# nreHieW/Eagle

Hardware: AMD Instinct MI355X
Metric: frames/sec end-to-end (detect+keypoint+homography) @1280x720 (higher is better)
Workload: dtype f32 (split: hi/lo binary16 pairs, 3 x fp16 MFMA per product, fp32 accumulate); detector (1.4 % of the FLOP): f32, exact v_mfma_f32_16x16x4_f32 chains

## Files before the change

### eagle_amd/csrc/common.h

```cpp
#pragma once
#include <hip/hip_runtime.h>
#include <hip/hip_fp16.h>
#include <cstdint>
#include <cstdio>
#include <string>
#include <vector>

#include "../../include/eagle.h"

namespace eagle {

enum Act : int { ACT_NONE = 0, ACT_RELU = 1, ACT_SILU = 2 };

struct Err {
    int code;
    std::string msg;
};
[[noreturn]] void fail(int code, const char* fmt, ...);

#define HIP_CHECK(expr)                                                                                \
    do {                                                                                               \
        hipError_t _e = (expr);                                                                        \
        if (_e != hipSuccess) ::eagle::fail(EAGLE_E_HIP, "%s failed: %s (%s:%d)", #expr, hipGetErrorString(_e), \
                                            __FILE__, __LINE__);                                       \
    } while (0)

void ensure_max_dynamic_lds(const void* fn, int bytes);

struct TView {
    void* p = nullptr;
    int n = 0, h = 0, w = 0;
    int c = 0;
    int cs = 0;
    int off = 0;
    int f32 = 0;
    size_t esize() const { return f32 ? 4 : 2; }
    TView slice(int o, int cc) const { TView v = *this; v.off = off + o; v.c = cc; return v; }
};

struct ConvConfig {
    int ks = 3, stride = 1;
    int kc = 0;
    int nt = 0;
    int wx = 2;
    int cin = 0, cout_pad = 0;
    int variant = 0;
};
struct ArgmaxPart { float score; int idx; };
struct ConvLaunch {
    ConvConfig cfg;
    TView x, y, r1, r2;
    const void* w = nullptr;
    const float* bias = nullptr;
    int pre_act = 0, post_act = 0;
    int out_f32 = 0;
    double flop = 0;
    float descale = 1.0f;
    ArgmaxPart* const* am_slot = nullptr;
    unsigned* const* sat_slot = nullptr;
};
int conv_tiles_per_frame(int precision, const ConvConfig& cfg, int ho, int wo);
void conv_tile_shape(int precision, const ConvConfig& cfg, int* th, int* tw);
bool conv_supported(int precision, const ConvConfig& cfg);
void conv_launch(int precision, const ConvLaunch& L, hipStream_t s);
size_t conv_weight_elems(int precision, const ConvConfig& cfg);
size_t conv_lds_bytes(int precision, const ConvConfig& cfg);
void conv_tile_weights(int precision, const ConvConfig& cfg, const float* w_hwio, int cin_real, int cout_real, void* dst, float* descale = nullptr);
inline int prec_tensor_fmt(int precision) { return precision == EAGLE_PREC_F32 ? 1 : precision == EAGLE_PREC_F32S ? 2 : 0; }
inline bool prec_is_f16_kernels(int precision) { return precision == EAGLE_PREC_F16 || precision == EAGLE_PREC_F32S; }
ConvConfig conv_choose(int precision, int ks, int stride, int cin_pad, int cout_pad, int wo, bool plain_epilogue = false, bool second_residual = false);

struct BneckLaunch {
    TView x, res, y;
    const void *w1 = nullptr, *w2 = nullptr, *w3 = nullptr;
    const float *b1 = nullptr, *b2 = nullptr, *b3 = nullptr;
    float ds1 = 1.f, ds2 = 1.f, ds3 = 1.f;
    unsigned* const* sat_slot = nullptr;
    unsigned long long* dbg = nullptr;
    bool ds_fused = false;
};
bool bneck_supported(const TView& x, int cmid, int cout);
void bneck_tile_weights(const float* w, int taps, int cin, int cout, std::vector<_Float16>& out, float* descale);
void bneck_scale_bias(std::vector<float>& b, float descale);
void bneck_launch(const BneckLaunch& L, hipStream_t s);

struct StemLaunch {
    const uint8_t* bgr = nullptr;
    int n = 0, sh = 0, sw = 0;
    int dh = 540, dw = 960;
    const void* w = nullptr;
    const float* bias = nullptr;
    float descale = 1.f;
    TView y;
    unsigned* const* sat_slot = nullptr;
};
bool stem_supported(int precision, int ks, int stride, int cin, int cout);
void stem_tile_weights(const float* w , std::vector<_Float16>& out, float* descale);
void stem_launch(const StemLaunch& L, hipStream_t s);

struct LetterBox { int new_h, new_w, top, left, out_h, out_w; };
LetterBox letterbox_geometry(int h, int w, int imgsz, int square = 0);
int detector_anchor_count(int h, int w, int imgsz, int square);
void preprocess_launch(int precision, const uint8_t* d_bgr, int n, int h, int w, const TView& kp, const TView& det,
                       const LetterBox& lb, hipStream_t s, int which = 3, int det_precision = -1);
struct FuseUp { TView z; };
void fuse_sum_launch(const TView& base, const FuseUp* ups, int n_up, int relu, const TView& y, hipStream_t s, unsigned* sat = nullptr);
void maxpool5_launch(const TView& x, const TView& y, hipStream_t s);
void upsample2_launch(const TView& x, const TView& y, hipStream_t s);
void split_to_f32_launch(const TView& x, const TView& y, hipStream_t s);

void heat_argmax_launch(const TView& logits, ArgmaxPart* parts, int chunks, hipStream_t s);

struct DetLevel { TView box, cls; int gh, gw; float stride; int a0; };
struct DetScratch {
    int A = 0;
    float* boxes = nullptr;
    float* conf = nullptr;
    int* cls = nullptr;
    unsigned long long* keys = nullptr;
    int* count = nullptr;
};
void yolo_decode_launch(const DetLevel* lv, int n_lv, int n, int nc, float conf_floor, const DetScratch& sc, hipStream_t s);

struct PostParams {
    int frame_h, frame_w, in_h, in_w;
    int hm_h, hm_w, hm_chunks;
    double keypoint_conf, detector_conf, ransac_thresh;
    float nms_iou;
    int ransac_max_iters, lm_iters;
};
void nms_launch(const DetScratch& sc, int n, const PostParams& pp, EagleFrameResult* d_out, hipStream_t s);
int nms_anchor_limit();
void check_anchor_limit(const EagleConfig& cfg);
void post_launch(const ArgmaxPart* parts, int n, const PostParams& pp, EagleFrameResult* d_out, hipStream_t s);
void reproject_launch(EagleFrameResult* d_recs, const double* d_Hs, const unsigned char* d_flags, int n, int frame_h, int frame_w, hipStream_t s);
void homography_only_launch(const float* d_img, const float* d_world, int npts, double thresh, int max_iters, int lm_iters,
                            double* d_H, uint8_t* d_mask, int* d_ok, hipStream_t s);


struct ClipView {
    const uint8_t* bgr = nullptr;
    const uint8_t* g[3] = {nullptr, nullptr, nullptr};
    int lh[3] = {0, 0, 0}, lw[3] = {0, 0, 0};
    int levels = 0;
    int n = 0, h = 0, w = 0;
};
struct MemList { int n; EagleFlowKp kp[EAGLE_N_LANDMARKS]; };
struct ChainState {
    int n_prev; EagleFlowKp prev[EAGLE_N_LANDMARKS];
    int has_H, compute_h; double H[9];
    int stalled;
    int error;
    int lk_valid, lk_n;
    float lk_prev[2 * EAGLE_N_LANDMARKS], lk_next[2 * EAGLE_N_LANDMARKS];
    unsigned char lk_status[EAGLE_N_LANDMARKS];
    int flow_n; EagleFlowKp flow[EAGLE_N_LANDMARKS];
};
void clip_view_levels(ClipView& cv);
void gray_pyramid_launch(const uint8_t* d_bgr, int n, int h, int w, uint8_t* g0, uint8_t* g1, uint8_t* g2, hipStream_t s);
void lk_launch(const ClipView& cv, int src_frame, int dst_frame, ChainState* st, const MemList* mem, int kint, hipStream_t s);
struct EccResult { int ok, iters; double rho; float M[6]; };
void ecc_small_launch(const uint8_t* gray, uint8_t* small, int n, int h, int w, int dh, int dw, double inv_scale , hipStream_t s);
void ecc_launch(const uint8_t* small, const uint8_t* carry, const int2* pairs, int n_pairs, EccResult* out, int h, int w, int max_iter, double eps, hipStream_t s);
struct YuvArgs {
    const uint8_t* src;
    uint8_t* dst;
    int h, w;
    int64_t frame_stride, y_pitch, c_offset, c_pitch, v_offset;
    int c_step;
    int vec;
};
void yuv_to_bgr_launch(const YuvArgs& a, int n, hipStream_t s);
struct AnnotArgs {
    const uint8_t* src;
    uint8_t* dst;
    const EaglePrim* prims;
    const int32_t* offs;
    int h, w, fmt;
    int64_t frame_stride, y_pitch, c_offset, c_pitch, v_offset;
    int c_step;
    int vec;
};
void annotate_launch(const AnnotArgs& a, int n, hipStream_t s);
int overlay_from_record(const EagleFrameResult& rec, const int32_t* team_ids, const int32_t* team_vals, int n_team, EaglePrim* out);
void check_prims(const EaglePrim* prims, const int32_t* offs, int n);
void team_colors_launch(const uint8_t* d_bgr, int n_frames, int fh, int fw, const EagleCrop* d_crops, int n_crops, int* d_counts, hipStream_t s);

void reid_crop_launch(const uint8_t* d_bgr, int n_frames, int fh, int fw, const EagleCrop* d_crops, int n, const TView& out, hipStream_t s);
void reid_conv7_launch(const TView& x, const float* w, const float* b, const TView& y, int n, hipStream_t s);
void reid_maxpool3s2_launch(const TView& x, const TView& y, int n, hipStream_t s);
void reid_avgpool2_launch(const TView& x, const TView& y, int n, hipStream_t s);
void reid_dw3_launch(const TView& x, const float* w, const float* b, const TView& y, int n, hipStream_t s);
void reid_gate_launch(const TView* streams, const float* w1, const float* b1, const float* w2, const float* b2, int c_real, int r, float* g, const TView& y, int n, hipStream_t s);
void reid_head_launch(const TView& x, const float* w, const float* b, float* feats, int dim, int n, hipStream_t s);

struct Tracker;
Tracker* tracker_create(const EagleTrackParams* p);
void tracker_destroy(Tracker* t);
bool tracker_apply(Tracker* t, EagleFrameResult* rec, int frame_h, int frame_w, double detector_conf, const double* warp = nullptr,
                   const float* feats = nullptr, const int* feat_det = nullptr, int n_feat = 0);
void similarity_ransac(const double* p0, const double* p1, int n, double* W6);
int lk_debug(const char* key, long long value, void* out, long long out_bytes);
void decode_mem_launch(const ArgmaxPart* parts, int n, const PostParams& pp, MemList* mem, int first, int stride, hipStream_t s);
void chain_launch(const ClipView& cv, ChainState* st, const MemList* mem, EagleFrameResult* recs, const PostParams& pp, int frame,
                  int kint, int hint, int calib, hipStream_t s);
void flow_filter_launch(const ClipView& cv, ChainState* st, int hue_frame, hipStream_t s);

}
```

### eagle_amd/csrc/conv.hip

```cpp
#include <algorithm>
#include <cmath>
#include <cstdlib>
#include <mutex>

#include "common.h"
#include "dmath.h"
#include "conv_internal.h"

namespace eagle {

static int f16_ps(int kc) { const int g = kc / 8; return kc * 2 + ((g % 2 == 0) ? 16 : 0); }
static int f16_ni(int ks, int kc) { return (ks * ks * (kc / 8) + 3) / 4; }

enum FormKind { GENERIC, WSTAT, ADIRECT };
enum StrideForm { S1, S2D, S2T, S1L };
enum WeightImage { W_F32, W_F16, W_F16_S2D, W_SPLIT, W_SPLIT_AD, W_SPLIT_S2D, W_SPLIT_M32 };
struct Form {
    int prec, variant, kind;
    int pw;
    int sform, rows, cols;
    int kc, nt, halo_bufs;
    int wimage;
    int grid_cap;
    ConvKernelGetter get;
};
static constexpr Form gen(int prec, int variant, int pw, int wimage, int kind = GENERIC) { return {prec, variant, kind, pw, S1, 0, 0, 0, 0, 0, wimage, 0, nullptr}; }
static constexpr Form ad(int prec, int variant, int sform, int rows, int cols, int nt, int halo_bufs, int wimage, ConvKernelGetter get, int grid_cap = 0)
{
    return {prec, variant, ADIRECT, 0, sform, rows, cols, prec == EAGLE_PREC_F16 ? 32 : 16, nt, halo_bufs, wimage, grid_cap, get};
}
static constexpr int F16 = EAGLE_PREC_F16, F32 = EAGLE_PREC_F32, F32S = EAGLE_PREC_F32S;
static constexpr Form g_forms[] = {
    gen(F32, 0, 4, W_F32), gen(F32, 3, 2, W_F32), gen(F32, 4, 1, W_F32),
    gen(F16, 0, 4, W_F16), gen(F16, 2, 4, W_F16), gen(F16, 3, 2, W_F16), gen(F16, 4, 1, W_F16), gen(F16, 6, 4, W_F16, WSTAT), gen(F16, 7, 2, W_F16, WSTAT),
    ad(F16, 8, S1, 4, 32, 12, 2, W_F16, conv_ad_kernel_s1_bn192), ad(F16, 9, S1, 8, 32, 6, 2, W_F16, conv_ad_kernel_s1_bn96),
    ad(F16, 10, S2D, 4, 32, 12, 2, W_F16_S2D, conv_ad_kernel_s2_bn192), ad(F16, 11, S2D, 8, 32, 6, 2, W_F16_S2D, conv_ad_kernel_s2_bn96),
    gen(F32S, 0, 4, W_SPLIT), gen(F32S, 3, 2, W_SPLIT), gen(F32S, 18, 6, W_SPLIT),
    ad(F32S, 8, S1, 4, 32, 12, 2, W_SPLIT_AD, conv_ad_split_kernel_bn192), ad(F32S, 9, S1, 8, 32, 6, 2, W_SPLIT_AD, conv_ad_split_kernel_bn96),
    ad(F32S, 10, S2D, 4, 32, 12, 2, W_SPLIT_S2D, conv_ad_split_kernel_s2_bn192), ad(F32S, 11, S2D, 8, 32, 6, 2, W_SPLIT_S2D, conv_ad_split_kernel_s2_bn96),
    ad(F32S, 12, S1, 8, 32, 3, 2, W_SPLIT_AD, conv_ad_split_kernel48), ad(F32S, 13, S1, 16, 32, 3, 1, W_SPLIT_AD, conv_ad_split_kernel48sb),
    ad(F32S, 19, S1, 16, 32, 3, 2, W_SPLIT_AD, conv_ad_split_kernel48ring, 256),
    ad(F32S, 14, S2T, 4, 32, 12, 1, W_SPLIT_AD, conv_ad_split_kernel_s2t_bn192), ad(F32S, 15, S2T, 4, 32, 6, 1, W_SPLIT_AD, conv_ad_split_kernel_s2t_bn96),
    ad(F32S, 21, S1, 4, 32, 12, 2, W_SPLIT_M32, conv_ad_split32_kernel_bn192), ad(F32S, 22, S1, 8, 32, 6, 2, W_SPLIT_M32, conv_ad_split32_kernel_bn96),
    ad(F32S, 23, S1, 2, 64, 12, 2, W_SPLIT_M32, conv_ad_split32_kernel_w64_bn192), ad(F32S, 24, S1, 4, 64, 6, 2, W_SPLIT_M32, conv_ad_split32_kernel_w64_bn96),
    ad(F32S, 27, S1L, 6, 30, 12, 2, W_SPLIT_M32, conv_ad_split32_kernel_lin30)};
static constexpr int LIN_PIXELS = 128;

static const Form* find_form(int precision, int variant)
{
    for (const Form& f : g_forms)
        if (f.prec == precision && f.variant == variant) return &f;
    return nullptr;
}
static const Form& form_of(int precision, const ConvConfig& c)
{
    const Form* f = find_form(precision, c.variant);
    if (!f) fail(EAGLE_E_NOKERNEL, "no conv kernel form: prec=%d variant=%d", precision, c.variant);
    return *f;
}
static int kind_of(int precision, const ConvConfig& c) { const Form* f = find_form(precision, c.variant); return f ? f->kind : -1; }

static size_t lds_bytes(int precision, const ConvConfig& c)
{
    const Form& f = form_of(precision, c);
    if (f.kind == ADIRECT) {
        int hpix, rec, strips;
        if (precision == EAGLE_PREC_F16) { hpix = f.sform == S2D ? (f.rows + 1) * 33 : (f.rows + 2) * 34; rec = 96; strips = 4 * 32 * 112; }
        else if (f.wimage == W_SPLIT_M32) { hpix = (f.rows + 2) * (f.cols + 2); rec = 80; strips = 4 * 32 * 128; }
        else { hpix = f.sform == S2T ? (2 * f.rows + 1) * 66 : (f.rows + 2) * 34; rec = 96; strips = 4 * 16 * 208; }
        const int slabs = ((hpix * rec + 1023) / 1024 + 3) / 4 * 4;
        return (size_t)f.halo_bufs * slabs * 1024 + strips;
    }
    const int th = 4 * f.pw / c.wx, tw = 16 * c.wx;
    const int hw = (tw - 1) * c.stride + c.ks, hh = (th - 1) * c.stride + c.ks;
    const int bn = c.nt * 16;
    if (precision == EAGLE_PREC_F16) {
        const size_t operands = (size_t)f16_ni(c.ks, c.kc) * 4 * bn * 16 + (size_t)hh * hw * f16_ps(c.kc);
        const size_t strips = (size_t)4 * f.pw * 16 * (bn * 2 + 16);
        return f.kind == WSTAT ? operands + strips + 16 : std::max(operands + 16, strips);
    }
    if (precision == EAGLE_PREC_F32S) {
        const size_t operands = (size_t)f16_ni(c.ks, c.kc) * 2 * 4 * bn * 16 + (size_t)hh * hw * f16_ps(2 * c.kc);
        const size_t strips = (size_t)4 * f.pw * 16 * (bn * 4 + 16);
        return std::max(operands + 16, strips);
    }
    return (size_t)c.ks * c.ks * (c.kc / 4) * 4 * bn * 4 + (size_t)hh * hw * (c.kc + 1) * 4;
}

size_t conv_lds_bytes(int precision, const ConvConfig& c) { return lds_bytes(precision, c); }
void conv_tile_shape(int precision, const ConvConfig& c, int* th, int* tw)
{
    const Form& f = form_of(precision, c);
    *th = f.kind == ADIRECT ? f.rows : 4 * f.pw / c.wx; *tw = f.kind == ADIRECT ? f.cols : 16 * c.wx;
}

int conv_tiles_per_frame(int precision, const ConvConfig& c, int ho, int wo)
{
    int th, tw;
    conv_tile_shape(precision, c, &th, &tw);
    if (form_of(precision, c).sform == S1L) return (ho * wo + LIN_PIXELS - 1) / LIN_PIXELS;
    return ((wo + tw - 1) / tw) * ((ho + th - 1) / th);
}

static const Inst* generic_inst(int precision, const ConvConfig& c)
{
    for (auto part : {conv_inst_part0, conv_inst_part1, conv_inst_part2, conv_inst_part3, conv_inst_split0, conv_inst_split1, conv_inst_split2}) {
        int n = 0;
        const Inst* t = part(&n);
        for (int k = 0; k < n; ++k)
            if (t[k].prec == precision && t[k].ks == c.ks && t[k].s == c.stride && t[k].kc == c.kc && t[k].nt == c.nt && t[k].variant == c.variant) return &t[k];
    }
    return nullptr;
}
bool conv_supported(int precision, const ConvConfig& c)
{
    const Form* f = find_form(precision, c.variant);
    if (f && f->kind == ADIRECT) return c.ks == 3 && c.stride == (f->sform == S1 || f->sform == S1L ? 1 : 2) && c.kc == f->kc && c.nt == f->nt;
    return f && generic_inst(precision, c);
}

struct Tuned { int ks, s, cin, cout, wo, kc, nt, wx, variant; };
static const Tuned g_tuned[] = {
#include "conv_tuned.inc"
    {0, 0, 0, 0, 0, 0, 0, 0, 0}};
static const Tuned g_tuned_f32[] = {
#include "conv_tuned_f32.inc"
    {0, 0, 0, 0, 0, 0, 0, 0, 0}};
static const Tuned g_tuned_split[] = {
#include "conv_tuned_split.inc"
    {0, 0, 0, 0, 0, 0, 0, 0, 0}};
static bool tuned_match(const Tuned& t, const ConvConfig& c, int wo, ConvConfig* q)
{
    if (t.ks != c.ks || t.s != c.stride || t.cin != c.cin || t.cout != c.cout_pad || t.wo != wo) return false;
    *q = c; q->kc = t.kc; q->nt = t.nt; q->wx = t.wx; q->variant = t.variant;
    return true;
}

static bool env_force(const char* name, int* a, int* b, int* c) { const char* f = getenv(name); return f && sscanf(f, "%d,%d,%d", a, b, c) == 3; }
static bool env_off(const char* name) { const char* e = getenv(name); return e && atoi(e) == 0; }

static const int g_nts[] = {6, 4, 3, 2, 1};
static ConvConfig with_ad(ConvConfig c, int kc, int v192, int v96)
{
    c.kc = kc;
    if (c.cout_pad % 192 == 0) { c.nt = 12; c.variant = v192; } else { c.nt = 6; c.variant = v96; }
    return c;
}

static ConvConfig choose_f32(ConvConfig c, int wo)
{
    ConvConfig q = c; q.kc = (c.cin < 16) ? 4 : 16;
    if (env_force("EAGLE_F32_FORCE", &q.nt, &q.wx, &q.variant) && (q.wx == 1 || q.wx == 2) && q.nt >= 1 && c.cout_pad % (16 * q.nt) == 0 &&
        conv_supported(EAGLE_PREC_F32, q) && lds_bytes(EAGLE_PREC_F32, q) <= 160 * 1024)
        return q;
    for (const Tuned& t : g_tuned_f32)
        if (tuned_match(t, c, wo, &q) && conv_supported(EAGLE_PREC_F32, q)) return q;
    c.nt = 1;
    for (int nt : g_nts)
        if (c.cout_pad % (16 * nt) == 0) { c.nt = nt; break; }
    c.kc = (c.cin < 16) ? 4 : 16;
    if (c.stride == 2 && c.ks == 3) {
        q = c; q.variant = 3;
        if (conv_supported(EAGLE_PREC_F32, q)) return q;
    }
    return c;
}

static ConvConfig choose_split(ConvConfig c, int wo, bool plain_epilogue)
{
    const int prec = EAGLE_PREC_F32S, cin = c.cin, cout = c.cout_pad;
    ConvConfig q = c;
    if (env_force("EAGLE_CONV_FORCE", &q.kc, &q.nt, &q.variant) && cin % q.kc == 0 && cout % (16 * q.nt) == 0 && conv_supported(prec, q) &&
        (form_of(prec, q).sform != S1L || (plain_epilogue && wo == form_of(prec, q).cols))) {
        if (form_of(prec, q).pw == 6) q.wx = 3;
        if (lds_bytes(prec, q) <= 160 * 1024) return q;
    }
    if (plain_epilogue && c.ks == 3 && c.stride == 2 && cin % 48 == 0 && cout % 96 == 0) return with_ad(c, 16, 14, 15);
    if (!env_off("EAGLE_CONV_M32") && plain_epilogue && c.ks == 3 && c.stride == 1 && cin % 16 == 0 && cout % 96 == 0) {
        q = with_ad(c, 16, 21, wo > 32 ? 24 : 22);
        if (q.variant == 21 && wo == 30) q.variant = 27;
        return q;
    }
    for (const Tuned& t : g_tuned_split)
        if (tuned_match(t, c, wo, &q)) {
            const Form* f = find_form(prec, q.variant);
            if (kind_of(prec, q) == ADIRECT && !(plain_epilogue && cin % (f->sform == S2D ? 16 : 48) == 0)) continue;
            if (conv_supported(prec, q) && lds_bytes(prec, q) <= 160 * 1024) return q;
        }
    if (plain_epilogue && c.ks == 3 && c.stride == 1 && cin % 48 == 0 && cout % 96 == 0) return with_ad(c, 16, 8, 9);
    static const int skcs[] = {32, 16, 8};
    long best = -1;
    c.nt = 1; c.kc = 8; c.variant = 0;
    for (int variant : {0, 3})
        for (int nt : g_nts) {
            if (cout % (16 * nt)) continue;
            for (int kc : skcs) {
                if (cin % kc) continue;
                ConvConfig t = c; t.nt = nt; t.kc = kc; t.variant = variant;
                if (!conv_supported(prec, t)) continue;
                if (lds_bytes(prec, t) > 80 * 1024) continue;
                const int pw = form_of(prec, t).pw;
                if (nt * pw > 12) continue;
                const long score = (long)nt * pw * 1000 + kc * 10 + (variant == 0 ? 1 : 0);
                if (score > best) { best = score; c.nt = nt; c.kc = kc; c.variant = variant; }
            }
        }
    return c;
}

static ConvConfig choose_f16(ConvConfig c, int wo, bool plain_epilogue, bool plain_one)
{
    const int prec = EAGLE_PREC_F16, cin = c.cin, cout = c.cout_pad;
    ConvConfig q = c;
    if (env_force("EAGLE_CONV_FORCE", &q.kc, &q.nt, &q.variant) && cin % q.kc == 0 && cout % (16 * q.nt) == 0 && conv_supported(prec, q) &&
        lds_bytes(prec, q) <= 160 * 1024 && (kind_of(prec, q) == WSTAT ? plain_one : kind_of(prec, q) == ADIRECT ? plain_epilogue : true))
        return q;
    if (plain_epilogue && c.ks == 3 && c.stride == 1 && cin % 32 == 0 && cout % 96 == 0) return with_ad(c, 32, 8, 9);
    if (plain_epilogue && c.ks == 3 && c.stride == 2 && cin % 8 == 0 && cin >= 32 && cout % 96 == 0) return with_ad(c, 32, 10, 11);
    for (const Tuned& t : g_tuned)
        if (tuned_match(t, c, wo, &q)) {
            if (kind_of(prec, q) == WSTAT && !plain_one) continue;
            if (conv_supported(prec, q) && lds_bytes(prec, q) <= 160 * 1024) return q;
        }
    static const int kcs[] = {64, 48, 32, 16, 8};
    long best = -1;
    c.nt = 1; c.kc = 8;
    for (int nt : g_nts) {
        if (cout % (16 * nt)) continue;
        for (int kc : kcs) {
            if (cin % kc) continue;
            ConvConfig t = c; t.nt = nt; t.kc = kc;
            if (!conv_supported(prec, t)) continue;
            if (lds_bytes(prec, t) > 80 * 1024) continue;
            const long score = (long)kc * nt * 1000 + kc;
            if (score > best) { best = score; c.nt = nt; c.kc = kc; }
        }
    }
    return c;
}

ConvConfig conv_choose(int precision, int ks, int stride, int cin_pad, int cout_pad, int wo, bool plain_epilogue, bool second_residual)
{
    ConvConfig c;
    c.ks = ks; c.stride = stride; c.cin = cin_pad; c.cout_pad = cout_pad;
    c.wx = (wo > 16) ? 2 : 1;
    if (precision == EAGLE_PREC_F32) return choose_f32(c, wo);
    if (precision == EAGLE_PREC_F32S) return choose_split(c, wo, plain_epilogue);
    return choose_f16(c, wo, plain_epilogue, plain_epilogue && !second_residual);
}

size_t conv_weight_elems(int precision, const ConvConfig& c)
{
    const int bn = c.nt * 16, nblk = c.cout_pad / bn, nch = c.cin / c.kc;
    switch (form_of(precision, c).wimage) {
    case W_F16_S2D: return (size_t)nblk * (4 * c.cin / 32) * 16 * bn * 8;
    case W_F16: return (size_t)nblk * nch * f16_ni(c.ks, c.kc) * 4 * bn * 8;
    case W_SPLIT_S2D: return (size_t)nblk * (4 * c.cin / 16) * 6 * 4 * bn * 8;
    case W_SPLIT_M32: return (size_t)nblk * (c.cin / 16) * 18 * (bn / 32) * 512;
    case W_SPLIT_AD: return (size_t)nblk * (c.cin / 16) * 14 * 4 * bn * 8;
    case W_SPLIT: return (size_t)nblk * nch * f16_ni(c.ks, c.kc) * 2 * 4 * bn * 8;
    default: return (size_t)nblk * nch * c.ks * c.ks * (c.kc / 4) * 4 * bn;
    }
}

void conv_tile_weights(int precision, const ConvConfig& c, const float* w, int cin_real, int cout_real, void* dst, float* descale)
{
    const int bn = c.nt * 16, nblk = c.cout_pad / bn, nch = c.cin / c.kc, taps = c.ks * c.ks, wimage = form_of(precision, c).wimage;
    auto W = [&](int tap, int ci, int co) -> float {
        return (ci < cin_real && co < cout_real) ? w[((size_t)tap * cin_real + ci) * cout_real + co] : 0.0f;
    };
    if (descale) *descale = 1.0f;
    if (precision == EAGLE_PREC_F32S) {
        float amax = 0.f;
        for (size_t k = 0; k < (size_t)taps * cin_real * cout_real; ++k) amax = std::max(amax, std::fabs(w[k]));
        int e = 0;
        if (amax > 0.f) (void)std::frexp(amax, &e);
        const int sw = 15 - e;
        const float scale = std::ldexp(1.0f, sw);
        if (descale) *descale = std::ldexp(1.0f, -(sw + 4));
        _Float16* d = (_Float16*)dst;
        if (wimage == W_SPLIT_S2D) {
            const int per_phase = c.cin / 16;
            for (int b = 0; b < nblk; ++b)
                for (int ch = 0; ch < 4 * per_phase; ++ch)
                    for (int k = 0; k < 6; ++k)
                        for (int qq = 0; qq < 4; ++qq)
                            for (int nn = 0; nn < bn; ++nn)
                                for (int j = 0; j < 8; ++j) {
                                    const int ph = ch / per_phase, c0 = (ch - ph * per_phase) * 16, ry = ph >> 1, rx = ph & 1;
                                    const int tp = k < 4 ? k : 2 * (k - 4) + (qq >> 1), tyy = tp >> 1, txx = tp & 1;
                                    const int ky = tyy == 0 ? (ry == 1 ? 0 : -1) : (ry == 0 ? 1 : 2), kx = txx == 0 ? (rx == 1 ? 0 : -1) : (rx == 0 ? 1 : 2);
                                    float v = 0.f;
                                    if (ky >= 0 && kx >= 0) v = W(ky * 3 + kx, c0 + (qq & 1) * 8 + j, b * bn + nn) * scale;
                                    const _Float16 hi = (_Float16)v;
                                    *d++ = k < 4 ? hi : (_Float16)(v - (float)hi);
                                }
            return;
        }
        if (wimage == W_SPLIT_M32) {
            for (int b = 0; b < nblk; ++b)
                for (int ch = 0; ch < c.cin / 16; ++ch)
                    for (int tap = 0; tap < 9; ++tap)
                        for (int part = 0; part < 2; ++part)
                            for (int mb = 0; mb < bn / 32; ++mb)
                                for (int l = 0; l < 64; ++l)
                                    for (int j = 0; j < 8; ++j) {
                                        const float v = W(tap, ch * 16 + (l >> 5) * 8 + j, b * bn + mb * 32 + (l & 31)) * scale;
                                        const _Float16 hi = (_Float16)v;
                                        *d++ = part == 0 ? hi : (_Float16)(v - (float)hi);
                                    }
            return;
        }
        if (wimage == W_SPLIT_AD) {
            for (int b = 0; b < nblk; ++b)
                for (int ch = 0; ch < c.cin / 16; ++ch)
                    for (int k = 0; k < 14; ++k)
                        for (int qq = 0; qq < 4; ++qq)
                            for (int nn = 0; nn < bn; ++nn)
                                for (int j = 0; j < 8; ++j) {
                                    const int tap = k < 9 ? k : 2 * (k - 9) + (qq >> 1);
                                    float v = 0.f;
                                    if (tap < 9) v = W(tap, ch * 16 + (qq & 1) * 8 + j, b * bn + nn) * scale;
                                    const _Float16 hi = (_Float16)v;
                                    *d++ = k < 9 ? hi : (_Float16)(v - (float)hi);
                                }
            return;
        }
        const int G = c.kc / 8, NGR = taps * G, NI = f16_ni(c.ks, c.kc);
        for (int b = 0; b < nblk; ++b)
            for (int ch = 0; ch < nch; ++ch)
                for (int i = 0; i < NI; ++i)
                    for (int part = 0; part < 2; ++part)
                        for (int qq = 0; qq < 4; ++qq)
                            for (int nn = 0; nn < bn; ++nn)
                                for (int j = 0; j < 8; ++j) {
                                    const int g = 4 * i + qq;
                                    float v = 0.f;
                                    if (g < NGR) { const int tap = g / G, cg = g % G; v = W(tap, ch * c.kc + cg * 8 + j, b * bn + nn) * scale; }
                                    const _Float16 hi = (_Float16)v;
                                    *d++ = part == 0 ? hi : (_Float16)(v - (float)hi);
                                }
        return;
    }
    if (wimage == W_F16_S2D) {
        _Float16* d = (_Float16*)dst;
        const int nch2 = 4 * c.cin / 32;
        for (int b = 0; b < nblk; ++b)
            for (int ch = 0; ch < nch2; ++ch)
                for (int g = 0; g < 16; ++g)
                    for (int nn = 0; nn < bn; ++nn)
                        for (int j = 0; j < 8; ++j) {
                            const int tp = g / 4, cg = g % 4, tyy = tp >> 1, txx = tp & 1;
                            const int sc = ch * 32 + cg * 8 + j, ph = sc / c.cin, ci = sc - ph * c.cin, ry = ph >> 1, rx = ph & 1;
                            const int ky = tyy == 0 ? (ry == 1 ? 0 : -1) : (ry == 0 ? 1 : 2), kx = txx == 0 ? (rx == 1 ? 0 : -1) : (rx == 0 ? 1 : 2);
                            *d++ = (_Float16)((ky < 0 || kx < 0) ? 0.f : W(ky * 3 + kx, ci, b * bn + nn));
                        }
        return;
    }
    if (precision == EAGLE_PREC_F16) {
        const int G = c.kc / 8, NGR = taps * G, NI = f16_ni(c.ks, c.kc);
        _Float16* d = (_Float16*)dst;
        for (int b = 0; b < nblk; ++b)
            for (int ch = 0; ch < nch; ++ch)
                for (int g = 0; g < NI * 4; ++g)
                    for (int nn = 0; nn < bn; ++nn)
                        for (int j = 0; j < 8; ++j) {
                            float v = 0.f;
                            if (g < NGR) {
                                const int tap = g / G, cg = g % G;
                                v = W(tap, ch * c.kc + cg * 8 + j, b * bn + nn);
                            }
                            *d++ = (_Float16)v;
                        }
    } else {
        const int CSTEPS = c.kc / 4;
        float* d = (float*)dst;
        for (int b = 0; b < nblk; ++b)
            for (int ch = 0; ch < nch; ++ch)
                for (int tap = 0; tap < taps; ++tap)
                    for (int cs = 0; cs < CSTEPS; ++cs)
                        for (int qq = 0; qq < 4; ++qq)
                            for (int nn = 0; nn < bn; ++nn) *d++ = W(tap, ch * c.kc + cs * 4 + qq, b * bn + nn);
    }
}

static std::mutex g_page_mutex;
static const void* conv_zero_page()
{
    static void* z[64] = {};
    int dev = 0;
    HIP_CHECK(hipGetDevice(&dev));
    std::lock_guard<std::mutex> g(g_page_mutex);
    if (!z[dev]) { HIP_CHECK(hipMalloc(&z[dev], 256)); HIP_CHECK(hipMemset(z[dev], 0, 256)); }
    return z[dev];
}
static void* conv_trash_page()
{
    static void* z[64] = {};
    int dev = 0;
    HIP_CHECK(hipGetDevice(&dev));
    std::lock_guard<std::mutex> g(g_page_mutex);
    if (!z[dev]) HIP_CHECK(hipMalloc(&z[dev], 8192));
    return z[dev];
}

void conv_launch(int precision, const ConvLaunch& L, hipStream_t s)
{
    const ConvConfig& c = L.cfg;
    if (!conv_supported(precision, c)) fail(EAGLE_E_NOKERNEL, "no conv kernel instance: prec=%d ks=%d s=%d kc=%d nt=%d", precision, c.ks, c.stride, c.kc, c.nt);
    const Form& f = form_of(precision, c);
    ConvArgs a;
    a.x = L.x.p; a.xcs = L.x.cs; a.xoff = L.x.off; a.N = L.x.n; a.H = L.x.h; a.W = L.x.w;
    a.w = L.w; a.bias = L.bias;
    a.y = L.y.p; a.ycs = L.y.cs; a.yoff = L.y.off; a.Ho = L.y.h; a.Wo = L.y.w;
    a.r1 = L.r1.p; a.r1cs = L.r1.cs; a.r1off = L.r1.off;
    a.r2 = L.r2.p; a.r2cs = L.r2.cs; a.r2off = L.r2.off;
    a.descale = L.descale;
    if (precision == EAGLE_PREC_F32S) {
        if (L.x.f32 != 2 || (L.r1.p && L.r1.f32 != 2) || (L.r2.p && L.r2.f32 != 2) || L.y.f32 != (L.out_f32 ? 1 : 2))
            fail(EAGLE_E_INVALID, "split conv: operand tensor formats do not match the family");
        a.xcs *= 2; a.xoff *= 2; a.r1cs *= 2; a.r1off *= 2; a.r2cs *= 2; a.r2off *= 2;
        if (!L.out_f32) { a.ycs *= 2; a.yoff *= 2; }
    }
    if (!a.r1 && a.r2) { a.r1 = a.r2; a.r1cs = a.r2cs; a.r1off = a.r2off; a.r2 = nullptr; }
    a.pre_act = L.pre_act; a.post_act = L.post_act; a.out_f32 = L.out_f32 || precision == EAGLE_PREC_F32;
    a.wx = c.wx;
    a.nchunks = c.cin / c.kc;
    a.zeros = conv_zero_page(); a.trash = conv_trash_page(); a.xcd = 0; a.gy = 1; a.stack = 0;
    a.am = L.am_slot ? *L.am_slot : nullptr; a.am_cs = c.cout_pad;
    a.sat = (L.sat_slot && precision == EAGLE_PREC_F32S) ? *L.sat_slot : nullptr;
    if (f.kind == ADIRECT) {
        if (a.out_f32 || a.pre_act != 0 || a.post_act > 1 || L.am_slot || (precision == EAGLE_PREC_F32S && c.cin % (f.wimage == W_SPLIT_AD ? 48 : 16)))
            fail(EAGLE_E_NOKERNEL, "A-direct conv needs 2-byte / split output, pre_act none, post_act in {none, ReLU} and, in the split family, Cin = 16 k (48 k for variants 8, 9 and 12 - 15)");
        if (f.sform == S2D) a.nchunks = 4 * c.cin / c.kc;
        a.tiles_x = (a.Wo + f.cols - 1) / f.cols; a.tiles_y = (a.Ho + f.rows - 1) / f.rows;
        if (f.sform == S1L) {
            if (a.Wo != f.cols || a.W != a.Wo || a.H != a.Ho) fail(EAGLE_E_NOKERNEL, "linear A-direct conv (variant %d) needs a map %d columns wide, got %d x %d", c.variant, f.cols, a.Ho, a.Wo);
            a.tiles_x = (a.Ho * a.Wo + LIN_PIXELS - 1) / LIN_PIXELS; a.tiles_y = 1;
        }
        a.gy = c.cout_pad / (c.nt * 16);
        const size_t lim = (size_t)1 << 31;
        if ((size_t)a.N * a.H * a.W * a.xcs * 2 >= lim || (size_t)a.N * a.Ho * a.Wo * std::max(std::max(a.ycs, a.r1 ? a.r1cs : 0), a.r2 ? a.r2cs : 0) * 2 >= lim)
            fail(EAGLE_E_INVALID, "fp16 conv: a tensor of %d frames reaches 2 GiB; use a smaller device batch", a.N);
        const int nres = (a.r1 ? 1 : 0) + (a.r2 ? 1 : 0);
        const int items = a.tiles_x * a.tiles_y * a.N * a.gy;
        const bool deep = items <= 256;
        for (bool d : {false, true}) ensure_max_dynamic_lds((const void*)f.get(nres, d), 160 * 1024);
        hipLaunchKernelGGL(f.get(nres, deep), dim3(f.grid_cap ? std::min(items, f.grid_cap) : items), dim3(256), lds_bytes(precision, c), s, a);
        HIP_CHECK(hipGetLastError());
        return;
    }
    const int th = 4 * f.pw / c.wx, tw = 16 * c.wx;
    a.tiles_x = (a.Wo + tw - 1) / tw; a.tiles_y = (a.Ho + th - 1) / th;
    if (precision == EAGLE_PREC_F32) {
        if (!env_off("EAGLE_F32_STACK") && c.stride == 1 && a.N > 1 && a.Ho == a.H) { a.stack = 1; a.tiles_y = (a.N * (a.Ho + 1) + th - 1) / th; }
        if ((size_t)a.N * a.H * a.W * a.xcs * 4 >= ((size_t)1 << 31)) fail(EAGLE_E_INVALID, "fp32 conv: the input tensor of %d frames reaches 2 GiB; use a smaller device batch", a.N);
    }
    const bool ws = f.kind == WSTAT;
    if (a.am && (!prec_is_f16_kernels(precision) || ws))
        fail(EAGLE_E_NOKERNEL, "fused heat-map maxima need the generic fp16 kernel");
    if (prec_is_f16_kernels(precision)) {
        const size_t lim = (size_t)1 << 31;
        const size_t cs_out = std::max(std::max(a.out_f32 ? 2 * a.ycs : a.ycs, a.r1 ? a.r1cs : 0), a.r2 ? a.r2cs : 0);
        if ((size_t)a.N * a.H * a.W * a.xcs * 2 >= lim || (size_t)a.N * a.Ho * a.Wo * cs_out * 2 >= lim)
            fail(EAGLE_E_INVALID, "fp16 conv: a tensor of %d frames reaches 2 GiB; use a smaller device batch", a.N);
    }
    const ConvKernel fn = generic_inst(precision, c)->fn;
    const size_t lds = lds_bytes(precision, c);
    ensure_max_dynamic_lds((const void*)fn, 160 * 1024);
    const int gy = c.cout_pad / (c.nt * 16);
    int gx = a.stack ? a.tiles_x * a.tiles_y : a.tiles_x * a.tiles_y * a.N;
    if (ws) {
        if (c.kc != c.cin || a.out_f32 || a.r2 || a.pre_act != 0 || a.post_act > 1 || (size_t)a.N * a.H * a.W * a.xcs * 2 >= (1ull << 31) || (size_t)a.N * a.Ho * a.Wo * std::max(a.ycs, a.r1 ? a.r1cs : 0) * 2 >= (1ull << 31))
            fail(EAGLE_E_NOKERNEL, "weight-stationary conv needs kc == cin, fp16 output, at most one residual, pre_act none, post_act in {none, ReLU} and tensors below 2 GiB (kc=%d cin=%d)", c.kc, c.cin);
        const int per_cu = (int)std::max<size_t>(1, std::min<size_t>(2, (160 * 1024) / lds));
        const int unit = 8 * gy;
        gx = std::max(unit, std::min((gx * gy + unit - 1) / unit * unit, 256 * per_cu / unit * unit));
    }
    a.gy = gy;
    a.xcd = (prec_is_f16_kernels(precision) && !ws && (c.ks == 3 || (c.ks == 1 && gy > 1))) ? 1 : 0;
    dim3 grid(gx, gy);
    if (a.xcd) grid = dim3(gx * gy, 1);
    if (ws) grid = dim3(gx, 1);
    hipLaunchKernelGGL(fn, grid, dim3(256), lds, s, a);
    HIP_CHECK(hipGetLastError());
}

}
```

### eagle_amd/csrc/conv_ad_split.inc

```
#ifndef EAGLE_CONV_AD_SPLIT_INC
#define EAGLE_CONV_AD_SPLIT_INC
#ifndef EAGLE_ABL_AD
#define EAGLE_ABL_AD 0
#endif
#if EAGLE_ABL_AD == 1 || EAGLE_ABL_AD == 6
__device__ __forceinline__ f32x4 abl_ad_xor(const half8& a_, const half8& b_, f32x4 c_)
{
    const u32x4 ua = __builtin_bit_cast(u32x4, a_), ub = __builtin_bit_cast(u32x4, b_);
    u32x4 uc = __builtin_bit_cast(u32x4, c_);
    uc[0] = uc[0] ^ ua[0] ^ ub[3];
    return __builtin_bit_cast(f32x4, uc);
}
#define EAGLE_MFMA_AD(A_, B_, C_) abl_ad_xor(A_, B_, C_)
#else
#define EAGLE_MFMA_AD(A_, B_, C_) __builtin_amdgcn_mfma_f32_16x16x32_f16(A_, B_, C_, 0, 0, 0)
#endif
template <int CQ, int PG, int RES, int KQ = 1, bool SB = false, bool S2 = false, bool S2T = false>
__global__ __launch_bounds__(256, 2) void conv_split_ad_kernel(ConvArgs a)
{
    static_assert(!S2 || (KQ == 1 && !SB), "stride-2 form: plain ring");
    static_assert(!S2T || (SB && !S2 && PG == 1), "true stride-2 form: one pixel group, single halo buffer");
    static_assert(CQ * PG * KQ == 4, "four waves per workgroup");
    static_assert(!SB || KQ == 1 || S2T, "single-buffer form: no K split (except the true stride-2 form)");
    static_assert(KQ == 1 || (KQ == 2 && (CQ == 1 || S2T)), "K split: one Cout group (two in the true stride-2 form)");
// ... 51 lines not shown
#pragma unroll
        for (int s = 0; s < KPW; ++s) {
            int o[2];
#pragma unroll
            for (int hq = 0; hq < 2; ++hq) {
                const int kg = hq * KPW + s;
                if (kg < 9) {
                    o[hq] = bbase + tapoff(kg) * PS;
                } else {
                    const int t0 = 2 * (kg - 9), t1 = t0 + 1 < 9 ? t0 + 1 : t0;
                    o[hq] = bpair + bsel * ((tapoff(t1) - tapoff(t0)) * PS) + tapoff(t0) * PS;
                }
            }
            bk[s] = kq == 0 ? o[0] : o[1];
        }
    }

    auto decode = [&](int item, int& n, int& ty, int& tx, int& nb) {
        int t = item / gy; nb = item - t * gy;
        tx = t % a.tiles_x; t /= a.tiles_x;
        ty = t % a.tiles_y; n = t / a.tiles_y;
    };
    int h_g = 0, h_ch = 0, h_item = item0;
    int h_iy0, h_ix0, h_gb;
    auto halo_origin = [&](int item) {
        int n, ty, tx, nb; decode(item, n, ty, tx, nb);
        h_iy0 = S2T ? 2 * ty * TH - 1 : ty * TH - 1; h_ix0 = S2T ? 64 * tx - 1 : tx * 32 - 1;
        h_gb = S2 ? n * a.H : (((n * a.H + h_iy0) * a.W + h_ix0) * a.xcs + a.xoff) * 2;
    };
    const int cin_s2 = nch * 4;
    halo_origin(h_item);
    auto issue_h = [&]() {
        char* dst = Hb + (SB ? 0 : (h_g & 1)) * HB;
        const unsigned so = S2 ? 0u : (unsigned)(h_ch * 32) * 2u;
        const int s2_ph = S2 ? (h_ch * 16) / cin_s2 : 0, s2_c0 = S2 ? h_ch * 16 - s2_ph * cin_s2 : 0;
#pragma unroll
        for (int k = 0; k < HK; ++k) {
            int hy, hx, unit; bool live;
            if constexpr (RECOMP) {
                int e = e0 + NW * 64 * k;
                asm volatile("" : "+v"(e));
                const int pix = (int)(((unsigned)e * 43691u) >> 18), slot = e - pix * 6;
                hy = S2T ? (int)(((unsigned)pix * 993u) >> 16) : S2 ? (int)(((unsigned)pix * 1986u) >> 16) : (int)(((unsigned)pix * 1928u) >> 16); hx = pix - hy * HW_;
                unit = (slot & 1) * 2 + (slot >> 1);
                live = pix < HPIX && slot < 4;
                if constexpr (S2T) { const int pl = hx >= 33 ? 1 : 0; hx = 2 * (hx - 33 * pl) + pl; live = live && hx <= 64; }
            } else {
                hy = hpk[k] & 0xFF; hx = (hpk[k] >> 8) & 0xFF; unit = (hpk[k] >> 16) & 7; live = hpk[k] >= 0;
            }
            const int iy = S2 ? 2 * (h_iy0 + hy) + (s2_ph >> 1) : h_iy0 + hy, ix = S2 ? 2 * (h_ix0 + hx) + (s2_ph & 1) : h_ix0 + hx;
            const unsigned off = !(live && (unsigned)iy < (unsigned)a.H && (unsigned)ix < (unsigned)a.W) ? OOB
                                 : S2 ? (unsigned)((((h_gb + iy) * a.W + ix) * a.xcs + a.xoff + 2 * s2_c0 + unit * 8) * 2)
                                      : (unsigned)(h_gb + ((hy * a.W + hx) * a.xcs + unit * 8) * 2);
            __builtin_amdgcn_raw_ptr_buffer_load_lds(xrs, (__attribute__((address_space(3))) void*)(dst + (wave + NW * k) * 1024), 16,
                                                     ((EAGLE_ABL_AD == 3 || EAGLE_ABL_AD >= 6) && h_g > 0) ? OOB : off, so, 0, 0);
        }
        if (h_g + 1 >= GC) return;
        ++h_g;
        if (++h_ch == nch) { h_ch = 0; ++h_item; halo_origin(h_item); }
    };
    if constexpr (!SB) issue_h();
    int gc = 0;
    for (int item = item0; item < item_end; ++item) {
        int n, ty, tx, nb; decode(item, n, ty, tx, nb);
        const int oy0 = ty * TH, ox0 = tx * 32;
        f32x4 acc[NT][PW];
#pragma unroll
        for (int i = 0; i < NT; ++i)
#pragma unroll
            for (int p = 0; p < PW; ++p) acc[i][p] = f32x4{0.f, 0.f, 0.f, 0.f};
        u32x4 A[RING][NT];
        unsigned wsrc = (unsigned)(nb * nch * KPC * 4) * (unsigned)(BN * 16) + (unsigned)(kq * KPW) * KSTEP;
        const unsigned wend = wsrc - (unsigned)(kq * KPW) * KSTEP + (unsigned)(nch * KPC) * KSTEP;
        int a_s = 0;
        bool abl_a_done = false;
        auto load_a = [&](int slot) {
            const unsigned so = wsrc < wend ? wsrc : wend - KSTEP;
#pragma unroll
            for (int tt = 0; tt < NT; ++tt)
                if (!((EAGLE_ABL_AD == 2 || EAGLE_ABL_AD >= 6) && abl_a_done)) A[slot][tt] = __builtin_amdgcn_raw_buffer_load_b128(wrs, wlane + tt * 256, so, 0);
            wsrc += KSTEP;
            if constexpr (KQ > 1) { if (++a_s == KPW) { a_s = 0; wsrc += (unsigned)(KPC - KPW) * KSTEP; } }
        };
        load_a(0); load_a(1);
        abl_a_done = true;
        auto chunk = [&](auto ph_, auto k0_) {
            constexpr int PH = decltype(ph_)::value, K0 = decltype(k0_)::value;
            if constexpr (SB) {
                __builtin_amdgcn_s_barrier();
                issue_h();
                asm volatile("s_waitcnt vmcnt(0)" ::: "memory");
                __builtin_amdgcn_s_barrier();
            } else {
                asm volatile("s_waitcnt vmcnt(6)" ::: "memory");
                __builtin_amdgcn_s_barrier();
                issue_h();
            }
            const char* hb = Hb + (SB ? 0 : (gc & 1)) * HB;
            half8 B[2][PW];
            auto read_b = [&](int slot, int kk) {
                if constexpr (KQ == 2) {
#pragma unroll
                    for (int p = 0; p < PW; ++p)
                        B[slot][p] = *(const half8*)(hb + bk[kk] + ((p >> 1) * ROWREC + (p & 1) * 16) * PS);
                } else if constexpr (S2) {
                    const int tp = kk < 4 ? kk : 2 * (kk - 4), ky = tp >> 1, kx = tp & 1;
                    const char* hp = kk < 4 ? hb + bbase : hb + bpair + bsel * PS;
#pragma unroll
                    for (int p = 0; p < PW; ++p)
                        B[slot][p] = *(const half8*)(hp + (((p >> 1) + ky) * HW_ + (p & 1) * 16 + kx) * PS);
                } else if (kk < 9) {
#pragma unroll
                    for (int p = 0; p < PW; ++p)
                        B[slot][p] = *(const half8*)(hb + bbase + ((p >> 1) * ROWREC + (p & 1) * 16 + tapoff(kk)) * PS);
                } else {
                    const int t0 = 2 * (kk - 9), t1 = t0 + 1 < 9 ? t0 + 1 : t0;
                    const int d = (tapoff(t1) - tapoff(t0)) * PS;
                    const char* hp = hb + bpair + bsel * d;
#pragma unroll
                    for (int p = 0; p < PW; ++p)
                        B[slot][p] = *(const half8*)(hp + ((p >> 1) * ROWREC + (p & 1) * 16 + tapoff(t0)) * PS);
                }
            };
            read_b(0, K0);
#pragma unroll
            for (int kk = 0; kk < KPW; ++kk) {
                load_a((PH + kk + 2) % RING);
                if (kk + 1 < KPW && !(EAGLE_ABL_AD == 4 || EAGLE_ABL_AD == 6)) read_b((kk + 1) & 1, K0 + kk + 1);
#pragma unroll
                for (int tt = 0; tt < NT; ++tt)
#pragma unroll
                    for (int p = 0; p < PW; ++p)
                        acc[tt][p] = EAGLE_MFMA_AD((half8)A[(PH + kk) % RING][tt], B[(EAGLE_ABL_AD == 4 || EAGLE_ABL_AD == 6) ? 0 : (kk & 1)][p], acc[tt][p]);
                __builtin_amdgcn_sched_barrier(0);
            }
        };
        using I0 = std::integral_constant<int, 0>;
        constexpr int P1 = KPW % RING, P2 = (2 * KPW) % RING;
        if constexpr (S2) {
            for (int ch = 0; ch < nch; ++ch) { chunk(I0{}, I0{}); ++gc; }
        } else
        for (int ch = 0; ch < nch; ch += 3) {
            if constexpr (KQ == 1) {
                chunk(I0{}, I0{}); ++gc;
                chunk(std::integral_constant<int, P1>{}, I0{}); ++gc;
                chunk(std::integral_constant<int, P2>{}, I0{}); ++gc;
            } else {
                chunk(I0{}, I0{}); ++gc;
                chunk(std::integral_constant<int, P1>{}, I0{}); ++gc;
                chunk(std::integral_constant<int, P2>{}, I0{}); ++gc;
            }
        }
        const int co0 = nb * BN + cq * 48;
        __builtin_amdgcn_sched_barrier(0);
        constexpr int NHR = 8 / KQ;
        const int row0 = (KQ == 2 && kq == 1) ? 2 : 0;
        if constexpr (KQ == 2) {
            if (kq == 1) {
#pragma unroll
                for (int tt = 0; tt < NT; ++tt)
#pragma unroll
                    for (int p = 0; p < 4; ++p) { const f32x4 t = acc[tt][p]; acc[tt][p] = acc[tt][p + 4]; acc[tt][p + 4] = t; }
            }
            char* const X = SB ? Hb : Hb + ((gc - 1) & 1) * HB;
            const int mine = wave * 6144, theirs = (wave ^ (CQ * PG)) * 6144;
#pragma unroll
            for (int rnd = 0; rnd < 2; ++rnd) {
                __builtin_amdgcn_s_barrier();
#pragma unroll
                for (int pp = 0; pp < 2; ++pp)
#pragma unroll
                    for (int tt = 0; tt < NT; ++tt) *(f32x4*)(X + mine + ((pp * NT + tt) * 64 + lane) * 16) = acc[tt][4 + rnd * 2 + pp];
                __builtin_amdgcn_fence(__ATOMIC_RELEASE, "workgroup", "local");
                __builtin_amdgcn_s_barrier();
                __builtin_amdgcn_fence(__ATOMIC_ACQUIRE, "workgroup", "local");
#pragma unroll
                for (int pp = 0; pp < 2; ++pp)
#pragma unroll
                    for (int tt = 0; tt < NT; ++tt) {
                        const f32x4 o = *(const f32x4*)(X + theirs + ((pp * NT + tt) * 64 + lane) * 16);
#pragma unroll
                        for (int r = 0; r < 4; ++r) acc[tt][rnd * 2 + pp][r] = kq == 0 ? acc[tt][rnd * 2 + pp][r] + o[r] : o[r] + acc[tt][rnd * 2 + pp][r];
                    }
            }
        }
        float4 bias[NT];
#pragma unroll
        for (int tt = 0; tt < NT; ++tt) bias[tt] = *(const float4*)(a.bias + co0 + tt * 16 + q * 4);
        const float ds = a.descale;
        int pstrip[3], ppx[3];
#pragma unroll
        for (int i = 0; i < 3; ++i) {
            const int e = i * 64 + lane, px = e / 12, gq = e - px * 12;
            pstrip[i] = px * RS + gq * 16;
            ppx[i] = px | (gq << 8);
        }
        auto piece_off = [&](int hr, int i, int cs, int off) -> unsigned {
            const int oy = oy0 + pg * 4 + row0 + (hr >> 1), ox2 = ox0 + (hr & 1) * 16 + (ppx[i] & 0xFF), gq = ppx[i] >> 8;
            return (oy < a.Ho && ox2 < a.Wo) ? (unsigned)((((n * a.Ho + oy) * a.Wo + ox2) * cs + off + co0 * 2 + gq * 8) * 2) : OOB;
        };
        float vmax = 0.0f;
        constexpr int HRB = (RES == 2 || KQ == 2) ? 4 : 8;
        u32x4 rres[RES >= 1 ? HRB : 1][3], rres2[RES >= 2 ? HRB : 1][3];
#pragma unroll
        for (int hb0 = 0; hb0 < NHR; hb0 += HRB) {
            if (RES >= 1) {
#pragma unroll
                for (int h2 = 0; h2 < HRB; ++h2)
#pragma unroll
                    for (int i = 0; i < 3; ++i) rres[h2][i] = __builtin_amdgcn_raw_buffer_load_b128(rrs, piece_off(hb0 + h2, i, a.r1cs, a.r1off), 0, EAGLE_RES_NT * 2);
            }
            if (RES >= 2) {
#pragma unroll
                for (int h2 = 0; h2 < HRB; ++h2)
#pragma unroll
                    for (int i = 0; i < 3; ++i) rres2[h2][i] = __builtin_amdgcn_raw_buffer_load_b128(rrs2, piece_off(hb0 + h2, i, a.r2cs, a.r2off), 0, EAGLE_RES_NT * 2);
            }
#pragma unroll
            for (int h2 = 0; h2 < HRB; ++h2) {
                const int p = hb0 + h2;
                if (RES >= 1) {
#pragma unroll
                    for (int i = 0; i < 3; ++i) *(u32x4*)(strip + pstrip[i]) = rres[h2][i];
                }
                float v[NT][4];
#pragma unroll
                for (int tt = 0; tt < NT; ++tt) {
                    const char* sp = strip + lx * RS + split_elem(tt * 16 + q * 4) * 2;
                    v[tt][0] = acc[tt][p][0] * ds + bias[tt].x; v[tt][1] = acc[tt][p][1] * ds + bias[tt].y;
                    v[tt][2] = acc[tt][p][2] * ds + bias[tt].z; v[tt][3] = acc[tt][p][3] * ds + bias[tt].w;
                    if (RES >= 1) {
                        const half4 rh = *(const half4*)sp, rl = *(const half4*)(sp + 16);
#pragma unroll
                        for (int r = 0; r < 4; ++r) v[tt][r] = ((float)rh[r] + (float)rl[r]) * SPLIT_RX + v[tt][r];
                    }
                }
                if (RES >= 2) {
#pragma unroll
                    for (int i = 0; i < 3; ++i) *(u32x4*)(strip + pstrip[i]) = rres2[h2][i];
#pragma unroll
                    for (int tt = 0; tt < NT; ++tt) {
                        const char* sp = strip + lx * RS + split_elem(tt * 16 + q * 4) * 2;
                        const half4 rh = *(const half4*)sp, rl = *(const half4*)(sp + 16);
#pragma unroll
                        for (int r = 0; r < 4; ++r) v[tt][r] = v[tt][r] + ((float)rh[r] + (float)rl[r]) * SPLIT_RX;
                    }
                }
#pragma unroll
                for (int tt = 0; tt < NT; ++tt) {
                    if (a.post_act == 1) {
#pragma unroll
                        for (int r = 0; r < 4; ++r) v[tt][r] = v[tt][r] > 0.f ? v[tt][r] : 0.f;
                    }
                    split_store4(strip + lx * RS + split_elem(tt * 16 + q * 4) * 2, v[tt][0], v[tt][1], v[tt][2], v[tt][3]);
                    vmax = split_absmax4(vmax, v[tt][0], v[tt][1], v[tt][2], v[tt][3]);
                }
#pragma unroll
                for (int i = 0; i < 3; ++i)
                    __builtin_amdgcn_raw_buffer_store_b128(*(const u32x4*)(strip + pstrip[i]), yrs, (EAGLE_ABL_AD >= 5) ? OOB : piece_off(p, i, a.ycs, a.yoff), 0, EAGLE_STORE_NT * 2);
            }
        }
        split_report(a.sat, n, vmax);
    }
}

#endif
```

### eagle_amd/csrc/conv_internal.h

```cpp
#pragma once
#include "common.h"

namespace eagle {

using half8 = __attribute__((ext_vector_type(8))) _Float16;
using half4 = __attribute__((ext_vector_type(4))) _Float16;
using f32x4 = __attribute__((ext_vector_type(4))) float;
using u32x4 = __attribute__((ext_vector_type(4))) unsigned int;
using u32x2 = __attribute__((ext_vector_type(2))) unsigned int;

struct ConvArgs {
    const void* x; int xcs, xoff; int N, H, W;
    const void* w; const float* bias;
    void* y; int ycs, yoff; int Ho, Wo;
    const void* r1; int r1cs, r1off;
    const void* r2; int r2cs, r2off;
    int pre_act, post_act, out_f32;
    int wx, tiles_x, tiles_y, nchunks;
    int gy;
    int stack;
    int xcd;
    ArgmaxPart* am;
    int am_cs;
    float descale;
    const void* zeros;
    void* trash;
    unsigned* sat;
};

struct BneckArgs {
    const void* x; int xcs, xoff; int N, H, W, nch1;
    const void *w1, *w2, *w3; const float *b1, *b2, *b3; float ds1, ds2, ds3;
    const void* r; int rcs, roff;
    void* y; int ycs, yoff;
    int tiles_x, tiles_y;
    unsigned* sat;
    unsigned long long* dbg;
};

typedef void (*ConvKernel)(ConvArgs);
struct Inst { int prec, ks, s, kc, nt, variant; ConvKernel fn; };
const Inst* conv_inst_part0(int* n); const Inst* conv_inst_part1(int* n); const Inst* conv_inst_part2(int* n); const Inst* conv_inst_part3(int* n);
const Inst* conv_inst_split0(int* n); const Inst* conv_inst_split1(int* n); const Inst* conv_inst_split2(int* n);
inline int res_slot(int n_res) { return n_res < 0 ? 0 : n_res > 2 ? 2 : n_res; }
typedef ConvKernel (*ConvKernelGetter)(int n_res, bool deep);
ConvKernel conv_ad_kernel_s1_bn192(int n_res, bool deep);
ConvKernel conv_ad_kernel_s1_bn96(int n_res, bool deep);
ConvKernel conv_ad_kernel_s2_bn192(int n_res, bool deep);
ConvKernel conv_ad_kernel_s2_bn96(int n_res, bool deep);
ConvKernel conv_ad_split_kernel_bn192(int n_res, bool deep);
ConvKernel conv_ad_split_kernel_bn96(int n_res, bool deep);
ConvKernel conv_ad_split_kernel_s2_bn192(int n_res, bool deep);
ConvKernel conv_ad_split_kernel_s2_bn96(int n_res, bool deep);
ConvKernel conv_ad_split_kernel_s2t_bn192(int n_res, bool deep);
ConvKernel conv_ad_split_kernel_s2t_bn96(int n_res, bool deep);
ConvKernel conv_ad_split_kernel48(int n_res, bool deep);
ConvKernel conv_ad_split_kernel48sb(int n_res, bool deep);
ConvKernel conv_ad_split_kernel48ring(int n_res, bool deep);
ConvKernel conv_ad_split32_kernel_bn192(int n_res, bool deep);
ConvKernel conv_ad_split32_kernel_bn96(int n_res, bool deep);
ConvKernel conv_ad_split32_kernel_w64_bn192(int n_res, bool deep);
ConvKernel conv_ad_split32_kernel_w64_bn96(int n_res, bool deep);
ConvKernel conv_ad_split32_kernel_lin30(int n_res, bool deep);

}
```

### eagle_amd/csrc/nets.hip

```cpp
#include "runtime.h"

namespace eagle {

struct Builder {
    EagleHandle* H;
    Net* net;
    int prec;
    double bn_eps;
    int N;
    const char* label_suffix = "";
    int cur_stream = 0;
    void set_stream(int k) { cur_stream = k; net->pool = k; }
    void fork_join(Op::Kind kind, int nbranch) { Op op; op.kind = kind; op.nbranch = nbranch; op.tag = kind == Op::FORK ? "fork" : "join"; net->ops.push_back(op); }

    int gran() const { return prec == EAGLE_PREC_F32 ? 4 : 8; }

    TView act(int h, int w, int c, bool f32 = false)
    {
        TView v; v.n = N; v.h = h; v.w = w; v.c = c; v.cs = c; v.off = 0;
        v.f32 = (f32 || prec == EAGLE_PREC_F32) ? 1 : prec_tensor_fmt(prec);
        v.p = net->get((size_t)N * h * w * c * v.esize());
        return v;
    }
    void release(const TView& v) { net->put(v.p); }

    const HostTensor& W(const std::string& name)
    {
        auto it = H->weights.find(name);
        if (it == H->weights.end()) fail(EAGLE_E_MISSING, "weight tensor '%s' was not loaded", name.c_str());
        return it->second;
    }

    TView conv(const TView& x, const std::string& cname, const std::string& bn, int stride, int pre, const TView* r1,
               const TView* r2, int post, const TView* out = nullptr, bool out_f32 = false, ArgmaxPart* const* am_slot = nullptr)
    {
        std::vector<float> hwio, bias; int cin, cout, ks;
        fold(cname, bn, hwio, bias, cin, cout, ks);
        if (cin > x.c) fail(EAGLE_E_INVALID, "%s: input has %d channels, weight expects %d", cname.c_str(), x.c, cin);
        const int cout_pad = (cout + 15) / 16 * 16;
        bias.resize(cout_pad, 0.f);
        const int ho = (x.h + 2 * (ks / 2) - ks) / stride + 1, wo = (x.w + 2 * (ks / 2) - ks) / stride + 1;
        if (const char* dump = getenv("EAGLE_DUMP_LAYERS")) {
            if (FILE* f = fopen(dump, "a")) { fprintf(f, "%d,%d,%d,%d,%d,%d,%d\n", ks, stride, x.c, cout_pad, x.h, x.w, N); fclose(f); }
        }
        ConvLaunch L;
        L.cfg = conv_choose(prec, ks, stride, x.c, cout_pad, wo, pre == ACT_NONE && post <= ACT_RELU && !out_f32, r1 && r2);
        if (!conv_supported(prec, L.cfg))
            fail(EAGLE_E_NOKERNEL, "%s: no kernel instance (ks=%d s=%d kc=%d nt=%d)", cname.c_str(), ks, stride, L.cfg.kc, L.cfg.nt);
        const size_t ne = conv_weight_elems(prec, L.cfg);
        std::vector<char> tiled(ne * (prec == EAGLE_PREC_F32 ? 4 : 2));
        conv_tile_weights(prec, L.cfg, hwio.data(), cin, cout, tiled.data(), &L.descale);
        L.w = net->upload(tiled.data(), tiled.size());
        L.bias = (const float*)net->upload(bias.data(), bias.size() * 4);
        L.x = x;
        if (out) {
            L.y = *out;
            if (out->c != cout_pad || out->h != ho || out->w != wo) fail(EAGLE_E_INVALID, "%s: output slice mismatch", cname.c_str());
        } else {
            L.y = act(ho, wo, cout_pad, out_f32);
        }
        if (r1) L.r1 = *r1;
        if (r2) L.r2 = *r2;
        L.pre_act = pre; L.post_act = post; L.out_f32 = out_f32 ? 1 : 0;
        refuse_2gib(cname, "layer", {&L.x, &L.y, r1 ? &L.r1 : nullptr, r2 ? &L.r2 : nullptr});
        L.am_slot = am_slot;
        if (prec == EAGLE_PREC_F32S && !out_f32 && !am_slot) L.sat_slot = &H->cur_sat;
        if (am_slot) { H->hm_chunks = conv_tiles_per_frame(prec, L.cfg, ho, wo); H->fused_argmax = true; }
        L.flop = 2.0 * N * ho * wo * (double)cout * cin * ks * ks;
        const int pr = prec;
        char label[64];
        snprintf(label, sizeof(label), "conv %dx%d/%d %d->%d @%dx%d v%d%s", ks, ks, stride, cin, cout, ho, wo, L.cfg.variant, label_suffix);
        const double es = prec == EAGLE_PREC_F16 ? 2 : 4;
        emit_conv(label, L.flop, (double)N * x.h * x.w * cin * es + (double)N * ho * wo * cout * ((out_f32 || prec != EAGLE_PREC_F16) ? 4 : 2) * (am_slot ? 0 : 1) +
                                 (r1 ? (double)N * ho * wo * cout * es : 0) + (r2 ? (double)N * ho * wo * cout * es : 0) + (double)ks * ks * cin * cout * es,
                  [L, pr](hipStream_t s) { conv_launch(pr, L, s); });
        return L.y;
    }
    void fold(const std::string& cname, const std::string& bn, std::vector<float>& hwio, std::vector<float>& bias, int& cin, int& cout, int& ks)
    {
        const HostTensor& w = W(cname + ".weight");
        if (w.shape.size() != 4) fail(EAGLE_E_INVALID, "%s.weight: expected 4-d", cname.c_str());
        cout = (int)w.shape[0]; cin = (int)w.shape[1]; ks = (int)w.shape[2];
        hwio.assign((size_t)ks * ks * cin * cout, 0.f); bias.assign(cout, 0.f);
        std::vector<double> scale(cout, 1.0);
        if (!bn.empty()) {
            const HostTensor &g = W(bn + ".weight"), &b = W(bn + ".bias"), &m = W(bn + ".running_mean"), &v = W(bn + ".running_var");
            for (int o = 0; o < cout; ++o) {
                scale[o] = (double)g.data[o] / std::sqrt((double)v.data[o] + bn_eps);
                bias[o] = (float)((double)b.data[o] - (double)m.data[o] * scale[o]);
            }
        } else if (H->weights.count(cname + ".bias")) {
            const HostTensor& b = W(cname + ".bias");
            for (int o = 0; o < cout; ++o) bias[o] = b.data[o];
        }
        for (int o = 0; o < cout; ++o)
            for (int i = 0; i < cin; ++i)
                for (int t = 0; t < ks * ks; ++t) {
                    const float wv = w.data[((size_t)o * cin + i) * ks * ks + t];
                    hwio[((size_t)t * cin + i) * cout + o] = bn.empty() ? wv : (float)((double)wv * scale[o]);
                }
    }
    void refuse_2gib(const std::string& name, const char* what, std::initializer_list<const TView*> ts)
    {
        for (const TView* t : ts)
            if (t && (size_t)t->n * t->h * t->w * t->cs * t->esize() >= ((size_t)1 << 31))
                fail(EAGLE_E_INVALID, "%s: a %d x %d x %d x %d-channel tensor of this %s reaches 2 GiB at a device batch of %d frames (32-bit tensor offsets); use a smaller EagleConfig.batch",
                     name.c_str(), t->n, t->h, t->w, t->cs, what, N);
    }
    void emit_conv(const char* label, double flop, double bytes, std::function<void(hipStream_t)> run)
    {
        net->names.emplace_back(new std::string(label));
        Op op; op.kind = Op::CONV; op.flop = flop; op.bytes = bytes; op.tag = net->names.back()->c_str(); op.stream = cur_stream; op.run = std::move(run);
        net->ops.push_back(op);
    }
    TView bottleneck(const TView& x, const std::string& q, const TView& res, const std::string& ds_conv = "", const std::string& ds_bn = "")
    {
        BneckLaunch L;
        const bool dsf = !ds_conv.empty();
        std::vector<float> hw, bs; int ci, co, ks;
        std::vector<_Float16> img;
        double flop = 0;
        const char* cn[3] = {"conv1", "conv2", "conv3"}; const char* bnn[3] = {"bn1", "bn2", "bn3"};
        const int want_ks[3] = {1, 3, 1}, want_ci[3] = {x.c, 64, 64}, want_co[3] = {64, 64, 256};
        for (int k = 0; k < 3; ++k) {
            fold(q + cn[k], q + bnn[k], hw, bs, ci, co, ks);
            if (ks != want_ks[k] || ci != want_ci[k] || co != want_co[k]) fail(EAGLE_E_INVALID, "%s%s: not the Bottleneck shape of the fused kernel", q.c_str(), cn[k]);
            if (k == 2 && dsf) {
                std::vector<float> hwd, bd; int cid, cod, ksd;
                fold(ds_conv, ds_bn, hwd, bd, cid, cod, ksd);
                if (ksd != 1 || cid != 64 || cod != 256 || x.c != 64) fail(EAGLE_E_INVALID, "%s: not the 1x1 64->256 downsample of the fused kernel", ds_conv.c_str());
                hw.insert(hw.end(), hwd.begin(), hwd.end());
                for (int o = 0; o < 256; ++o) bs[o] = bs[o] + bd[o];
                ci = 128;
                flop += 2.0 * N * x.h * x.w * 256.0 * 64;
            }
            float ds = 1.f;
            bneck_tile_weights(hw.data(), ks * ks, ci, co, img, &ds);
            bneck_scale_bias(bs, ds);
            const void* dw = net->upload(img.data(), img.size() * 2);
            const float* db = (const float*)net->upload(bs.data(), bs.size() * 4);
            if (k == 0) { L.w1 = dw; L.b1 = db; L.ds1 = ds; } else if (k == 1) { L.w2 = dw; L.b2 = db; L.ds2 = ds; } else { L.w3 = dw; L.b3 = db; L.ds3 = ds; }
            flop += 2.0 * N * x.h * x.w * (double)co * (k == 2 ? 64 : ci) * ks * ks;
        }
        L.x = x; L.y = act(x.h, x.w, 256); L.res = dsf ? L.y : res; L.ds_fused = dsf;
        L.sat_slot = &H->cur_sat;
        refuse_2gib(q, "block", {&L.x, &L.y, &L.res});
        char label[64];
        snprintf(label, sizeof(label), "bneck %d->64->256%s @%dx%d%s", x.c, dsf ? "+ds" : "", x.h, x.w, label_suffix);
        emit_conv(label, flop, (double)N * x.h * x.w * 4.0 * (x.c + 256 + ((dsf || res.p == x.p) ? 0 : 256)) + 4.0 * (x.c * 64 + 9 * 64 * 64 + 64 * 256 + (dsf ? 64 * 256 : 0)),
                  [L](hipStream_t s) { bneck_launch(L, s); });
        return L.y;
    }
    TView stem(const TView& x_in, const std::string& cname, const std::string& bn)
    {
        std::vector<float> hwio, bias; int cin, cout, ks;
        fold(cname, bn, hwio, bias, cin, cout, ks);
        if (!stem_supported(prec, ks, 2, cin, cout)) fail(EAGLE_E_NOKERNEL, "%s: not the 3x3/2 3->64 convolution of the fused stem", cname.c_str());
        StemLaunch L;
        std::vector<_Float16> img;
        stem_tile_weights(hwio.data(), img, &L.descale);
        L.w = net->upload(img.data(), img.size() * 2);
        L.bias = (const float*)net->upload(bias.data(), bias.size() * 4);
        L.sh = H->cfg.frame_h; L.sw = H->cfg.frame_w; L.dh = x_in.h; L.dw = x_in.w;
        L.y = act((x_in.h - 1) / 2 + 1, (x_in.w - 1) / 2 + 1, 64);
        L.sat_slot = &H->cur_sat;
        refuse_2gib(cname, "layer", {&L.y});
        const double flop = 2.0 * N * L.y.h * L.y.w * 64.0 * 27;
        char label[64];
        snprintf(label, sizeof(label), "conv stem 3x3/2 3->64 @%dx%d%s", L.y.h, L.y.w, label_suffix);
        EagleHandle* const Hh = H;
        emit_conv(label, flop, (double)N * L.sh * L.sw * 3.0 + (double)N * L.y.h * L.y.w * 64 * 4.0 + 27.0 * 64 * 4,
                  [L, Hh](hipStream_t s) { StemLaunch l = L; l.bgr = Hh->cur_src; l.n = Hh->cur_n; stem_launch(l, s); });
        return L.y;
    }
    static double vbytes(const TView& v) { return (double)v.n * v.h * v.w * v.c * (v.f32 ? 4 : 2); }
    void other(std::function<void(hipStream_t)> fn, const char* tag, double bytes = 0)
    {
        Op op; op.kind = Op::OTHER; op.run = std::move(fn); op.tag = tag; op.stream = cur_stream; op.bytes = bytes;
        net->ops.push_back(op);
    }
};

static const char* HRP = "unnormalized_model.0.";

static std::vector<TView> hr_stage(Builder& B, std::vector<TView> xs, int stage_idx, int n_modules, int nb, bool last_single)
{
    const int R = ACT_RELU;
    for (int m = 0; m < n_modules; ++m) {
        const std::string q = std::string(HRP) + "stage" + std::to_string(stage_idx) + "." + std::to_string(m) + ".";
        B.fork_join(Op::FORK, nb - 1);
        const bool interleave = !(getenv("EAGLE_HR_INTERLEAVE") && atoi(getenv("EAGLE_HR_INTERLEAVE")) == 0);
        for (int step = 0; step < 4 * nb; ++step) {
            const int k = interleave ? step / nb : step % 4, b = interleave ? nb - 1 - step % nb : step / 4;
            B.set_stream(b);
            TView x = xs[b];
            const std::string r = q + "branches." + std::to_string(b) + "." + std::to_string(k) + ".";
            TView o = B.conv(x, r + "conv1", r + "bn1", 1, 0, nullptr, nullptr, R);
            TView y = B.conv(o, r + "conv2", r + "bn2", 1, 0, &x, nullptr, R);
            B.release(o);
            B.release(x);
            xs[b] = y;
        }
        B.set_stream(0);
        B.fork_join(Op::JOIN, nb - 1);
        const int n_out = (last_single && m == n_modules - 1) ? 1 : nb;
        std::vector<TView> out;
        if (n_out > 1) B.fork_join(Op::FORK, n_out - 1);
        for (int i = 0; i < n_out; ++i) {
            B.set_stream(n_out > 1 ? i : 0);
            TView y; bool have_y = false;
            for (int j = 0; j < i; ++j) {
                TView t = xs[j];
                for (int k = 0; k < i - j; ++k) {
                    const std::string r = q + "fuse_layers." + std::to_string(i) + "." + std::to_string(j) + "." + std::to_string(k) + ".";
                    const bool last = k == i - j - 1;
                    TView nt;
                    if (!last) {
                        nt = B.conv(t, r + "0", r + "1", 2, 0, nullptr, nullptr, R);
                    } else {
                        const TView* ident = (j == i - 1) ? &xs[i] : nullptr;
                        const bool relu_now = ident && i == nb - 1;
                        nt = B.conv(t, r + "0", r + "1", 2, 0, have_y ? &y : nullptr, ident, relu_now ? R : 0);
                    }
                    if (k > 0) B.release(t);
                    t = nt;
                }
                if (have_y) B.release(y);
                y = t; have_y = true;
            }
            if (i == 0) y = xs[0];
            FuseUp ups[3]; int nu = 0;
            for (int j = i + 1; j < nb; ++j) {
                const std::string r = q + "fuse_layers." + std::to_string(i) + "." + std::to_string(j) + ".";
                ups[nu++].z = B.conv(xs[j], r + "0", r + "1", 1, 0, nullptr, nullptr, 0);
            }
            if (nu) {
                TView o = B.act(y.h, y.w, y.c);
                const TView base = y; FuseUp u0 = ups[0], u1 = ups[1], u2 = ups[2]; const int n_up = nu;
                EagleHandle* const Hh = B.H;
                B.other([base, u0, u1, u2, n_up, o, Hh](hipStream_t s) { FuseUp u[3] = {u0, u1, u2}; fuse_sum_launch(base, u, n_up, 1, o, s, Hh->cur_sat); }, "fuse_sum",
                        Builder::vbytes(base) + Builder::vbytes(o) + (nu > 0 ? Builder::vbytes(ups[0].z) : 0) + (nu > 1 ? Builder::vbytes(ups[1].z) : 0) + (nu > 2 ? Builder::vbytes(ups[2].z) : 0));
                for (int k = 0; k < nu; ++k) B.release(ups[k].z);
                if (i != 0) B.release(y);
                y = o;
            }
            out.push_back(y);
        }
        B.set_stream(0);
        if (n_out > 1) B.fork_join(Op::JOIN, n_out - 1);
        for (int b = 0; b < nb; ++b) B.release(xs[b]);
        xs = out;
    }
    return xs;
}

static TView build_hrnet(Builder& B, const TView& x_in)
{
    const int R = ACT_RELU;
    const std::string P = HRP;
    TView x = B.H->stem_on ? B.stem(x_in, P + "conv1", P + "bn1") : B.conv(x_in, P + "conv1", P + "bn1", 2, 0, nullptr, nullptr, R);
    TView x2 = B.conv(x, P + "conv2", P + "bn2", 2, 0, nullptr, nullptr, R);
    B.release(x); x = x2;
    for (int b = 0; b < 4; ++b) {
        const std::string q = P + "layer1." + std::to_string(b) + ".";
        const char* fe = getenv("EAGLE_BNECK_FUSED");
        const char* de = getenv("EAGLE_BNECK_DS");
        const bool fused = B.prec == EAGLE_PREC_F32S && !(fe && atoi(fe) == 0) && bneck_supported(x, 64, 256);
        const bool dsf = fused && b == 0 && x.c == 64 && !(de && atoi(de) == 0);
        TView res = x;
        if (b == 0 && !dsf) res = B.conv(x, q + "downsample.0", q + "downsample.1", 1, 0, nullptr, nullptr, 0);
        if (fused) {
            TView y = dsf ? B.bottleneck(x, q, x, q + "downsample.0", q + "downsample.1") : B.bottleneck(x, q, res);
            if (b == 0 && !dsf) B.release(res);
            B.release(x);
            x = y;
            continue;
        }
        TView o1 = B.conv(x, q + "conv1", q + "bn1", 1, 0, nullptr, nullptr, R);
        TView o2 = B.conv(o1, q + "conv2", q + "bn2", 1, 0, nullptr, nullptr, R);
        TView y = B.conv(o2, q + "conv3", q + "bn3", 1, 0, &res, nullptr, R);
        B.release(o1); B.release(o2);
        if (b == 0) B.release(res);
        B.release(x);
        x = y;
    }
    std::vector<TView> ys(2);
    B.fork_join(Op::FORK, 1);
    B.set_stream(1);
    ys[1] = B.conv(x, P + "transition1.1.0.0", P + "transition1.1.0.1", 2, 0, nullptr, nullptr, R);
    B.set_stream(0);
    ys[0] = B.conv(x, P + "transition1.0.0", P + "transition1.0.1", 1, 0, nullptr, nullptr, R);
    B.fork_join(Op::JOIN, 1);
    B.release(x);
    ys = hr_stage(B, ys, 2, 1, 2, false);
    ys.push_back(B.conv(ys.back(), P + "transition2.2.0.0", P + "transition2.2.0.1", 2, 0, nullptr, nullptr, R));
    ys = hr_stage(B, ys, 3, 4, 3, false);
    ys.push_back(B.conv(ys.back(), P + "transition3.3.0.0", P + "transition3.3.0.1", 2, 0, nullptr, nullptr, R));
    ys = hr_stage(B, ys, 4, 3, 4, true);
    ArgmaxPart* const* am = (prec_is_f16_kernels(B.prec) && !getenv("EAGLE_NO_FUSED_ARGMAX")) ? &B.H->cur_parts : nullptr;
    TView logits = B.conv(ys[0], "unnormalized_model.1", "", 1, 0, nullptr, nullptr, 0, nullptr, true, am);
    B.release(ys[0]);
    return logits;
}

struct YoloDims { int c[5]; int n[4]; };
static YoloDims yolo_dims(int variant)
{
    static const double D[5] = {0.33, 0.33, 0.67, 1.0, 1.0}, Wd[5] = {0.25, 0.5, 0.75, 1.0, 1.25};
    static const int MC[5] = {1024, 1024, 768, 512, 512};
    YoloDims y;
    const int base[5] = {64, 128, 256, 512, 1024};
    for (int i = 0; i < 5; ++i) y.c[i] = (int)std::ceil(std::min(base[i], MC[variant]) * Wd[variant] / 8.0) * 8;
    const int rep[4] = {3, 6, 6, 3};
    for (int i = 0; i < 4; ++i) y.n[i] = std::max((int)std::nearbyint(rep[i] * D[variant]), 1);
    return y;
}

struct YoloBuilder {
    Builder& B;
    int S = ACT_SILU;
    TView cv(const TView& x, const std::string& name, int stride = 1, const TView* r1 = nullptr, const TView* out = nullptr)
    {
        return B.conv(x, name + ".conv", name + ".bn", stride, S, r1, nullptr, 0, out);
    }
    TView c2f(const TView& x, int idx, int cout, int n, bool shortcut, const TView* out = nullptr)
    {
        const std::string p = "model." + std::to_string(idx);
        const int c = cout / 2;
        TView cat = B.act(x.h, x.w, (2 + n) * c);
        TView first = cat.slice(0, 2 * c);
        cv(x, p + ".cv1", 1, nullptr, &first);
        for (int k = 0; k < n; ++k) {
            TView in = cat.slice((1 + k) * c, c);
            TView t = cv(in, p + ".m." + std::to_string(k) + ".cv1");
            TView o = cat.slice((2 + k) * c, c);
            cv(t, p + ".m." + std::to_string(k) + ".cv2", 1, shortcut ? &in : nullptr, &o);
            B.release(t);
        }
        TView y = cv(cat, p + ".cv2", 1, nullptr, out);
        B.release(cat);
        return y;
    }
};

static void build_yolo(Builder& B, const TView& x_in, int variant, DetLevel lv[3], int nc, bool mixed = false)
{
    YoloBuilder Y{B};
    const YoloDims d = yolo_dims(variant);
    const int c1 = d.c[0], c2 = d.c[1], c3 = d.c[2], c4 = d.c[3], c5 = d.c[4];
    TView x0 = Y.cv(x_in, "model.0", 2);
    TView x1 = Y.cv(x0, "model.1", 2); B.release(x0);
    TView x2 = Y.c2f(x1, 2, c2, d.n[0], true); B.release(x1);
    TView x3 = Y.cv(x2, "model.3", 2); B.release(x2);
    const int h3 = x3.h, w3 = x3.w;
    const int h4 = (h3 - 1) / 2 + 1, w4 = (w3 - 1) / 2 + 1, h5 = (h4 - 1) / 2 + 1, w5 = (w4 - 1) / 2 + 1;
    TView cat15 = B.act(h3, w3, c4 + c3);
    TView cat12 = B.act(h4, w4, c5 + c4);
    TView cat18 = B.act(h4, w4, c3 + c4);
    TView cat21 = B.act(h5, w5, c4 + c5);
    TView p3 = cat15.slice(c4, c3), p4 = cat12.slice(c5, c4), p5 = cat21.slice(c4, c5), h12 = cat18.slice(c3, c4);
    Y.c2f(x3, 4, c3, d.n[1], true, &p3); B.release(x3);
    TView x5 = Y.cv(p3, "model.5", 2);
    Y.c2f(x5, 6, c4, d.n[2], true, &p4); B.release(x5);
    TView x7 = Y.cv(p4, "model.7", 2);
    TView x8 = Y.c2f(x7, 8, c5, d.n[3], true); B.release(x7);
    {
        const int ch = c5 / 2;
        TView cat = B.act(h5, w5, 4 * ch);
        TView s0 = cat.slice(0, ch), s1 = cat.slice(ch, ch), s2 = cat.slice(2 * ch, ch), s3 = cat.slice(3 * ch, ch);
        Y.cv(x8, "model.9.cv1", 1, nullptr, &s0); B.release(x8);
        B.other([s0, s1](hipStream_t s) { maxpool5_launch(s0, s1, s); }, "maxpool5", 2 * Builder::vbytes(s0));
        B.other([s1, s2](hipStream_t s) { maxpool5_launch(s1, s2, s); }, "maxpool5", 2 * Builder::vbytes(s0));
        B.other([s2, s3](hipStream_t s) { maxpool5_launch(s2, s3, s); }, "maxpool5", 2 * Builder::vbytes(s0));
        Y.cv(cat, "model.9.cv2", 1, nullptr, &p5);
        B.release(cat);
    }
    {
        TView u = cat12.slice(0, c5);
        B.other([p5, u](hipStream_t s) { upsample2_launch(p5, u, s); }, "upsample2", Builder::vbytes(p5) + Builder::vbytes(u));
        Y.c2f(cat12, 12, c4, d.n[0], false, &h12);
    }
    TView h15, h18, h21;
    {
        TView u = cat15.slice(0, c4);
        B.other([h12, u](hipStream_t s) { upsample2_launch(h12, u, s); }, "upsample2", Builder::vbytes(h12) + Builder::vbytes(u));
    }
    if (!mixed) {
        h15 = Y.c2f(cat15, 15, c3, d.n[0], false);
        {
            TView o = cat18.slice(0, c3);
            Y.cv(h15, "model.16", 2, nullptr, &o);
        }
        h18 = Y.c2f(cat18, 18, c4, d.n[0], false);
        {
            TView o = cat21.slice(0, c4);
            Y.cv(h18, "model.19", 2, nullptr, &o);
        }
        h21 = Y.c2f(cat21, 21, c5, d.n[0], false);
    } else {
        B.prec = EAGLE_PREC_F32;
        auto to_f32 = [&B](const TView& x, const TView& y) {
            B.other([x, y](hipStream_t s) { split_to_f32_launch(x, y, s); }, "split_to_f32", Builder::vbytes(x) + Builder::vbytes(y));
// ... 225 lines not shown
```

### eagle_amd/csrc/ops_api.hip

```cpp
#include "runtime.h"

extern "C" {

static void to_dev(Net& net, int prec, const float* src, int n, int h, int w, int c, int cpad, TView& v)
{
    v.n = n; v.h = h; v.w = w; v.c = cpad; v.cs = cpad; v.off = 0; v.f32 = prec_tensor_fmt(prec);
    const size_t px = (size_t)n * h * w;
    if (v.f32 == 2) {
        std::vector<_Float16> t(px * cpad * 2, (_Float16)0.f);
        for (size_t p = 0; p < px; ++p)
            for (int k = 0; k < c; ++k) {
                const float sv = src[p * c + k] * 16.0f;
                const _Float16 hi = (_Float16)sv;
                t[p * cpad * 2 + (k / 8) * 16 + (k % 8)] = hi;
                t[p * cpad * 2 + (k / 8) * 16 + 8 + (k % 8)] = (_Float16)(sv - (float)hi);
            }
        v.p = net.upload(t.data(), t.size() * 2);
    } else if (v.f32) {
        std::vector<float> t(px * cpad, 0.f);
        for (size_t p = 0; p < px; ++p) for (int k = 0; k < c; ++k) t[p * cpad + k] = src[p * c + k];
        v.p = net.upload(t.data(), t.size() * 4);
    } else {
        std::vector<_Float16> t(px * cpad, (_Float16)0.f);
        for (size_t p = 0; p < px; ++p) for (int k = 0; k < c; ++k) t[p * cpad + k] = (_Float16)src[p * c + k];
        v.p = net.upload(t.data(), t.size() * 2);
    }
}
static void from_dev(const TView& v, int c, float* dst)
{
    const size_t px = (size_t)v.n * v.h * v.w;
    if (v.f32 == 2) {
        std::vector<_Float16> t(px * v.cs * 2);
        HIP_CHECK(hipMemcpy(t.data(), v.p, t.size() * 2, hipMemcpyDeviceToHost));
        for (size_t p = 0; p < px; ++p)
            for (int k = 0; k < c; ++k) {
                const size_t e = p * v.cs * 2 + (size_t)((v.off + k) / 8) * 16 + (v.off + k) % 8;
                dst[p * c + k] = ((float)t[e] + (float)t[e + 8]) * 0.0625f;
            }
    } else if (v.f32) {
        std::vector<float> t(px * v.cs);
        HIP_CHECK(hipMemcpy(t.data(), v.p, t.size() * 4, hipMemcpyDeviceToHost));
        for (size_t p = 0; p < px; ++p) for (int k = 0; k < c; ++k) dst[p * c + k] = t[p * v.cs + v.off + k];
    } else {
        std::vector<_Float16> t(px * v.cs);
        HIP_CHECK(hipMemcpy(t.data(), v.p, t.size() * 2, hipMemcpyDeviceToHost));
        for (size_t p = 0; p < px; ++p) for (int k = 0; k < c; ++k) dst[p * c + k] = (float)t[p * v.cs + v.off + k];
    }
}

int eagle_op_conv2d(int device, int precision, const float* x, int n, int h, int w, int cin, const float* w_hwio,
                    const float* bias, int cout, int ks, int stride, int pre_act, const float* r1, const float* r2,
                    int post_act, float* y)
{
    EagleHandle* hh = nullptr;
    API_BEGIN
    HIP_CHECK(hipSetDevice(device));
    Net net;
    const int g = precision == EAGLE_PREC_F32 ? 4 : 8;
    const int cin_pad = cin <= g ? g : (cin + 15) / 16 * 16, cout_pad = (cout + 15) / 16 * 16;
    const int ho = (h + 2 * (ks / 2) - ks) / stride + 1, wo = (w + 2 * (ks / 2) - ks) / stride + 1;
    ConvLaunch L;
    to_dev(net, precision, x, n, h, w, cin, cin_pad, L.x);
    L.cfg = conv_choose(precision, ks, stride, cin_pad, cout_pad, wo, pre_act == ACT_NONE && post_act <= ACT_RELU, r1 && r2);
    if (!conv_supported(precision, L.cfg)) fail(EAGLE_E_NOKERNEL, "no kernel instance ks=%d s=%d kc=%d nt=%d", ks, stride, L.cfg.kc, L.cfg.nt);
    std::vector<char> tiled(conv_weight_elems(precision, L.cfg) * (precision == EAGLE_PREC_F32 ? 4 : 2));
    conv_tile_weights(precision, L.cfg, w_hwio, cin, cout, tiled.data(), &L.descale);
    L.w = net.upload(tiled.data(), tiled.size());
    std::vector<float> b(cout_pad, 0.f);
    for (int i = 0; i < cout; ++i) b[i] = bias[i];
    L.bias = (const float*)net.upload(b.data(), b.size() * 4);
    L.y.n = n; L.y.h = ho; L.y.w = wo; L.y.c = cout_pad; L.y.cs = cout_pad; L.y.f32 = prec_tensor_fmt(precision);
    L.y.p = net.get((size_t)n * ho * wo * cout_pad * L.y.esize());
    if (r1) to_dev(net, precision, r1, n, ho, wo, cout, cout_pad, L.r1);
    if (r2) to_dev(net, precision, r2, n, ho, wo, cout, cout_pad, L.r2);
    L.pre_act = pre_act; L.post_act = post_act;
    conv_launch(precision, L, nullptr);
    HIP_CHECK(hipDeviceSynchronize());
    from_dev(L.y, cout, y);
    API_END(hh)
}

int eagle_op_bottleneck(int device, const float* x, int n, int h, int w, int cin, const float* w1, const float* b1, const float* w2, const float* b2,
                        const float* w3, const float* b3, const float* res, float* y, int reps, float* ms, const float* wd, const float* bd)
{
    EagleHandle* hh = nullptr;
    API_BEGIN
    HIP_CHECK(hipSetDevice(device));
    if (!x || !w1 || !b1 || !w2 || !b2 || !w3 || !b3 || !y || n < 1 || h < 1 || w < 1 || cin % 16 || cin < 16) fail(EAGLE_E_INVALID, "eagle_op_bottleneck: bad argument (Cin must be a multiple of 16)");
    if ((wd != nullptr) != (bd != nullptr) || (wd && (res || cin != 64))) fail(EAGLE_E_INVALID, "eagle_op_bottleneck: the in-kernel downsample branch takes (wd, bd) together, Cin = 64 and no residual tensor");
    if (!res && !wd && cin != 256) fail(EAGLE_E_INVALID, "eagle_op_bottleneck: an identity shortcut needs Cin = 256");
    Net net;
    BneckLaunch L;
    to_dev(net, EAGLE_PREC_F32S, x, n, h, w, cin, cin, L.x);
    if (res) to_dev(net, EAGLE_PREC_F32S, res, n, h, w, 256, 256, L.res); else L.res = L.x;
    L.y = L.x; L.y.c = L.y.cs = 256; L.y.off = 0; L.y.p = net.get((size_t)n * h * w * 256 * 4);
    if (wd) L.res = L.y;
    std::vector<_Float16> img;
    bneck_tile_weights(w1, 1, cin, 64, img, &L.ds1); L.w1 = net.upload(img.data(), img.size() * 2);
    bneck_tile_weights(w2, 9, 64, 64, img, &L.ds2); L.w2 = net.upload(img.data(), img.size() * 2);
    std::vector<float> w3x(w3, w3 + 64 * 256), sb3(b3, b3 + 256);
    if (wd) {
        w3x.insert(w3x.end(), wd, wd + 64 * 256);
        for (int o = 0; o < 256; ++o) sb3[o] = sb3[o] + bd[o];
        L.ds_fused = true;
    }
    bneck_tile_weights(w3x.data(), 1, wd ? 128 : 64, 256, img, &L.ds3); L.w3 = net.upload(img.data(), img.size() * 2);
    std::vector<float> sb1(b1, b1 + 64), sb2(b2, b2 + 64);
    bneck_scale_bias(sb1, L.ds1); bneck_scale_bias(sb2, L.ds2); bneck_scale_bias(sb3, L.ds3);
    L.b1 = (const float*)net.upload(sb1.data(), 64 * 4); L.b2 = (const float*)net.upload(sb2.data(), 64 * 4); L.b3 = (const float*)net.upload(sb3.data(), 256 * 4);
    if (getenv("EAGLE_BNECK_TIMING")) L.dbg = (unsigned long long*)net.get(8192 * 8 * 8);
    unsigned* op_sat = nullptr; unsigned* const* op_sat_slot = &op_sat;
    if (getenv("EAGLE_BNECK_OPSAT")) { op_sat = (unsigned*)net.get(sizeof(unsigned) * (size_t)n); L.sat_slot = op_sat_slot; }
    bneck_launch(L, nullptr);
    HIP_CHECK(hipDeviceSynchronize());
    if (L.dbg) {
        std::vector<unsigned long long> t(8192 * 8);
        HIP_CHECK(hipMemcpy(t.data(), L.dbg, t.size() * 8, hipMemcpyDeviceToHost));
        double sum[8] = {0}; int nw = 0;
        for (int b = 0; b < 8192; ++b) { bool any = false; for (int k = 0; k < 8; ++k) { sum[k] += (double)t[b * 8 + k]; any |= t[b * 8 + k] != 0; } nw += any; }
        if (nw) fprintf(stderr, "[bneck timing] %d workgroups, mean us per workgroup: phase1 %.1f  wait %.1f  epi1 %.1f  phase2 %.1f  epi2 %.1f  phase3 %.1f\n", nw,
                        sum[0] / nw / 100, sum[1] / nw / 100, sum[2] / nw / 100, sum[3] / nw / 100, sum[4] / nw / 100, sum[5] / nw / 100);
    }
    if (reps > 0 && ms) {
        hipEvent_t e0, e1;
        HIP_CHECK(hipEventCreate(&e0)); HIP_CHECK(hipEventCreate(&e1));
        HIP_CHECK(hipEventRecord(e0, nullptr));
        for (int i = 0; i < reps; ++i) bneck_launch(L, nullptr);
        HIP_CHECK(hipEventRecord(e1, nullptr));
        HIP_CHECK(hipEventSynchronize(e1));
        HIP_CHECK(hipEventElapsedTime(ms, e0, e1));
        *ms /= (float)reps;
        (void)hipEventDestroy(e0); (void)hipEventDestroy(e1);
    }
    from_dev(L.y, 256, y);
    API_END(hh)
}

int eagle_op_stem(int device, const uint8_t* bgr, int n, int h, int w, int dh, int dw, const float* w1, const float* b1, float* y, uint32_t* sat)
{
    EagleHandle* hh = nullptr;
    API_BEGIN
    HIP_CHECK(hipSetDevice(device));
    if (!bgr || !w1 || !b1 || !y || n < 1 || h < 1 || w < 1 || dh < 1 || dw < 1) fail(EAGLE_E_INVALID, "eagle_op_stem: bad argument");
    if (!stem_supported(EAGLE_PREC_F32S, 3, 2, 3, 64)) fail(EAGLE_E_NOKERNEL, "eagle_op_stem: no kernel");
    Net net;
    StemLaunch L;
    L.bgr = (const uint8_t*)net.upload(bgr, (size_t)n * h * w * 3);
    L.n = n; L.sh = h; L.sw = w; L.dh = dh; L.dw = dw;
    std::vector<_Float16> img;
    stem_tile_weights(w1, img, &L.descale);
    L.w = net.upload(img.data(), img.size() * 2);
    L.bias = (const float*)net.upload(b1, 64 * 4);
    L.y.n = n; L.y.h = (dh - 1) / 2 + 1; L.y.w = (dw - 1) / 2 + 1; L.y.c = L.y.cs = 64; L.y.f32 = 2;
    L.y.p = net.get((size_t)n * L.y.h * L.y.w * 64 * 4);
    unsigned* d_sat = (unsigned*)net.get(sizeof(unsigned) * (size_t)n);
    unsigned* const* slot = &d_sat;
    L.sat_slot = slot;
    stem_launch(L, nullptr);
    HIP_CHECK(hipDeviceSynchronize());
    from_dev(L.y, 64, y);
    if (sat) HIP_CHECK(hipMemcpy(sat, d_sat, sizeof(unsigned) * (size_t)n, hipMemcpyDeviceToHost));
    API_END(hh)
}

int eagle_op_fuse_sum(int device, int precision, const float* base, int n, int H, int W, int c, int n_up,
                      const float* const* ups, const int* up_h, const int* up_w, int relu, float* y)
{
    EagleHandle* hh = nullptr;
    API_BEGIN
    HIP_CHECK(hipSetDevice(device));
    if (n_up > 3 || c % 8) fail(EAGLE_E_INVALID, "fuse_sum: n_up <= 3 and c %% 8 == 0 required");
    Net net;
    TView b, o;
    to_dev(net, precision, base, n, H, W, c, c, b);
    FuseUp u[3];
    for (int i = 0; i < n_up; ++i) to_dev(net, precision, ups[i], n, up_h[i], up_w[i], c, c, u[i].z);
    o = b; o.p = net.get((size_t)n * H * W * c * b.esize());
    fuse_sum_launch(b, u, n_up, relu, o, nullptr);
    HIP_CHECK(hipDeviceSynchronize());
    from_dev(o, c, y);
    API_END(hh)
}

int eagle_op_preprocess(int device, int precision, const uint8_t* bgr, int n, int h, int w, int det_imgsz,
                        float* kp_out, float* det_out, int* det_hw)
{
    return eagle_op_preprocess_lb(device, precision, bgr, n, h, w, det_imgsz, EAGLE_LETTERBOX_RECT, kp_out, det_out, det_hw);
}

int eagle_op_preprocess_lb(int device, int precision, const uint8_t* bgr, int n, int h, int w, int det_imgsz, int letterbox,
                           float* kp_out, float* det_out, int* det_hw)
{
    EagleHandle* hh = nullptr;
    API_BEGIN
    HIP_CHECK(hipSetDevice(device));
    Net net;
    const int cp = precision == EAGLE_PREC_F32 ? 4 : 8;
    const LetterBox lb = letterbox_geometry(h, w, det_imgsz, letterbox);
    det_hw[0] = lb.out_h; det_hw[1] = lb.out_w;
    if (!kp_out || !det_out) return EAGLE_OK;
    uint8_t* d = (uint8_t*)net.upload(bgr, (size_t)n * h * w * 3);
    TView kp, det;
    kp.n = n; kp.h = 540; kp.w = 960; kp.c = kp.cs = cp; kp.f32 = prec_tensor_fmt(precision);
    det = kp; det.h = lb.out_h; det.w = lb.out_w;
    kp.p = net.get((size_t)n * 540 * 960 * cp * kp.esize());
    det.p = net.get((size_t)n * lb.out_h * lb.out_w * cp * det.esize());
    preprocess_launch(precision, d, n, h, w, kp, det, lb, nullptr);
    HIP_CHECK(hipDeviceSynchronize());
    from_dev(kp, 3, kp_out);
    from_dev(det, 3, det_out);
    API_END(hh)
}

int eagle_op_find_homography(int device, const float* img_pts, const float* world_pts, int n, double thresh,
                             int max_iters, int lm_iters, double* H9, uint8_t* mask, int* ok)
{
    EagleHandle* hh = nullptr;
    API_BEGIN
    HIP_CHECK(hipSetDevice(device));
    if (n < 0 || n > EAGLE_MAX_KP) fail(EAGLE_E_INVALID, "0 <= n <= %d required", EAGLE_MAX_KP);
    Net net;
    float* di = (float*)net.upload(img_pts, sizeof(float) * 2 * std::max(n, 1));
    float* dw = (float*)net.upload(world_pts, sizeof(float) * 2 * std::max(n, 1));
    double* dH = (double*)net.get(72);
    uint8_t* dm = (uint8_t*)net.get(256);
    int* dok = (int*)net.get(16);
    homography_only_launch(di, dw, n, thresh, max_iters, lm_iters, dH, dm, dok, nullptr);
    HIP_CHECK(hipDeviceSynchronize());
    HIP_CHECK(hipMemcpy(H9, dH, 72, hipMemcpyDeviceToHost));
    if (n > 0) HIP_CHECK(hipMemcpy(mask, dm, n, hipMemcpyDeviceToHost));
    HIP_CHECK(hipMemcpy(ok, dok, sizeof(int), hipMemcpyDeviceToHost));
// ... 463 lines not shown
```

### eagle_amd/csrc/runtime.h

```cpp
#pragma once
#include <algorithm>
#include <atomic>
#include <chrono>
#include <cmath>
#include <condition_variable>
#include <mutex>
#include <shared_mutex>
#include <thread>
#include <cstdarg>
#include <cstring>
#include <functional>
#include <map>
#include <memory>
#include <string>
#include <vector>
#include <cstddef>
#include "common.h"

namespace eagle {

extern thread_local std::string g_create_error;
extern std::shared_timed_mutex g_capture_mutex;
extern std::mutex g_gate_m;
extern std::condition_variable g_gate_cv;
// ... 106 lines not shown
    }
    void put(void* p) { if (p) free_list[pool].insert({sizes.at(p), p}); }
    void* upload(const void* src, size_t b)
    {
        void* p = nullptr;
        HIP_CHECK(hipMalloc(&p, std::max<size_t>(b, 16)));
        HIP_CHECK(hipMemcpy(p, src, b, hipMemcpyHostToDevice));
        owned.push_back(p); bytes += b;
        return p;
    }
};

}

using namespace eagle;

struct EagleHandle {
    EagleConfig cfg;
    std::string err;
    std::map<std::string, HostTensor> weights;
    bool finalized = false;
    int prec = 0, det_prec = 0;
    hipStream_t s_main = nullptr, s_det = nullptr, s_post = nullptr, s_copy = nullptr;
    hipStream_t s_br[3] = {nullptr, nullptr, nullptr};
    hipEvent_t ev_fork = nullptr, ev_join[3] = {nullptr, nullptr, nullptr};
    bool multi_stream = true;
    hipEvent_t ev_pre = nullptr, ev_det = nullptr, ev_t0 = nullptr, ev_t1 = nullptr;
    struct StepBuf {
        ArgmaxPart* parts = nullptr;
        EagleFrameResult* d_out = nullptr;
        EagleFrameResult* h_out = nullptr;
        unsigned* d_sat = nullptr;
        unsigned* h_sat = nullptr;
        uint8_t* d_frames = nullptr;
        uint8_t* h_frames = nullptr;
        uint8_t* d_yuv = nullptr;
        uint8_t* h_yuv = nullptr;
        bool copy_pending = false;
        hipEvent_t ev_compute = nullptr, ev_done = nullptr, ev_copy = nullptr;
        std::map<int, hipGraphExec_t> graphs;
        int capture_backoff = 0, capture_skip = 0;
    } sb[2];
    bool graph_broken = false;
    int graph_captures = 0, graph_skipped = 0;
    std::unique_ptr<Net> hr, yo, misc, reid;
    TView reid_in; float* reid_feats = nullptr; EagleCrop* reid_crops = nullptr; EagleCrop* reid_crops_h = nullptr; float* reid_feats_h = nullptr;
    eagle::Tracker* tracker = nullptr;
    std::unique_ptr<CopyPool> pool;
    TView kp_in, det_in, logits;
    bool stem_on = false;
    const uint8_t* cur_src = nullptr;
    int cur_n = 0;
    LetterBox lb;
    int hm_chunks = 64;
    ArgmaxPart* cur_parts = nullptr;
    unsigned* cur_sat = nullptr;
    unsigned* clip_sat = nullptr;
    unsigned* clip_sat_h = nullptr;
    long long sat_events = 0; int sat_frames = 0;
    bool fused_argmax = false;
    DetScratch ds;
    DetLevel levels[3];
    PostParams pp;
    bool warmed = false;
    int call_steps = 0;
    bool prof = false;
    std::vector<hipEvent_t> conv_ev;
    struct Span { int k; double bytes; hipEvent_t a, b; };
    std::vector<hipEvent_t> span_pool; size_t span_used = 0;
    std::vector<Span> spans;
    std::vector<EagleKernelTime> ktab;
    std::vector<const Op*> conv_ops;
    EagleTimings timings{};
    double conv_flop_step = 0; int n_conv = 0, n_launch = 0;
    struct Clip {
        bool open = false;
        ClipView cv;
        uint8_t* g[3] = {nullptr, nullptr, nullptr};
        EagleFrameResult* recs = nullptr;
        MemList* mem = nullptr;
        ChainState* st = nullptr;
        ChainState* st_op = nullptr;
        ChainState* h_st = nullptr;
        ChainState* h_zero = nullptr;
        int* h_tail = nullptr;
        MemList* h_mem = nullptr;
        hipEvent_t ev_gray = nullptr, ev_det = nullptr, ev_kp = nullptr, ev_loop = nullptr;
        uint8_t* ecc_small = nullptr;
        int ecc_h = 0, ecc_w = 0;
        int2* ecc_pairs = nullptr; eagle::EccResult* ecc_out = nullptr;
        int ecc_next = -1, ecc_tmpl = -2;
    } clip;
    uint8_t* ecc_prev = nullptr; int ecc_prev_h = 0, ecc_prev_w = 0; bool ecc_has_prev = false;
    void* rccl = nullptr; void* comm = nullptr; int rank = 0, world = 1;
    void* gather_buf = nullptr; size_t gather_cap = 0;
    void* annot_prims = nullptr; size_t annot_prims_cap = 0;
    uint8_t* annot_out = nullptr; size_t annot_out_cap = 0;
    uint8_t* annot_ring = nullptr; size_t annot_ring_cap = 0;
    void* mm_list = nullptr; size_t mm_list_cap = 0;
    void* mm_cols = nullptr; size_t mm_cols_cap = 0;
    void* mm_tr[9] = {}; size_t mm_tr_cap[9] = {};
    uint8_t* mm_mask = nullptr; size_t mm_mask_cap = 0; int mm_mask_scale = 0, mm_mask_margin = -1;
    void* ct_list = nullptr; size_t ct_list_cap = 0;
    void* ct_cols = nullptr; size_t ct_cols_cap = 0;
    void* ct_grid = nullptr; size_t ct_grid_cap = 0;
};

struct EaglePostTable {
    EagleHandle* h = nullptr;
    int rows = 0, cols = 0, flags = 0;
    std::vector<int32_t> frames;
    std::vector<EaglePostColumn> columns;
    std::vector<int32_t> team_ids, team_vals;
    bool has_team = false;
    std::vector<EaglePostMerge> merges;
    double* d_values = nullptr;
    std::vector<double> host;
    bool host_ok = false;
    double* d_vel = nullptr;
    EagleKinematicsParams kin{};
    std::vector<double> host_vel;
    bool host_vel_ok = false;
    bool has_control = false;
    EagleControlParams control{};
    void* d_poss = nullptr;
    bool has_poss = false;
    std::vector<EaglePossessionEvent> events;
    int64_t max_bytes = 0;
    void* d_occ = nullptr;
    int occ_nsel = 0, occ_R = 0;
    bool has_occ = false;
    bool has_trails = false;
    EagleTrailParams trails{};
    std::vector<int32_t> trail_cols;
    void* d_shape = nullptr;
    bool has_shape = false;
    bool has_hulls = false;
    EagleHullParams hulls{};
    void* d_phys = nullptr;
    int phys_persons = 0;
    bool has_phys = false;
    std::vector<EagleLoadTotals> phys_totals;
    std::vector<EagleLoadEffort> phys_efforts;
    void* d_roles = nullptr;
    int roles_members = 0;
    bool has_roles = false;
    void* d_space = nullptr;
    int space_members = 0;
};

namespace eagle {
constexpr int REID_NB = 64;
void finalize(EagleHandle* h);
size_t sat_pad_bytes(int B);
void run_net(EagleHandle* h, Net* net, hipStream_t s, size_t& ev_i);
void check_saturation(EagleHandle* h, const char* what);
void timed_launch(EagleHandle* h, const char* name, double bytes, hipStream_t st, const std::function<void()>& fn);
void collect_spans(EagleHandle* h);
struct HostPlane { int64_t off, pitch, rows, row_bytes, dense_off; };
struct YuvGeom {
    int fmt, h, w, nplanes;
    int64_t frame_stride, y_pitch, c_offset, c_pitch, v_offset;
    int64_t extent;
    int64_t dense_bytes;
    bool dense;
    HostPlane pl[3];
};
YuvGeom yuv_geometry(int fmt, int h, int w, const EagleYuvLayout* L, bool output = false);
bool host_pinned(EagleHandle* h, const void* p);
AnnotArgs annot_args(const YuvGeom& g, const uint8_t* src, uint8_t* dst, const EaglePrim* prims, const int32_t* offs);
void frames_to_host(EagleHandle* h, int n, int fh, int fw, int batch, int out_format, const EagleYuvLayout* out_layout, uint8_t* out,
                    const std::function<void(int, int, const YuvGeom&, uint8_t*)>& draw);
void clip_close(EagleHandle* h);
struct CtCol { int32_t col; int32_t team0; };
struct ControlArgs {
    const double2* values;
    const double2* vel;
    const CtCol* cols;
    float4* lists;
    uint8_t* out;
    unsigned long long* share;
    int rows, row0, n, ncols, stride, R, gw, gh;
    float t_react, v_max, beta;
};
static constexpr int CT_PASS = 65535;
void control_check(const EagleControlParams* p);
void control_columns(const EaglePostColumn* columns, int ncols, const int32_t* team_ids, const int32_t* team_vals, size_t n_team, std::vector<CtCol>& out);
void control_launch(const ControlArgs& a, hipStream_t s);
ControlArgs control_prepare(EagleHandle* h, EaglePostTable* t, const EagleControlParams* p, int max_pass);
void control_rows(EagleHandle* h, const ControlArgs& prepared, int row0, int n, uint8_t* d_out, int64_t* d_share);
struct MmPlan { int S, M, w, h, r, rb, t; };
MmPlan minimap_plan(const EagleMinimapParams* p);
std::vector<uint8_t> markings_mask(const MmPlan& pl, int* pitch);
const uint8_t* minimap_mask(EagleHandle* h, const MmPlan& pl);
struct ShapeCols { std::vector<int32_t> gcols; int n0 = 0, n1 = 0; };
ShapeCols shape_columns(const char* who, const EaglePostColumn* columns, int ncols, const int32_t* team_ids, const int32_t* team_vals, size_t n_team);
void hull_check(const char* who, const EagleHullParams* p);
void shape_run(EagleHandle* h, const ShapeCols& sc, const double2* d_values, int rows, EagleTeamShape* d_shapes, int32_t* d_hull, hipStream_t s);
void shape_edges_launch(const double2* values, int rows, const EagleTeamShape* shapes, const int32_t* hull, int row0, int n, int scale, int margin, int4* edges, hipStream_t s);
}

#define API_BEGIN try { eagle::ApiGuard api_guard_;
#define API_BEGIN_H(h) if (!(h)) return EAGLE_E_INVALID; API_BEGIN
#define API_END(h)                                                       \
    }                                                                    \
    catch (const eagle::Err& e) { if (h) (h)->err = e.msg; else eagle::g_create_error = e.msg; return e.code; } \
    catch (const std::exception& e) { if (h) (h)->err = e.what(); else eagle::g_create_error = e.what(); return EAGLE_E_INVALID; } \
    return EAGLE_OK;
```

### eagle_amd/lib.py

```python
import ctypes as C
import os

import numpy as np

_HERE = os.path.dirname(os.path.abspath(__file__))
LIB_PATH = os.environ.get("EAGLE_HIP_LIB") or os.path.join(_HERE, "libeagle_hip.so")

MAX_DET, N_LANDMARKS, MAX_KP = 300, 57, 87
PREC_F16, PREC_F32, PREC_F32S = 0, 1, 2
PRECISIONS = {"f16": PREC_F16, "f32": PREC_F32, "f32s": PREC_F32S}
DET_VARIANTS = {"n": 0, "s": 1, "m": 2, "l": 3, "x": 4}
AUTO, SMALL_BATCH = -1, 32
LETTERBOX = {"rect": 0, "square": 1}
DET_PREC_AUTO = -1
DET_PREC_MIXED = 4


class EagleError(RuntimeError):
    pass


class EagleRangeError(EagleError):
    records = None

# ... 85 lines not shown
                               ("opp_rows", "<i4"), ("within_rows", "<i4"), ("reserved", "<i4")])
assert C.sizeof(EagleSpaceParams) == 32 and (SPACE_ROW_DTYPE.itemsize, SPACE_SITE_DTYPE.itemsize, SPACE_TOTALS_DTYPE.itemsize) == (64, 48, 64)


class EagleShotParams(C.Structure):
    _fields_ = [("cut", C.c_int32), ("low", C.c_int32), ("grass_thr", C.c_int32), ("window", C.c_int32), ("min_len", C.c_int32), ("reserved", C.c_int32 * 3)]


SHOT_SIGNATURE = 1537
SHOT_START, SHOT_AFTER_CUT, SHOT_AFTER_TRANSITION, SHOT_TRANSITION = 0, 1, 2, 3
SHOT_KIND_NAMES = ("start", "after_cut", "after_transition", "transition")
SHOT_FRAME_FLASH, SHOT_FRAME_HARD, SHOT_FRAME_GRADUAL_END, SHOT_FRAME_IN_TRANSITION = 1, 2, 4, 8
SHOT_PITCH, SHOT_SHORT, SHOT_USABLE = 1, 2, 4
SHOT_FRAME_DTYPE = np.dtype([("d1", "<i4"), ("d2", "<i4"), ("dW", "<i4"), ("sg", "<i4"), ("st", "<i4"), ("grass", "<u4"), ("flags", "<i4"), ("reserved", "<i4")])
SHOT_DTYPE = np.dtype([("first", "<i4"), ("count", "<i4"), ("kind", "<i4"), ("flags", "<i4"), ("grass_sum", "<i8"), ("reserved", "<i4", 2)])
assert C.sizeof(EagleShotParams) == 32 and (SHOT_FRAME_DTYPE.itemsize, SHOT_DTYPE.itemsize) == (32, 32)


class EagleTopviewParams(C.Structure):
    _fields_ = [("scale", C.c_int32), ("margin", C.c_int32), ("background", C.c_uint32), ("markings", C.c_int32), ("marking_colour", C.c_uint32),
                ("mask_boxes", C.c_int32), ("box_pad", C.c_double), ("first", C.c_int32), ("step", C.c_int32), ("min_count", C.c_int32), ("reserved", C.c_int32 * 3)]


TOPVIEW_VIDEO, TOPVIEW_MOSAIC, TOPVIEW_RESIDUAL = 1, 2, 4
TOPVIEW_MAX_FRAMES = 1 << 23
assert C.sizeof(EagleTopviewParams) == 56


class EagleKinematicsParams(C.Structure):
    _fields_ = [("fps", C.c_int32), ("max_gap", C.c_int32), ("speed_cap", C.c_double), ("reserved", C.c_int64)]


class EagleControlParams(C.Structure):
    _fields_ = [("cells_per_metre", C.c_int32), ("t_react", C.c_float), ("v_max", C.c_float), ("beta", C.c_float), ("reserved", C.c_int32 * 4)]


class EaglePossessionParams(C.Structure):
    _fields_ = [("fps", C.c_int32), ("min_hold", C.c_int32), ("max_gap", C.c_int32), ("reserved0", C.c_int32), ("radius", C.c_double), ("reserved", C.c_int64)]


class EagleLoadParams(C.Structure):
    _fields_ = [("fps", C.c_int32), ("max_gap", C.c_int32), ("min_frames", C.c_int32 * 2), ("zone_edges", C.c_double * 4), ("effort_speed", C.c_double * 2),
                ("accel", C.c_double), ("reserved", C.c_int64 * 2)]


LOAD_HSR, LOAD_SPRINT, LOAD_ACCEL, LOAD_DECEL, LOAD_ABSENT, LOAD_Q = 0, 1, 2, 3, 255, 1 << 20
LOAD_TOTALS_DTYPE = np.dtype([("zone_frames", "<i8", 5), ("zone_dist_q", "<i8", 5), ("top_speed", "<f8"), ("col", "<i4"), ("rows_present", "<i4"),
                              ("efforts", "<i4", 4), ("reserved", "<i4", 4)])
LOAD_EFFORT_DTYPE = np.dtype([("col", "<i4"), ("kind", "<i4"), ("first_row", "<i4"), ("last_row", "<i4"), ("frames", "<i4"), ("reserved0", "<i4"),
                              ("distance_q", "<i8"), ("peak_speed", "<f8"), ("peak_accel", "<f8")])
assert C.sizeof(EagleLoadParams) == 88 and LOAD_TOTALS_DTYPE.itemsize == 128 and LOAD_EFFORT_DTYPE.itemsize == 48


class EaglePassOptionParams(C.Structure):
    _fields_ = [("cells_per_metre", C.c_int32), ("samples", C.c_int32), ("t_react", C.c_float), ("v_max", C.c_float), ("beta", C.c_float), ("v_ball", C.c_float),
                ("reserved", C.c_int32 * 2)]


PASS_ACTIVE, PASS_NO_OWNER, PASS_IN_FLIGHT, PASS_NO_TEAM, PASS_OFF_DOMAIN = 0, 1, 2, 3, 4
PASS_STATUS_NAMES = ("active", "no_owner", "in_flight", "no_team", "off_domain")
PASS_MAX_SITES = 1024
PASS_ROW_DTYPE = np.dtype([("status", "<i4"), ("owner_col", "<i4"), ("group", "<i4"), ("n_mates", "<i4"), ("n_defenders", "<i4"), ("best_col", "<i4"),
                           ("best_byte", "<i4"), ("reserved", "<i4"), ("sum", "<i8")])
assert C.sizeof(EaglePassOptionParams) == 32 and PASS_ROW_DTYPE.itemsize == 40


class EagleOccupancyParams(C.Structure):
    _fields_ = [("fps", C.c_int32), ("max_gap", C.c_int32), ("cells_per_metre", C.c_int32), ("reserved0", C.c_int32), ("sigma", C.c_double), ("reserved", C.c_int64)]


POST_PLAYER, POST_GOALKEEPER, POST_BALL, POST_BOUNDARY = 0, 1, 2, 3
POST_NO_BALL = 1
POSTCOL_DTYPE = np.dtype([("kind", "<i4"), ("id", "<i4"), ("video", "<i4"), ("reserved", "<i4")])
POSTMERGE_DTYPE = np.dtype([("kind", "<i4"), ("from_id", "<i4"), ("to_id", "<i4"), ("head_id", "<i4"), ("gap_frames", "<i4"), ("team", "<i4"),
                            ("dist", "<f8")])
EVENT_PASS, EVENT_TURNOVER, EVENT_UNKNOWN = 0, 1, 2
EVENT_DTYPE = np.dtype([("row", "<i4"), ("from_col", "<i4"), ("to_col", "<i4"), ("release_row", "<i4"), ("receive_row", "<i4"), ("kind", "<i4"),
                        ("reserved", "<i4", 2), ("x0", "<f8"), ("y0", "<f8"), ("x1", "<f8"), ("y1", "<f8"), ("length", "<f8"),
                        ("duration", "<f8")])
E_INVALID = -1


class EagleKernelTime(C.Structure):
    _fields_ = [("name", C.c_char * 40), ("ms", C.c_float), ("launches", C.c_int32), ("bytes", C.c_double), ("flop", C.c_double)]


DET_DTYPE = np.dtype([("x1", "<f4"), ("y1", "<f4"), ("x2", "<f4"), ("y2", "<f4"), ("conf", "<f4"), ("cls", "<i4"),
                      ("id", "<i4"), ("bx1", "<i4"), ("by1", "<i4"), ("bx2", "<i4"), ("by2", "<i4"),
                      ("foot_x", "<i4"), ("foot_y", "<i4"), ("pitch_xf", "<f4"), ("pitch_yf", "<f4"),
                      ("pitch_x", "<i4"), ("pitch_y", "<i4"), ("reported", "u1"), ("in_bounds", "u1"), ("pad", "u1", 2)],
                     align=True)
KP_DTYPE = np.dtype([("label", "<i4"), ("x", "<i4"), ("y", "<i4"), ("score", "<f4"), ("synthesized", "u1"),
                     ("on_plane", "u1"), ("inlier", "u1"), ("pad", "u1")], align=True)
RESULT_DTYPE = np.dtype([("n_det", "<i4"), ("n_kp", "<i4"), ("n_candidates", "<i4"), ("H_valid", "u1"),
                         ("bounds_valid", "u1"), ("pad", "u1", 2), ("H", "<f8", 9), ("bounds", "<f8", 4),
                         ("hm_idx", "<i4", N_LANDMARKS), ("hm_score", "<f4", N_LANDMARKS),
                         ("kp", KP_DTYPE, MAX_KP), ("det", DET_DTYPE, MAX_DET)], align=True)

_lib = None


def require_torch_first():
    import sys
    if "torch" not in sys.modules and _lib is not None:
        raise EagleError("torch must be imported before eagle_amd.lib loads libeagle_hip.so in a process that uses both "
                         "(two ROCm runtimes would be mapped: torch's bundled one and /opt/rocm's); import torch first, or keep the process torch-free")


def load():
    global _lib
    if _lib is not None:
        return _lib
    if not os.path.exists(LIB_PATH):
        raise EagleError(f"{LIB_PATH} not found: run `python -c 'import __graft_entry__ as g; g.build()'` "
                         "(there is no CPU fallback for the product path)")
    L = C.CDLL(LIB_PATH)
    vp, i32, i64 = C.c_void_p, C.c_int, C.c_int64
    fp, dp, u8p = C.POINTER(C.c_float), C.POINTER(C.c_double), C.POINTER(C.c_uint8)
    L.eagle_abi_sizes.argtypes = [C.POINTER(C.c_int32)]
    L.eagle_default_config.argtypes = [C.POINTER(EagleConfig)]
    L.eagle_create.argtypes = [C.POINTER(EagleConfig), C.POINTER(vp)]
    L.eagle_destroy.argtypes = [vp]
    L.eagle_destroy.restype = None
    L.eagle_last_error.argtypes = [vp]
    L.eagle_last_error.restype = C.c_char_p
    L.eagle_get_config.argtypes = [vp, C.POINTER(EagleConfig)]
    L.eagle_resolve_config.argtypes = [C.POINTER(EagleConfig)]
    L.eagle_load_weights.argtypes = [vp, C.c_char_p, fp, C.POINTER(i64), i32]
    L.eagle_finalize_weights.argtypes = [vp]
    L.eagle_process_frames.argtypes = [vp, u8p, i32, i64, i64, vp]
    L.eagle_process_device_frames.argtypes = [vp, vp, i32, vp]
    L.eagle_host_alloc.argtypes = [vp, i64, C.POINTER(vp)]
    L.eagle_host_free.argtypes = [vp, vp]
    L.eagle_device_alloc.argtypes = [vp, i64, C.POINTER(vp)]
    L.eagle_device_free.argtypes = [vp, vp]
    L.eagle_device_upload.argtypes = [vp, vp, vp, i64]
    L.eagle_reproject.argtypes = [vp, vp, i32, dp, u8p]
    L.eagle_clip_open.argtypes = [vp, vp, i32]
    L.eagle_clip_close.argtypes = [vp]
    L.eagle_clip_detect_keypoints.argtypes = [vp, i32, i32, i32]
    L.eagle_clip_get_keypoints.argtypes = [vp, i32, vp, C.POINTER(i32)]
    L.eagle_clip_set_keypoints.argtypes = [vp, i32, vp, i32]
    L.eagle_clip_flow.argtypes = [vp, i32, i32, i32, vp, i32, vp, C.POINTER(i32), fp, u8p]
    L.eagle_clip_run.argtypes = [vp, i32, i32, i32, i32, i32, i32, C.POINTER(i32)]
    L.eagle_clip_detect_objects.argtypes = [vp, i32, i32]
    L.eagle_clip_fetch.argtypes = [vp, vp]
    L.eagle_comm_id.argtypes = [vp]
    L.eagle_comm_init.argtypes = [vp, i32, i32, vp]
    L.eagle_gather.argtypes = [vp, vp, i32, vp]
    L.eagle_set_profiling.argtypes = [vp, i32]
    L.eagle_get_timings.argtypes = [vp, C.POINTER(EagleTimings)]
    L.eagle_get_kernel_times.argtypes = [vp, C.POINTER(EagleKernelTime), i32, C.POINTER(i32)]
    L.eagle_op_conv2d.argtypes = [i32, i32, fp, i32, i32, i32, i32, fp, fp, i32, i32, i32, i32, fp, fp, i32, fp]
    L.eagle_op_bottleneck.argtypes = [i32, fp, i32, i32, i32, i32, fp, fp, fp, fp, fp, fp, fp, fp, i32, fp, fp, fp]
    L.eagle_op_stem.argtypes = [i32, u8p, i32, i32, i32, i32, i32, fp, fp, fp, C.POINTER(C.c_uint32)]
    L.eagle_op_fuse_sum.argtypes = [i32, i32, fp, i32, i32, i32, i32, i32, C.POINTER(fp), C.POINTER(i32), C.POINTER(i32), i32, fp]
    L.eagle_op_preprocess.argtypes = [i32, i32, u8p, i32, i32, i32, i32, fp, fp, C.POINTER(i32)]
    L.eagle_op_preprocess_lb.argtypes = [i32, i32, u8p, i32, i32, i32, i32, i32, fp, fp, C.POINTER(i32)]
    L.eagle_op_find_homography.argtypes = [i32, fp, fp, i32, C.c_double, i32, i32, dp, u8p, C.POINTER(i32)]
    L.eagle_op_detect_tail.argtypes = [i32, i32, C.POINTER(i32), C.POINTER(i32), fp, C.POINTER(fp), C.POINTER(fp), i32, i32, C.c_float, C.c_float, C.c_double,
                                       i32, i32, i32, i32, vp, fp, fp, C.POINTER(C.c_int32)]
    L.eagle_op_post.argtypes = [i32, i32, i32, i32, i32, fp, vp, vp, vp, i32, i32, C.c_double, C.c_double, i32, i32]
    L.eagle_op_conv2d_argmax.argtypes = [i32, i32, fp, i32, i32, i32, i32, fp, fp, i32, i32, i32, fp, vp, C.POINTER(i32), C.POINTER(i32), C.POINTER(i32)]
    L.eagle_debug.argtypes = [C.c_char_p, i64, vp, i64]
    L.eagle_team_colors.argtypes = [vp, vp, i32, vp, i32, vp]
    L.eagle_track_open.argtypes = [vp, C.POINTER(EagleTrackParams)]
    L.eagle_track_frames.argtypes = [vp, vp, i32]
    L.eagle_track_frames_cmc.argtypes = [vp, vp, i32, C.POINTER(C.c_double)]
    L.eagle_clip_motion.argtypes = [vp, i32, i32, C.POINTER(C.c_double)]
    L.eagle_clip_motion_ecc.argtypes = [vp, i32, i32, i32, C.POINTER(C.c_double), C.POINTER(i32)]
    L.eagle_reid_features.argtypes = [vp, vp, i32, vp, i32, fp]
    yl = C.POINTER(EagleYuvLayout)
    L.eagle_process_frames_yuv.argtypes = [vp, i32, u8p, i32, yl, vp]
    L.eagle_process_device_frames_yuv.argtypes = [vp, i32, vp, i32, yl, vp]
    L.eagle_yuv_to_bgr.argtypes = [vp, i32, vp, i32, yl, vp]
    L.eagle_op_yuv_to_bgr.argtypes = [i32, i32, u8p, i32, i32, i32, yl, u8p]
    L.eagle_track_frames_reid.argtypes = [vp, vp, i32, C.POINTER(C.c_double), fp, C.POINTER(i32), C.POINTER(i32)]
    L.eagle_annotate_device_frames.argtypes = [vp, vp, i32, vp, vp, vp, i32, i32, yl, vp]
    L.eagle_annotate_frames.argtypes = [vp, vp, i32, vp, vp, vp, i32, i32, yl, vp]
    L.eagle_overlay_from_record.argtypes = [vp, vp, vp, i32, vp, i32, C.POINTER(i32)]
    L.eagle_op_annotate.argtypes = [i32, u8p, i32, i32, i32, vp, vp, i32, yl, u8p]
    L.eagle_annotate_frames_prims.argtypes = [vp, vp, i32, vp, vp, i32, yl, vp]
    L.eagle_postprocess.argtypes = [vp, vp, i32, C.POINTER(EaglePostParams), C.POINTER(vp)]
    L.eagle_post_free.argtypes = [vp]
    L.eagle_post_free.restype = None
    L.eagle_post_shape.argtypes = [vp, C.POINTER(C.c_int32), C.POINTER(C.c_int32), C.POINTER(C.c_int32)]
    L.eagle_post_layout.argtypes = [vp, vp, vp]
    L.eagle_post_values.argtypes = [vp, vp]
    L.eagle_post_device_values.argtypes = [vp, C.POINTER(vp)]
    L.eagle_post_merges.argtypes = [vp, vp, i32, C.POINTER(C.c_int)]
    L.eagle_overlay_from_table.argtypes = [vp, i32, vp, vp, i32, C.POINTER(i32)]
    mp = C.POINTER(EagleMinimapParams)
    L.eagle_minimap_size.argtypes = [mp, C.POINTER(i32), C.POINTER(i32)]
    L.eagle_minimap_device_frames.argtypes = [vp, vp, i32, i32, mp, i32, yl, vp]
    L.eagle_minimap_frames.argtypes = [vp, vp, i32, i32, mp, i32, yl, vp]
    L.eagle_op_minimap.argtypes = [i32, vp, vp, i32, i32, vp, vp, i32, mp, i32, i32, i32, yl, vp]
    kp, cp = C.POINTER(EagleKinematicsParams), C.POINTER(EagleControlParams)
    L.eagle_post_velocities.argtypes = [vp, vp, kp]
    L.eagle_post_velocity_values.argtypes = [vp, vp]
    L.eagle_post_device_velocity_values.argtypes = [vp, C.POINTER(vp)]
    L.eagle_control_size.argtypes = [cp, C.POINTER(i32), C.POINTER(i32)]
    L.eagle_control_device_grids.argtypes = [vp, vp, i32, i32, cp, vp, vp]
    L.eagle_control_grids.argtypes = [vp, vp, i32, i32, cp, vp, vp]
    L.eagle_minimap_set_control.argtypes = [vp, cp]
    L.eagle_op_velocities.argtypes = [i32, vp, vp, i32, i32, kp, vp]
    L.eagle_op_control.argtypes = [i32, vp, vp, vp, i32, i32, vp, vp, i32, cp, i32, i32, vp, vp]
    L.eagle_op_minimap_control.argtypes = [i32, vp, vp, vp, i32, i32, vp, vp, i32, mp, cp, i32, i32, i32, yl, vp]
    pp = C.POINTER(EaglePossessionParams)
    L.eagle_post_possession.argtypes = [vp, vp, pp]
    L.eagle_post_possession_values.argtypes = [vp, vp, vp, vp]
    L.eagle_post_device_possession.argtypes = [vp, C.POINTER(vp)]
    L.eagle_post_events.argtypes = [vp, vp, i32, C.POINTER(C.c_int)]
    L.eagle_op_possession.argtypes = [i32, vp, vp, vp, i32, i32, vp, vp, i32, pp, vp, vp, vp, vp, i32, C.POINTER(C.c_int)]
    po = C.POINTER(EaglePassOptionParams)
    L.eagle_pass_options_size.argtypes = [po, C.POINTER(C.c_int), C.POINTER(C.c_int)]
    L.eagle_pass_options_layout.argtypes = [vp, vp, i32, C.POINTER(C.c_int)]
    L.eagle_pass_options_device.argtypes = [vp, vp, i32, i32, po, vp, vp, vp]
    L.eagle_pass_options.argtypes = [vp, vp, i32, i32, po, vp, vp, vp]
    L.eagle_op_pass_options.argtypes = [i32, vp, vp, vp, i32, i32, vp, vp, i32, vp, vp, po, i32, i32, vp, vp, vp]
    op = C.POINTER(EagleOccupancyParams)
    L.eagle_occupancy_size.argtypes = [op, C.POINTER(C.c_int), C.POINTER(C.c_int)]
    L.eagle_post_occupancy.argtypes = [vp, vp, op, vp, vp, i32]
    L.eagle_post_occupancy_values.argtypes = [vp, vp, vp, vp, vp, vp]
    L.eagle_post_device_occupancy.argtypes = [vp, C.POINTER(vp), C.POINTER(vp)]
    L.eagle_occupancy_picture.argtypes = [vp, vp, i32, i32, i32, C.c_uint32, vp]
    L.eagle_op_occupancy.argtypes = [i32, vp, vp, vp, i32, i32, op, vp, vp, i32, vp, vp, vp, vp, vp]
    L.eagle_op_occupancy_picture.argtypes = [i32, vp, i32, i32, i32, C.c_uint32, vp]
    tp = C.POINTER(EagleTrailParams)
    L.eagle_minimap_set_trails.argtypes = [vp, tp, vp, i32]
    L.eagle_trajectory_picture.argtypes = [vp, vp, vp, i32, i32, i32, i32, i32, i32, i32, vp]
    L.eagle_pass_picture.argtypes = [vp, vp, i32, i32, i32, i32, vp]
    L.eagle_op_minimap_trails.argtypes = [i32, vp, vp, vp, i32, i32, vp, vp, i32, mp, tp, vp, i32, vp, vp, i32, i32, i32, i32, yl, vp]
    L.eagle_op_trajectory_picture.argtypes = [i32, vp, vp, vp, i32, i32, vp, vp, i32, vp, i32, i32, i32, i32, i32, i32, i32, vp]
    L.eagle_op_pass_picture.argtypes = [i32, vp, vp, i32, i32, vp, vp, i32, vp, i32, i32, i32, i32, i32, vp]
    hp = C.POINTER(EagleHullParams)
    L.eagle_post_team_shape.argtypes = [vp, vp]
    L.eagle_post_team_shape_values.argtypes = [vp, vp, vp]
    L.eagle_post_device_team_shape.argtypes = [vp, C.POINTER(vp), C.POINTER(vp)]
    L.eagle_minimap_set_hulls.argtypes = [vp, hp]
    L.eagle_op_team_shape.argtypes = [i32, vp, vp, i32, i32, vp, vp, i32, vp, vp]
    L.eagle_op_minimap_hulls.argtypes = [i32, vp, vp, vp, i32, i32, vp, vp, i32, mp, hp, tp, vp, i32, vp, vp, i32, i32, i32, i32, yl, vp]
    rp = C.POINTER(EagleRoleParams)
    L.eagle_post_roles.argtypes = [vp, vp, rp]
    L.eagle_post_roles_values.argtypes = [vp, vp, vp, vp]
    L.eagle_post_device_roles.argtypes = [vp, C.POINTER(vp), C.POINTER(vp), C.POINTER(vp), C.POINTER(C.c_int)]
    L.eagle_op_roles.argtypes = [i32, vp, vp, i32, i32, vp, vp, i32, rp, vp, vp, vp]
    sp = C.POINTER(EagleSpaceParams)
    L.eagle_post_space.argtypes = [vp, vp, sp]
    L.eagle_post_space_values.argtypes = [vp, vp, vp, vp]
    L.eagle_post_device_space.argtypes = [vp, C.POINTER(vp), C.POINTER(vp), C.POINTER(vp), C.POINTER(C.c_int)]
    L.eagle_space_device_grids.argtypes = [vp, vp, i32, i32, sp, vp]
    L.eagle_space_grids.argtypes = [vp, vp, i32, i32, sp, vp]
    L.eagle_op_space.argtypes = [i32, vp, vp, i32, i32, vp, vp, i32, sp, i32, i32, vp, vp, vp, vp]
    shp = C.POINTER(EagleShotParams)
    L.eagle_shots_device_frames.argtypes = [vp, vp, i32, shp, vp, vp, i32, C.POINTER(C.c_int)]
    L.eagle_shots_frames.argtypes = [vp, vp, i32, i64, i64, i64, shp, vp, vp, i32, C.POINTER(C.c_int)]
    L.eagle_op_shots.argtypes = [i32, vp, i32, i32, i32, shp, vp, vp, i32, C.POINTER(C.c_int), vp]
    tvp, lay = C.POINTER(EagleTopviewParams), C.POINTER(EagleYuvLayout)
    L.eagle_topview_size.argtypes = [tvp, C.POINTER(C.c_int), C.POINTER(C.c_int)]
    L.eagle_topview_device_frames.argtypes = [vp, vp, i32, vp, vp, tvp, i32, lay, vp]
    L.eagle_topview_frames.argtypes = [vp, vp, i32, vp, vp, tvp, i32, lay, vp]
    L.eagle_topview_mosaic_device.argtypes = [vp, vp, i32, vp, vp, vp, tvp, vp, i32]
    L.eagle_topview_mosaic_finish.argtypes = [vp, vp, tvp, vp, vp]
    L.eagle_topview_residual_device.argtypes = [vp, vp, i32, vp, vp, vp, tvp, vp, vp, vp, vp]
    L.eagle_topview_mosaic_frames.argtypes = [vp, vp, i32, i64, vp, vp, vp, tvp, vp, i32]
    L.eagle_topview_residual_frames.argtypes = [vp, vp, i32, i64, vp, vp, vp, tvp, vp, vp, vp, vp]
    L.eagle_op_topview.argtypes = [i32, vp, i32, i32, i32, vp, vp, vp, vp, tvp, i32, i32, lay, vp, vp, vp, vp, vp, vp]
    lp = C.POINTER(EagleLoadParams)
    L.eagle_post_physical.argtypes = [vp, vp, lp]
    L.eagle_post_physical_values.argtypes = [vp, vp, vp, vp]
    L.eagle_post_physical_totals.argtypes = [vp, vp, i32, C.POINTER(C.c_int)]
    L.eagle_post_physical_efforts.argtypes = [vp, vp, i32, C.POINTER(C.c_int)]
    L.eagle_post_device_physical.argtypes = [vp, C.POINTER(vp), C.POINTER(vp)]
    L.eagle_op_physical.argtypes = [i32, vp, vp, vp, i32, i32, lp, vp, vp, vp, vp, i32, C.POINTER(C.c_int), vp, i32, C.POINTER(C.c_int)]
    L.eagle_op_reid_crop.argtypes = [i32, u8p, i32, i32, i32, vp, i32, i32, i32, i32, i32, fp]
    L.eagle_op_reid_conv7.argtypes = [i32, fp, i32, i32, i32, i32, i32, fp, fp, i32, i32, fp]
    L.eagle_op_reid_maxpool3s2.argtypes = [i32, fp, i32, i32, i32, i32, i32, i32, i32, i32, fp]
    L.eagle_op_reid_avgpool2.argtypes = [i32, fp, i32, i32, i32, i32, i32, i32, i32, i32, fp]
    L.eagle_op_reid_dw3.argtypes = [i32, fp, i32, i32, i32, i32, i32, i32, fp, fp, i32, i32, fp]
    L.eagle_op_reid_gate.argtypes = [i32, C.POINTER(fp), i32, i32, i32, i32, i32, i32, fp, fp, fp, fp, i32, i32, i32, i32, fp, fp]
    L.eagle_op_reid_head.argtypes = [i32, fp, i32, i32, i32, i32, i32, i32, fp, fp, i32, fp]
    L.eagle_op_conv2d_sliced.argtypes = [i32, i32, fp, i32, i32, i32, i32, i32, i32, fp, fp, i32, i32, i32, i32, fp, i32, i32, i32, fp, i32, i32, i32, i32, i32, i32, fp]
    L.eagle_op_maxpool5.argtypes = [i32, i32, fp, i32, i32, i32, i32, i32, i32, i32, i32, i32, fp]
    L.eagle_op_upsample2.argtypes = [i32, i32, fp, i32, i32, i32, i32, i32, i32, i32, i32, i32, i32, i32, fp]
    L.eagle_op_split_to_f32.argtypes = [i32, fp, i32, i32, i32, i32, i32, i32, i32, i32, fp]
    L.eagle_op_gray_pyramid.argtypes = [i32, u8p, i32, i32, i32, u8p, u8p, u8p, C.POINTER(i32)]
    L.eagle_op_flow.argtypes = [i32, u8p, i32, i32, i32, i32, i32, i32, vp, i32, vp, C.POINTER(i32), fp, u8p]
    _lib = L
    return L


EXPORTS = ["eagle_abi_sizes", "eagle_default_config", "eagle_create", "eagle_destroy", "eagle_last_error", "eagle_get_config", "eagle_resolve_config", "eagle_load_weights",
           "eagle_finalize_weights", "eagle_process_frames", "eagle_process_device_frames", "eagle_device_alloc",
           "eagle_device_free", "eagle_device_upload", "eagle_host_alloc", "eagle_host_free", "eagle_reproject", "eagle_comm_id", "eagle_comm_init", "eagle_gather",
           "eagle_set_profiling", "eagle_get_timings", "eagle_get_kernel_times", "eagle_op_conv2d", "eagle_op_bottleneck", "eagle_op_stem", "eagle_op_fuse_sum", "eagle_op_preprocess", "eagle_op_preprocess_lb",
           "eagle_op_find_homography", "eagle_op_detect_tail", "eagle_op_post", "eagle_op_conv2d_argmax", "eagle_clip_open", "eagle_clip_close", "eagle_clip_detect_objects", "eagle_clip_detect_keypoints", "eagle_clip_get_keypoints",
           "eagle_clip_set_keypoints", "eagle_clip_flow", "eagle_clip_run", "eagle_clip_fetch", "eagle_debug", "eagle_track_open", "eagle_track_frames", "eagle_track_frames_cmc", "eagle_clip_motion_ecc", "eagle_clip_motion", "eagle_team_colors",
           "eagle_reid_features", "eagle_track_frames_reid", "eagle_process_frames_yuv", "eagle_process_device_frames_yuv", "eagle_yuv_to_bgr",
           "eagle_op_yuv_to_bgr", "eagle_annotate_device_frames", "eagle_annotate_frames", "eagle_overlay_from_record", "eagle_op_annotate",
           "eagle_annotate_frames_prims", "eagle_postprocess", "eagle_post_free", "eagle_post_shape", "eagle_post_layout", "eagle_post_values",
           "eagle_post_device_values", "eagle_post_merges", "eagle_overlay_from_table", "eagle_minimap_size", "eagle_minimap_device_frames", "eagle_minimap_frames",
           "eagle_op_minimap", "eagle_post_velocities", "eagle_post_velocity_values", "eagle_post_device_velocity_values", "eagle_control_size",
           "eagle_control_device_grids", "eagle_control_grids", "eagle_minimap_set_control", "eagle_op_velocities", "eagle_op_control",
           "eagle_op_minimap_control", "eagle_post_possession", "eagle_post_possession_values", "eagle_post_device_possession", "eagle_post_events",
           "eagle_op_possession", "eagle_pass_options_size", "eagle_pass_options_layout", "eagle_pass_options_device", "eagle_pass_options",
           "eagle_op_pass_options", "eagle_occupancy_size", "eagle_post_occupancy", "eagle_post_occupancy_values", "eagle_post_device_occupancy",
           "eagle_occupancy_picture", "eagle_op_occupancy", "eagle_op_occupancy_picture", "eagle_minimap_set_trails", "eagle_trajectory_picture",
           "eagle_pass_picture", "eagle_op_minimap_trails", "eagle_op_trajectory_picture", "eagle_op_pass_picture", "eagle_post_team_shape", "eagle_post_team_shape_values",
           "eagle_post_device_team_shape", "eagle_minimap_set_hulls", "eagle_op_team_shape", "eagle_op_minimap_hulls", "eagle_post_physical", "eagle_post_physical_values",
           "eagle_post_physical_totals", "eagle_post_physical_efforts", "eagle_post_device_physical", "eagle_op_physical", "eagle_post_roles",
           "eagle_post_roles_values", "eagle_post_device_roles", "eagle_op_roles", "eagle_post_space", "eagle_post_space_values", "eagle_post_device_space",
           "eagle_space_device_grids", "eagle_space_grids", "eagle_op_space", "eagle_shots_device_frames", "eagle_shots_frames", "eagle_op_shots", "eagle_topview_size", "eagle_topview_device_frames", "eagle_topview_frames",
           "eagle_topview_mosaic_device", "eagle_topview_mosaic_finish", "eagle_topview_residual_device", "eagle_topview_mosaic_frames", "eagle_topview_residual_frames",
           "eagle_op_topview", "eagle_op_reid_crop", "eagle_op_reid_conv7", "eagle_op_reid_maxpool3s2", "eagle_op_reid_avgpool2", "eagle_op_reid_dw3",
           "eagle_op_reid_gate", "eagle_op_reid_head", "eagle_op_conv2d_sliced", "eagle_op_maxpool5", "eagle_op_upsample2", "eagle_op_split_to_f32", "eagle_op_gray_pyramid",
           "eagle_op_flow"]

FLOWKP_DTYPE = np.dtype([("label", "<i4"), ("x", "<i4"), ("y", "<i4"), ("score", "<f4")], align=True)
E_REFERENCE_RAISES = -7
E_RANGE = -8


def debug(key, value=0, out=None):
    rc = load().eagle_debug(key.encode(), int(value), None if out is None else out.ctypes.data_as(C.c_void_p), 0 if out is None else out.nbytes)
    if rc:
        raise EagleError(f"eagle_debug({key}) failed ({rc})")
    return out


def resolve_config(cfg):
    out = EagleConfig.from_buffer_copy(cfg)
    rc = load().eagle_resolve_config(C.byref(out))
    if rc:
        raise EagleError(f"eagle_resolve_config failed ({rc}): {load().eagle_last_error(None).decode()}")
    return out


def abi_sizes():
    o = (C.c_int32 * 4)()
    load().eagle_abi_sizes(o)
    return list(o)


def _fp(a):
    return a.ctypes.data_as(C.POINTER(C.c_float)) if a is not None else None


def default_config(**kw):
    cfg = EagleConfig()
    load().eagle_default_config(C.byref(cfg))
    for k, v in kw.items():
        if k == "det_variant" and isinstance(v, str):
            v = DET_VARIANTS[v]
        if k == "letterbox" and isinstance(v, str):
            v = LETTERBOX[v]
        if not hasattr(cfg, k):
            raise TypeError(f"unknown config field {k}")
        setattr(cfg, k, v)
    return cfg


class Handle:

    def __init__(self, cfg=None, **kw):
        self.L = load()
        self.cfg = cfg or default_config(**kw)
        self._h = C.c_void_p()
        rc = self.L.eagle_create(C.byref(self.cfg), C.byref(self._h))
        if rc:
            raise EagleError(f"eagle_create failed ({rc}): {self.L.eagle_last_error(None).decode()}")
        resolved = EagleConfig()
        self._check(self.L.eagle_get_config(self._h, C.byref(resolved)), "get_config")
        self.cfg = resolved

    def _check(self, rc, what):
        if rc == E_RANGE:
            raise EagleRangeError(f"{what}: {self.L.eagle_last_error(self._h).decode()}")
        if rc:
            raise EagleError(f"{what} failed ({rc}): {self.L.eagle_last_error(self._h).decode()}")

    def _check_records(self, rc, what, out):
        try:
            self._check(rc, what)
        except EagleRangeError as e:
            e.records = out
            raise

    def close(self):
        if self._h:
            self.L.eagle_destroy(self._h)
            self._h = C.c_void_p()

    def __del__(self):
        try:
            self.close()
        except Exception:
            pass

    def load_weight(self, name, arr):
        arr = np.ascontiguousarray(arr, np.float32)
        shape = (C.c_int64 * max(arr.ndim, 1))(*arr.shape)
        self._check(self.L.eagle_load_weights(self._h, name.encode(), _fp(arr), shape, arr.ndim), f"load_weights({name})")

    def finalize_weights(self):
        self._check(self.L.eagle_finalize_weights(self._h), "finalize_weights")

    def process(self, frames, out=None, strides=None):
        frames = np.asarray(frames)
        if frames.dtype != np.uint8:
            frames = frames.astype(np.uint8)
        if frames.ndim == 3:
            frames = frames[None]
        n, h, w, c = frames.shape
        if (h, w, c) != (self.cfg.frame_h, self.cfg.frame_w, 3):
            raise EagleError(f"frame shape {(h, w, c)} does not match the handle ({self.cfg.frame_h}, {self.cfg.frame_w}, 3)")
        fs, rs, ps, cs = frames.strides
        if n == 1:
            fs = max(fs, rs * (h - 1) + 3 * w)
        if not (cs == 1 and ps == 3 and rs >= 3 * w and fs >= rs * (h - 1) + 3 * w):
            frames = np.ascontiguousarray(frames)
            fs, rs = h * w * 3, w * 3
        if strides is not None:
            fs, rs = strides
        if out is None:
            out = np.zeros(n, RESULT_DTYPE)
        assert out.dtype == RESULT_DTYPE and len(out) >= n and out.flags.c_contiguous
        self._check_records(self.L.eagle_process_frames(self._h, C.cast(frames.ctypes.data, C.POINTER(C.c_uint8)), n, int(fs), int(rs),
                                                        out.ctypes.data_as(C.c_void_p)), "process_frames", out)
        return out

    def host_frames(self, n):
        shape = (n, self.cfg.frame_h, self.cfg.frame_w, 3)
        nbytes = int(np.prod(shape))
        p = C.c_void_p()
        self._check(self.L.eagle_host_alloc(self._h, nbytes, C.byref(p)), "host_alloc")
        buf = (C.c_uint8 * max(nbytes, 1)).from_address(p.value)
        a = np.frombuffer(buf, np.uint8, nbytes).reshape(shape)
        self._pinned = getattr(self, "_pinned", {})
        self._pinned[a.ctypes.data] = p
        return a

    def host_buffer(self, nbytes):
        p = C.c_void_p()
        self._check(self.L.eagle_host_alloc(self._h, int(nbytes), C.byref(p)), "host_alloc")
        a = np.frombuffer((C.c_uint8 * max(int(nbytes), 1)).from_address(p.value), np.uint8, int(nbytes))
        self._pinned = getattr(self, "_pinned", {})
        self._pinned[a.ctypes.data] = p
        return a

    def host_free(self, a):
        p = self._pinned.pop(a.ctypes.data)
        self._check(self.L.eagle_host_free(self._h, p), "host_free")

    def upload(self, frames):
        frames = np.ascontiguousarray(frames, np.uint8)
        d = C.c_void_p()
        self._check(self.L.eagle_device_alloc(self._h, frames.nbytes, C.byref(d)), "device_alloc")
        self._check(self.L.eagle_device_upload(self._h, d, frames.ctypes.data_as(C.c_void_p), frames.nbytes), "device_upload")
        return d

    def free(self, d):
        self._check(self.L.eagle_device_free(self._h, d), "device_free")

    def process_device(self, dptr, n, out=None):
        if out is None:
            out = np.zeros(n, RESULT_DTYPE)
        self._check_records(self.L.eagle_process_device_frames(self._h, dptr, n, out.ctypes.data_as(C.c_void_p)), "process_device_frames", out)
        return out

# ... 478 lines not shown

    def team_colors(self, dptr, n_frames, crops):
        crops = np.ascontiguousarray(crops, np.int32).reshape(-1, 5)
        out = np.zeros((len(crops), 12), np.int32)
        self._check(self.L.eagle_team_colors(self._h, dptr, n_frames, crops.ctypes.data_as(C.c_void_p), len(crops), out.ctypes.data_as(C.c_void_p)), "team_colors")
        return out

    def track_open(self, **params):
        p = None
        if params:
            d = dict(track_high_thresh=0.5, track_low_thresh=0.1, new_track_thresh=0.6, match_thresh=0.8, track_buffer=30, frame_rate=30)
            d.update(params)
            p = C.byref(EagleTrackParams(**d))
        self._check(self.L.eagle_track_open(self._h, p), "track_open")

    def reid_features(self, dptr, n_frames, crops):
        crops = np.ascontiguousarray(crops, np.int32).reshape(-1, 5)
        out = np.zeros((len(crops), 512), np.float32)
        self._check(self.L.eagle_reid_features(self._h, dptr, n_frames, crops.ctypes.data_as(C.c_void_p), len(crops), out.ctypes.data_as(C.POINTER(C.c_float))), "reid_features")
        return out

    def track_frames_reid(self, recs, feats, feat_det, feat_count, warps=None):
        assert recs.dtype == RESULT_DTYPE and recs.flags.c_contiguous
        feats = np.ascontiguousarray(feats, np.float32).reshape(-1, 512)
        feat_det = np.ascontiguousarray(feat_det, np.int32); feat_count = np.ascontiguousarray(feat_count, np.int32)
        assert len(feat_count) == len(recs) and int(feat_count.sum()) == len(feats) == len(feat_det)
        w = None if warps is None else np.ascontiguousarray(warps, np.float64).reshape(len(recs), 6)
        self._check(self.L.eagle_track_frames_reid(self._h, recs.ctypes.data_as(C.c_void_p), len(recs), None if w is None else w.ctypes.data_as(C.POINTER(C.c_double)),
                                                   feats.ctypes.data_as(C.POINTER(C.c_float)), feat_det.ctypes.data_as(C.POINTER(C.c_int32)),
                                                   feat_count.ctypes.data_as(C.POINTER(C.c_int32))), "track_frames_reid")
        return recs

    def track_frames(self, recs, warps=None):
        assert recs.dtype == RESULT_DTYPE and recs.flags.c_contiguous
        w = None
        if warps is not None:
            w = np.ascontiguousarray(warps, np.float64).reshape(len(recs), 6)
        self._check(self.L.eagle_track_frames_cmc(self._h, recs.ctypes.data_as(C.c_void_p), len(recs),
                                                  w.ctypes.data_as(C.POINTER(C.c_double)) if w is not None else None), "track_frames")
        return recs

    def clip_motion(self, first, count):
        w = np.zeros((max(count, 0), 6), np.float64)
        self._check(self.L.eagle_clip_motion(self._h, first, count, w.ctypes.data_as(C.POINTER(C.c_double))), "clip_motion")
        return w

    def clip_motion_ecc(self, first, count, carry=False, return_ok=False):
        w = np.zeros((max(count, 0), 6), np.float64)
        ok = np.zeros(max(count, 0), np.int32)
        self._check(self.L.eagle_clip_motion_ecc(self._h, first, count, int(bool(carry)), w.ctypes.data_as(C.POINTER(C.c_double)),
                                                 ok.ctypes.data_as(C.POINTER(C.c_int32))), "clip_motion_ecc")
        return (w, ok) if return_ok else w

    def set_profiling(self, on):
        self._check(self.L.eagle_set_profiling(self._h, int(on)), "set_profiling")

    def timings(self):
        t = EagleTimings()
        self._check(self.L.eagle_get_timings(self._h, C.byref(t)), "get_timings")
        return t

    def kernel_times(self):
        buf = (EagleKernelTime * 256)(); n = C.c_int(0)
        self._check(self.L.eagle_get_kernel_times(self._h, buf, 256, C.byref(n)), "get_kernel_times")
        return [(buf[i].name.decode(), float(buf[i].ms), int(buf[i].launches), float(buf[i].bytes), float(buf[i].flop)) for i in range(min(n.value, 256))]

    def comm_init(self, rank, world, uid_bytes):
        buf = C.create_string_buffer(bytes(uid_bytes), 128)
        self._check(self.L.eagle_comm_init(self._h, rank, world, buf), "comm_init")

    def gather(self, local, world, out=None):
        local = np.ascontiguousarray(local)
        if out is None:
            out = np.zeros(len(local) * world, RESULT_DTYPE)
        assert out.dtype == RESULT_DTYPE and len(out) == len(local) * world and out.flags.c_contiguous
        self._check(self.L.eagle_gather(self._h, local.ctypes.data_as(C.c_void_p), len(local), out.ctypes.data_as(C.c_void_p)), "gather")
        return out


BOUNDARY_NAMES = ("Bottom_Left", "Top_Left", "Top_Right", "Bottom_Right")


class PostTable:

    def __init__(self, handle, ptr, team_mapping=None):
        self.handle, self._t, self.team_mapping = handle, ptr, team_mapping
        L = handle.L
        r, c, f = C.c_int32(), C.c_int32(), C.c_int32()
        L.eagle_post_shape(ptr, C.byref(r), C.byref(c), C.byref(f))
        self.flags = f.value
        self.rows = np.zeros(r.value, np.int32)
        self.columns = np.zeros(c.value, POSTCOL_DTYPE)
        L.eagle_post_layout(ptr, self.rows.ctypes.data_as(C.c_void_p), self.columns.ctypes.data_as(C.c_void_p))
        self.names = [BOUNDARY_NAMES[int(k["id"])] if k["kind"] == POST_BOUNDARY else
                      ("Ball" if k["kind"] == POST_BALL else f"{'Player' if k['kind'] == POST_PLAYER else 'Goalkeeper'}_{int(k['id'])}") + ("_video" if k["video"] else "")
                      for k in self.columns]
        self._values = None
        n = C.c_int(0)
        L.eagle_post_merges(ptr, None, 0, C.byref(n))
        m = np.zeros(n.value, POSTMERGE_DTYPE)
        L.eagle_post_merges(ptr, m.ctypes.data_as(C.c_void_p), n.value, C.byref(n))
        self.merges = [{k: (float(e[k]) if k == "dist" else int(e[k])) for k in POSTMERGE_DTYPE.names} for e in m]
        if self.merges and team_mapping is not None:
            self.team_mapping = dict(team_mapping)
            heads = {(e["kind"], e["head_id"]): e["team"] for e in self.merges if e["team"] >= 0}
            for k in self.columns:
                if k["video"] and (int(k["kind"]), int(k["id"])) in heads and self.team_mapping.get(int(k["id"]), -1) < 0:
                    self.team_mapping[int(k["id"])] = heads[(int(k["kind"]), int(k["id"]))]

    @property
    def values(self):
        if self._values is None:
            v = np.zeros((len(self.columns), len(self.rows), 2), np.float64)
            self.handle._check(self.handle.L.eagle_post_values(self._t, v.ctypes.data_as(C.c_void_p)), "post_values")
            self._values = v
        return self._values

    @property
    def device_values(self):
        d = C.c_void_p()
        self.handle._check(self.handle.L.eagle_post_device_values(self._t, C.byref(d)), "post_device_values")
        return d.value

    def overlay(self, row, rec=None):
        cap = 2 * len(self.columns) + MAX_PRIMS
        out = np.zeros(cap, PRIM_DTYPE); n = C.c_int(0)
        rec = None if rec is None else np.ascontiguousarray(rec, RESULT_DTYPE).reshape(-1)[:1]
        self.handle._check(self.handle.L.eagle_overlay_from_table(self._t, int(row), None if rec is None else rec.ctypes.data_as(C.c_void_p),
                                                                  out.ctypes.data_as(C.c_void_p), cap, C.byref(n)), "overlay_from_table")
        return out[: n.value].copy()

    def close(self):
        if self._t:
            _ = self.values
            self.handle.L.eagle_post_free(self._t)
            self._t = C.c_void_p()

    def __del__(self):
        try:
            if self._t and self.handle._h:
                self.handle.L.eagle_post_free(self._t)
        except Exception:
            pass


def comm_unique_id():
    buf = C.create_string_buffer(128)
    rc = load().eagle_comm_id(buf)
    if rc:
        raise EagleError(f"eagle_comm_id failed ({rc}): {load().eagle_last_error(None).decode()}")
    return buf.raw


def op_conv2d(x, w_hwio, bias, stride=1, pre=0, r1=None, r2=None, post=0, precision=PREC_F32, device=0):
    L = load()
    x = np.ascontiguousarray(x, np.float32); w = np.ascontiguousarray(w_hwio, np.float32); b = np.ascontiguousarray(bias, np.float32)
    n, h, wd, cin = x.shape
    ks, _, _, cout = w.shape
    ho = (h + 2 * (ks // 2) - ks) // stride + 1
    wo = (wd + 2 * (ks // 2) - ks) // stride + 1
    y = np.empty((n, ho, wo, cout), np.float32)
    r1 = None if r1 is None else np.ascontiguousarray(r1, np.float32)
    r2 = None if r2 is None else np.ascontiguousarray(r2, np.float32)
    rc = L.eagle_op_conv2d(device, precision, _fp(x), n, h, wd, cin, _fp(w), _fp(b), cout, ks, stride, pre, _fp(r1), _fp(r2), post, _fp(y))
    if rc:
        raise EagleError(f"eagle_op_conv2d failed ({rc}): {L.eagle_last_error(None).decode()}")
    return y


def op_bottleneck(x, w1, b1, w2, b2, w3, b3, res=None, reps=0, device=0, wd=None, bd=None):
    L = load()
    x = np.ascontiguousarray(x, np.float32)
    n, h, w, cin = x.shape
    arrs = [np.ascontiguousarray(a, np.float32) for a in (w1, b1, w2, b2, w3, b3)]
    assert arrs[0].shape == (1, 1, cin, 64) and arrs[2].shape == (3, 3, 64, 64) and arrs[4].shape == (1, 1, 64, 256), "HWIO weights of a 64-wide Bottleneck"
    res = None if res is None else np.ascontiguousarray(res, np.float32)
    y = np.empty((n, h, w, 256), np.float32)
    ms = C.c_float(0)
    wd = None if wd is None else np.ascontiguousarray(wd, np.float32)
    bd = None if bd is None else np.ascontiguousarray(bd, np.float32)
    rc = L.eagle_op_bottleneck(device, _fp(x), n, h, w, cin, *[_fp(a) for a in arrs], _fp(res), _fp(y), int(reps), C.byref(ms), _fp(wd), _fp(bd))
    if rc:
        raise EagleError(f"eagle_op_bottleneck failed ({rc}): {L.eagle_last_error(None).decode()}")
    return (y, ms.value) if reps > 0 else y


def op_stem(frames, w1, b1, out_hw=(540, 960), device=0):
    L = load()
    frames = np.ascontiguousarray(frames, np.uint8)
    n, h, w, _ = frames.shape
    w1 = np.ascontiguousarray(w1, np.float32); b1 = np.ascontiguousarray(b1, np.float32)
    assert w1.shape == (3, 3, 3, 64) and b1.shape == (64,), "HWIO weights of HRNet's conv1"
    dh, dw = out_hw
    y = np.empty((n, (dh - 1) // 2 + 1, (dw - 1) // 2 + 1, 64), np.float32)
    sat = np.zeros(n, np.uint32)
    rc = L.eagle_op_stem(device, frames.ctypes.data_as(C.POINTER(C.c_uint8)), n, h, w, dh, dw, _fp(w1), _fp(b1), _fp(y), sat.ctypes.data_as(C.POINTER(C.c_uint32)))
    if rc:
        raise EagleError(f"eagle_op_stem failed ({rc}): {L.eagle_last_error(None).decode()}")
    return y, sat


def op_fuse_sum(base, ups, relu=True, precision=PREC_F32, device=0):
    L = load()
    base = np.ascontiguousarray(base, np.float32)
    n, H, W, c = base.shape
    ups = [np.ascontiguousarray(u, np.float32) for u in ups]
    arr = (C.POINTER(C.c_float) * max(len(ups), 1))(*[_fp(u) for u in ups])
    uh = (C.c_int * max(len(ups), 1))(*[u.shape[1] for u in ups])
    uw = (C.c_int * max(len(ups), 1))(*[u.shape[2] for u in ups])
    y = np.empty_like(base)
    rc = L.eagle_op_fuse_sum(device, precision, _fp(base), n, H, W, c, len(ups), arr, uh, uw, int(relu), _fp(y))
    if rc:
        raise EagleError(f"eagle_op_fuse_sum failed ({rc}): {L.eagle_last_error(None).decode()}")
    return y


def op_preprocess(frames, det_imgsz=640, precision=PREC_F32, device=0, letterbox=0):
    L = load()
    frames = np.ascontiguousarray(frames, np.uint8)
    n, h, w, _ = frames.shape
    hw = (C.c_int * 2)()
    rc = L.eagle_op_preprocess_lb(device, precision, frames.ctypes.data_as(C.POINTER(C.c_uint8)), n, h, w, det_imgsz, int(letterbox), None, None, hw)
    if rc:
        raise EagleError(f"eagle_op_preprocess failed ({rc}): {L.eagle_last_error(None).decode()}")
    kp = np.empty((n, 540, 960, 3), np.float32)
    det = np.empty((n, hw[0], hw[1], 3), np.float32)
    rc = L.eagle_op_preprocess_lb(device, precision, frames.ctypes.data_as(C.POINTER(C.c_uint8)), n, h, w, det_imgsz, int(letterbox), _fp(kp), _fp(det), hw)
    if rc:
        raise EagleError(f"eagle_op_preprocess failed ({rc}): {L.eagle_last_error(None).decode()}")
    return kp, det


def op_find_homography(img_pts, world_pts, thresh=5.0, max_iters=2000, lm_iters=10, device=0):
    L = load()
    a = np.ascontiguousarray(img_pts, np.float32).reshape(-1, 2)
    b = np.ascontiguousarray(world_pts, np.float32).reshape(-1, 2)
    n = len(a)
    H = np.zeros(9, np.float64); mask = np.zeros(max(n, 1), np.uint8); ok = C.c_int(0)
    rc = L.eagle_op_find_homography(device, _fp(a), _fp(b), n, thresh, max_iters, lm_iters,
                                    H.ctypes.data_as(C.POINTER(C.c_double)), mask.ctypes.data_as(C.POINTER(C.c_uint8)), C.byref(ok))
    if rc:
        raise EagleError(f"eagle_op_find_homography failed ({rc}): {L.eagle_last_error(None).decode()}")
    return (H.reshape(3, 3), mask[:n]) if ok.value else (None, None)


PART_DTYPE = np.dtype([("score", "<f4"), ("idx", "<i4")], align=True)


def op_detect_tail(levels, nc, in_hw, frame_hw, conf_floor=0.15, nms_iou=0.7, detector_conf=0.35, device=0):
    L = load()
    nl = len(levels)
    box = [np.ascontiguousarray(b, np.float32) for b, _, _ in levels]
    cls = [np.ascontiguousarray(c, np.float32) for _, c, _ in levels]
    n = box[0].shape[0]
    for b, c in zip(box, cls):
        assert b.ndim == 4 and b.shape[0] == n and b.shape[3] == 64 and c.shape == b.shape[:3] + (nc,), (b.shape, c.shape)
    gh = (C.c_int * nl)(*[b.shape[1] for b in box]); gw = (C.c_int * nl)(*[b.shape[2] for b in box])
    st = (C.c_float * nl)(*[float(s) for _, _, s in levels])
    bp = (C.POINTER(C.c_float) * nl)(*[_fp(b) for b in box]); cp = (C.POINTER(C.c_float) * nl)(*[_fp(c) for c in cls])
    A = sum(b.shape[1] * b.shape[2] for b in box)
    out = np.zeros(n, RESULT_DTYPE)
    boxes = np.zeros((n, A, 4), np.float32); conf = np.zeros((n, A), np.float32); cl = np.zeros((n, A), np.int32)
    rc = L.eagle_op_detect_tail(device, nl, gh, gw, st, bp, cp, n, nc, conf_floor, nms_iou, detector_conf, frame_hw[0], frame_hw[1], in_hw[0], in_hw[1],
                                out.ctypes.data_as(C.c_void_p), _fp(boxes), _fp(conf), cl.ctypes.data_as(C.POINTER(C.c_int32)))
    if rc:
        raise EagleError(f"eagle_op_detect_tail failed ({rc}): {L.eagle_last_error(None).decode()}")
    return out, boxes, conf, cl


def op_post(hm_hw, frame_hw, logits=None, chunks=64, parts=None, recs=None, keypoint_conf=0.3, ransac_thresh=5.0, ransac_max_iters=2000, lm_iters=10, device=0):
    L = load()
    if logits is not None:
        logits = np.ascontiguousarray(logits, np.float32)
        n = logits.shape[0]
        assert logits.shape == (n, hm_hw[0], hm_hw[1], 64), logits.shape
    else:
        parts = np.ascontiguousarray(parts, PART_DTYPE)
        n, chunks = parts.shape[0], parts.shape[1]
        assert parts.shape == (n, chunks, 64), parts.shape
    out = np.zeros(n, RESULT_DTYPE) if recs is None else np.ascontiguousarray(recs, RESULT_DTYPE).copy()
    assert len(out) == n
    pout = np.zeros((n, chunks, 64), PART_DTYPE)
    rc = L.eagle_op_post(device, n, hm_hw[0], hm_hw[1], chunks, _fp(logits), None if parts is None else parts.ctypes.data_as(C.c_void_p),
                         pout.ctypes.data_as(C.c_void_p), out.ctypes.data_as(C.c_void_p), frame_hw[0], frame_hw[1], keypoint_conf, ransac_thresh, ransac_max_iters, lm_iters)
    if rc:
        raise EagleError(f"eagle_op_post failed ({rc}): {L.eagle_last_error(None).decode()}")
    return out, pout


def conv2d_argmax_tiles(hw, cin, cout, ks=1, stride=1, precision=PREC_F32S):
    L = load()
    tiles, th, tw = C.c_int(0), C.c_int(0), C.c_int(0)
    rc = L.eagle_op_conv2d_argmax(0, precision, None, 1, hw[0], hw[1], cin, None, None, cout, ks, stride, None, None, C.byref(tiles), C.byref(th), C.byref(tw))
    if rc:
        raise EagleError(f"eagle_op_conv2d_argmax failed ({rc}): {L.eagle_last_error(None).decode()}")
    return tiles.value, th.value, tw.value


def op_conv2d_argmax(x, w_hwio, bias, stride=1, precision=PREC_F32S, device=0):
    L = load()
    x = np.ascontiguousarray(x, np.float32); w = np.ascontiguousarray(w_hwio, np.float32); b = np.ascontiguousarray(bias, np.float32)
    n, h, wd, cin = x.shape
    ks, _, _, cout = w.shape
    ho = (h + 2 * (ks // 2) - ks) // stride + 1
    wo = (wd + 2 * (ks // 2) - ks) // stride + 1
    tiles, th, tw = C.c_int(0), C.c_int(0), C.c_int(0)
    args = (device, precision, _fp(x), n, h, wd, cin, _fp(w), _fp(b), cout, ks, stride)
    rc = L.eagle_op_conv2d_argmax(*args, None, None, C.byref(tiles), C.byref(th), C.byref(tw))
    if rc:
        raise EagleError(f"eagle_op_conv2d_argmax failed ({rc}): {L.eagle_last_error(None).decode()}")
    y = np.empty((n, ho, wo, cout), np.float32)
    parts = np.zeros((n, tiles.value, (cout + 15) // 16 * 16), PART_DTYPE)
    rc = L.eagle_op_conv2d_argmax(*args, _fp(y), parts.ctypes.data_as(C.c_void_p), C.byref(tiles), C.byref(th), C.byref(tw))
    if rc:
        raise EagleError(f"eagle_op_conv2d_argmax failed ({rc}): {L.eagle_last_error(None).decode()}")
    return y, parts, (th.value, tw.value)


def _pix(fmt):
    if isinstance(fmt, str):
# ... 824 lines not shown
```

### include/eagle.h

```cpp
#ifndef EAGLE_H
#define EAGLE_H
#include <stdint.h>

#ifdef __cplusplus
extern "C" {
#endif

#define EAGLE_OK 0
#define EAGLE_E_INVALID (-1)
#define EAGLE_E_HIP (-2)
#define EAGLE_E_STATE (-3)
#define EAGLE_E_MISSING (-4)
#define EAGLE_E_NOKERNEL (-5)
#define EAGLE_E_COMM (-6)
#define EAGLE_E_RANGE (-8)

#define EAGLE_MAX_DET 300
#define EAGLE_N_LANDMARKS 57
#define EAGLE_MAX_KP 87

#define EAGLE_PREC_F16 0
#define EAGLE_PREC_F32 1
#define EAGLE_PREC_F32S 2

// ... 436 lines not shown
int eagle_post_device_space(const EaglePostTable* t, const EagleSpaceRow** d_rows, const EagleSpaceSite** d_sites, const EagleSpaceTotals** d_totals, int* n_members);
int eagle_space_device_grids(EagleHandle* h, EaglePostTable* t, int row0, int n, const EagleSpaceParams* p, uint8_t* d_grid);
int eagle_space_grids(EagleHandle* h, EaglePostTable* t, int row0, int n, const EagleSpaceParams* p, uint8_t* grid);
int eagle_op_space(int device, const double* values, const EaglePostColumn* columns, int rows, int cols, const int32_t* team_ids, const int32_t* team_vals, int n_team,
                   const EagleSpaceParams* p, int row0, int n, EagleSpaceRow* rows_out, EagleSpaceSite* sites_out, EagleSpaceTotals* totals_out, uint8_t* grid);

#define EAGLE_SHOT_SIGNATURE 1537
#define EAGLE_SHOT_START 0
#define EAGLE_SHOT_AFTER_CUT 1
#define EAGLE_SHOT_AFTER_TRANSITION 2
#define EAGLE_SHOT_TRANSITION 3
#define EAGLE_SHOT_FRAME_FLASH 1
#define EAGLE_SHOT_FRAME_HARD 2
#define EAGLE_SHOT_FRAME_GRADUAL_END 4
#define EAGLE_SHOT_FRAME_IN_TRANSITION 8
#define EAGLE_SHOT_PITCH 1
#define EAGLE_SHOT_SHORT 2
#define EAGLE_SHOT_USABLE 4
typedef struct EagleShotParams {
    int32_t cut;
    int32_t low;
    int32_t grass_thr;
    int32_t window;
    int32_t min_len;
    int32_t reserved[3];
} EagleShotParams;
typedef struct EagleShotFrame {
    int32_t d1, d2, dW;
    int32_t sg, st;
    uint32_t grass;
    int32_t flags;
    int32_t reserved;
} EagleShotFrame;
typedef struct EagleShot {
    int32_t first, count;
    int32_t kind;
    int32_t flags;
    int64_t grass_sum;
    int32_t reserved[2];
} EagleShot;
int eagle_shots_device_frames(EagleHandle* h, const uint8_t* d_bgr, int n, const EagleShotParams* p, EagleShotFrame* frames_out, EagleShot* shots_out, int cap, int* n_shots);
int eagle_shots_frames(EagleHandle* h, const uint8_t* bgr, int n, int64_t row_stride, int64_t frame_stride, int64_t max_staging_bytes, const EagleShotParams* p,
                       EagleShotFrame* frames_out, EagleShot* shots_out, int cap, int* n_shots);
int eagle_op_shots(int device, const uint8_t* bgr, int n, int h, int w, const EagleShotParams* p, EagleShotFrame* frames_out, EagleShot* shots_out, int cap, int* n_shots,
                   uint32_t* signatures_out);

#define EAGLE_TOPVIEW_MAX_FRAMES (1 << 23)
#define EAGLE_TOPVIEW_VIDEO 1
#define EAGLE_TOPVIEW_MOSAIC 2
#define EAGLE_TOPVIEW_RESIDUAL 4
typedef struct EagleTopviewParams {
    int32_t scale, margin;
    uint32_t background;
    int32_t markings;
    uint32_t marking_colour;
    int32_t mask_boxes;
    double box_pad;
    int32_t first, step;
    int32_t min_count;
    int32_t reserved[3];
} EagleTopviewParams;
int eagle_topview_size(const EagleTopviewParams* p, int* w, int* h);
int eagle_topview_device_frames(EagleHandle* h, const uint8_t* d_bgr, int n, const double* Hs, const uint8_t* valid, const EagleTopviewParams* p, int out_format,
                                const EagleYuvLayout* out_layout, void* d_out);
int eagle_topview_frames(EagleHandle* h, const uint8_t* bgr, int n, const double* Hs, const uint8_t* valid, const EagleTopviewParams* p, int out_format,
                         const EagleYuvLayout* out_layout, uint8_t* out);
int eagle_topview_mosaic_device(EagleHandle* h, const uint8_t* d_bgr, int n, const double* Hs, const uint8_t* valid, const EagleFrameResult* recs,
                                const EagleTopviewParams* p, uint32_t* d_acc, int reset);
int eagle_topview_mosaic_finish(EagleHandle* h, const uint32_t* d_acc, const EagleTopviewParams* p, uint8_t* bgr_out, uint32_t* cnt_out);
int eagle_topview_residual_device(EagleHandle* h, const uint8_t* d_bgr, int n, const double* Hs, const uint8_t* valid, const EagleFrameResult* recs,
                                  const EagleTopviewParams* p, const uint32_t* d_acc, uint64_t* res_sum, uint32_t* res_cnt, uint32_t* covered);
int eagle_topview_mosaic_frames(EagleHandle* h, const uint8_t* bgr, int n, int64_t max_staging_bytes, const double* Hs, const uint8_t* valid, const EagleFrameResult* recs,
                                const EagleTopviewParams* p, uint32_t* d_acc, int reset);
int eagle_topview_residual_frames(EagleHandle* h, const uint8_t* bgr, int n, int64_t max_staging_bytes, const double* Hs, const uint8_t* valid, const EagleFrameResult* recs,
                                  const EagleTopviewParams* p, const uint32_t* d_acc, uint64_t* res_sum, uint32_t* res_cnt, uint32_t* covered);
int eagle_op_topview(int device, const uint8_t* bgr, int n, int h, int w, const double* Hs, const uint8_t* valid, const float* boxes, const int32_t* box_off,
                     const EagleTopviewParams* p, int mode, int out_format, const EagleYuvLayout* out_layout, uint8_t* out, uint8_t* mosaic_out, uint32_t* cnt_out,
                     uint64_t* res_sum, uint32_t* res_cnt, uint32_t* covered);

typedef struct EagleOccupancyParams {
    int32_t fps;
    int32_t max_gap;
    int32_t cells_per_metre;
    int32_t reserved0;
    double sigma;
    int64_t reserved;
} EagleOccupancyParams;
int eagle_occupancy_size(const EagleOccupancyParams* p, int* gw, int* gh);
int eagle_post_occupancy(EagleHandle* h, EaglePostTable* t, const EagleOccupancyParams* p, const int32_t* sel_off, const int32_t* sel_cols, int n_sel);
int eagle_post_occupancy_values(EaglePostTable* t, float* grids, uint8_t* bytes, int64_t* total, int64_t* outside, int32_t* counts);
int eagle_post_device_occupancy(const EaglePostTable* t, const float** d_grids, const uint8_t** d_bytes);
int eagle_occupancy_picture(EagleHandle* h, EaglePostTable* t, int sel, int scale, int margin, uint32_t bgr_colour, uint8_t* out);
int eagle_op_occupancy(int device, const double* values, const int32_t* frames, const EaglePostColumn* columns, int rows, int cols, const EagleOccupancyParams* p,
                       const int32_t* sel_off, const int32_t* sel_cols, int n_sel, float* grids, uint8_t* bytes, int64_t* total, int64_t* outside, int32_t* counts);
int eagle_op_occupancy_picture(int device, const uint8_t* bytes_grid, int cells_per_metre, int scale, int margin, uint32_t bgr_colour, uint8_t* out);

int eagle_reproject(EagleHandle* h, EagleFrameResult* recs, int n, const double* Hs, const uint8_t* flags);

typedef struct EagleFlowKp { int32_t label; int32_t x, y; float score; } EagleFlowKp;
int eagle_clip_open(EagleHandle* h, const void* d_bgr, int n);
int eagle_clip_detect_objects(EagleHandle* h, int first, int count);
int eagle_clip_detect_keypoints(EagleHandle* h, int first, int stride, int count);
int eagle_clip_get_keypoints(EagleHandle* h, int frame, EagleFlowKp* out , int* n );
int eagle_clip_set_keypoints(EagleHandle* h, int frame, const EagleFlowKp* in, int n);
int eagle_clip_flow(EagleHandle* h, int src_frame, int dst_frame, int hue_frame, const EagleFlowKp* in, int n_in,
                    EagleFlowKp* out , int* n_out, float* next_pts , uint8_t* status );
int eagle_clip_run(EagleHandle* h, int first, int last, int keypoint_interval, int homography_interval, int calibration, int wait,
                   int* stalled_at);
int eagle_clip_fetch(EagleHandle* h, EagleFrameResult* out);
int eagle_clip_close(EagleHandle* h);
#define EAGLE_E_REFERENCE_RAISES (-7)

typedef struct EagleCrop { int32_t frame, x1, y1, x2, y2; } EagleCrop;
typedef struct EagleTrackParams {
    float track_high_thresh, track_low_thresh, new_track_thresh, match_thresh;
    int32_t track_buffer, frame_rate;
} EagleTrackParams;
int eagle_track_open(EagleHandle* h, const EagleTrackParams* params );
int eagle_track_frames(EagleHandle* h, EagleFrameResult* recs, int n);
int eagle_clip_motion(EagleHandle* h, int first, int count, double* warps);
int eagle_clip_motion_ecc(EagleHandle* h, int first, int count, int carry, double* warps, int* ok);
int eagle_track_frames_cmc(EagleHandle* h, EagleFrameResult* recs, int n, const double* warps );
#define EAGLE_REID_DIM 512
int eagle_reid_features(EagleHandle* h, const void* d_bgr, int n_frames, const EagleCrop* crops, int n_crops, float* feats);
int eagle_track_frames_reid(EagleHandle* h, EagleFrameResult* recs, int n, const double* warps , const float* feats,
                            const int32_t* feat_det, const int32_t* feat_count);

int eagle_team_colors(EagleHandle* h, const void* d_bgr, int n_frames, const EagleCrop* crops, int n_crops, int32_t* counts);

int eagle_comm_id(void* id128);
int eagle_comm_init(EagleHandle* h, int rank, int world, const void* id128);
int eagle_gather(EagleHandle* h, const EagleFrameResult* local, int n_local, EagleFrameResult* all );

typedef struct EagleTimings {
    float total_ms;
    float conv_ms;
    int32_t n_launches;
    int32_t n_conv_launches;
    double conv_flop;
    int32_t sat_events;
    int32_t sat_frames;
    int32_t graph_captures;
    int32_t graph_skipped;
    int32_t reserved[4];
} EagleTimings;
int eagle_set_profiling(EagleHandle* h, int per_kernel_events);
int eagle_get_timings(EagleHandle* h, EagleTimings* t);
typedef struct EagleKernelTime { char name[40]; float ms; int32_t launches; double bytes; double flop; } EagleKernelTime;
int eagle_get_kernel_times(EagleHandle* h, EagleKernelTime* out, int cap, int* n);

int eagle_op_conv2d(int device, int precision, const float* x, int n, int h, int w, int cin, const float* w_hwio,
                    const float* bias, int cout, int ks, int stride, int pre_act, const float* r1, const float* r2,
                    int post_act, float* y);
int eagle_op_bottleneck(int device, const float* x, int n, int h, int w, int cin, const float* w1, const float* b1, const float* w2, const float* b2,
                        const float* w3, const float* b3, const float* res, float* y, int reps, float* ms,
                        const float* wd , const float* bd);
int eagle_op_stem(int device, const uint8_t* bgr, int n, int h, int w, int dh, int dw, const float* w1, const float* b1, float* y, uint32_t* sat);
int eagle_op_fuse_sum(int device, int precision, const float* base, int n, int H, int W, int c, int n_up,
                      const float* const* ups, const int* up_h, const int* up_w, int relu, float* y);
int eagle_op_preprocess(int device, int precision, const uint8_t* bgr, int n, int h, int w, int det_imgsz,
                        float* kp_out , float* det_out , int* det_hw );
int eagle_op_preprocess_lb(int device, int precision, const uint8_t* bgr, int n, int h, int w, int det_imgsz, int letterbox ,
                           float* kp_out, float* det_out, int* det_hw);
int eagle_op_find_homography(int device, const float* img_pts, const float* world_pts, int n, double thresh,
                             int max_iters, int lm_iters, double* H9, uint8_t* mask, int* ok);

typedef struct EagleArgmaxPart { float score; int32_t idx; } EagleArgmaxPart;
int eagle_op_detect_tail(int device, int n_lv, const int* gh, const int* gw, const float* stride, const float* const* box, const float* const* cls, int n, int nc,
                         float conf_floor, float nms_iou, double detector_conf, int frame_h, int frame_w, int in_h, int in_w,
                         EagleFrameResult* out, float* boxes, float* conf, int32_t* cls_out);
int eagle_op_post(int device, int n, int hm_h, int hm_w, int chunks, const float* logits, const EagleArgmaxPart* parts, EagleArgmaxPart* parts_out,
                  EagleFrameResult* recs, int frame_h, int frame_w, double keypoint_conf, double ransac_thresh, int ransac_max_iters, int lm_iters);
int eagle_op_conv2d_argmax(int device, int precision, const float* x, int n, int h, int w, int cin, const float* w_hwio, const float* bias, int cout, int ks, int stride,
                           float* logits, EagleArgmaxPart* parts, int* tiles, int* tile_h, int* tile_w);

#define EAGLE_OP_SENTINEL_BITS 0x7fc5e171u
int eagle_op_reid_crop(int device, const uint8_t* bgr, int nf, int fh, int fw, const EagleCrop* crops, int n, int oh, int ow, int y_cs, int y_off, float* y);
int eagle_op_reid_conv7(int device, const float* x, int n, int h, int w, int x_cs, int x_off, const float* wt, const float* b, int y_cs, int y_off, float* y);
int eagle_op_reid_maxpool3s2(int device, const float* x, int n, int h, int w, int c, int x_cs, int x_off, int y_cs, int y_off, float* y);
int eagle_op_reid_avgpool2(int device, const float* x, int n, int h, int w, int c, int x_cs, int x_off, int y_cs, int y_off, float* y);
int eagle_op_reid_dw3(int device, const float* x, int n, int h, int w, int c, int x_cs, int x_off, const float* wt, const float* b, int y_cs, int y_off, float* y);
int eagle_op_reid_gate(int device, const float* const* streams, int n, int h, int w, int c, int x_cs, int x_off, const float* w1, const float* b1,
                       const float* w2, const float* b2, int c_real, int r, int y_cs, int y_off, float* g, float* y);
int eagle_op_reid_head(int device, const float* x, int n, int h, int w, int c, int x_cs, int x_off, const float* wt, const float* b, int dim, float* feats);

#define EAGLE_OP_RES_OWN 0
#define EAGLE_OP_RES_IN_Y 1
#define EAGLE_OP_RES_IN_X 2
int eagle_op_conv2d_sliced(int device, int precision, const float* x, int n, int h, int w, int cin, int x_cs, int x_off, const float* w_hwio, const float* bias,
                           int cout, int ks, int stride, int pre_act, const float* r1, int r1_cs, int r1_off, int r1_where,
                           const float* r2, int r2_cs, int r2_off, int r2_where, int post_act, int y_cs, int y_off, float* y);
int eagle_op_maxpool5(int device, int precision, const float* x, int n, int h, int w, int c, int x_cs, int x_off, int same_buffer, int y_cs, int y_off, float* y);
int eagle_op_upsample2(int device, int precision, const float* x, int n, int h, int w, int c, int x_cs, int x_off, int same_buffer, int yh, int yw, int y_cs, int y_off, float* y);
int eagle_op_split_to_f32(int device, const float* x, int n, int h, int w, int c, int x_cs, int x_off, int y_cs, int y_off, float* y);

int eagle_op_gray_pyramid(int device, const uint8_t* bgr, int n, int h, int w, uint8_t* g0, uint8_t* g1, uint8_t* g2, int* levels_out);
int eagle_op_flow(int device, const uint8_t* bgr, int n, int h, int w, int src_frame, int dst_frame, int hue_frame, const EagleFlowKp* in, int n_in,
                  EagleFlowKp* out , int* n_out, float* next_pts , uint8_t* status );

int eagle_debug(const char* key, int64_t value, void* out, int64_t out_bytes);

#ifdef __cplusplus
}
#endif
#endif
```

Baseline: 846.9.

## Merge HRNet fuse-layer stride-2 downsample heads from branch 0 into one conv

```diff
diff --git a/eagle_amd/csrc/common.h b/eagle_amd/csrc/common.h
--- a/eagle_amd/csrc/common.h
+++ b/eagle_amd/csrc/common.h
@@ -47,12 +47,14 @@
     int variant = 0;
 };
 struct ArgmaxPart { float score; int idx; };
+constexpr int CONV_NO_CUT = 0x7fffffff;
 struct ConvLaunch {
     ConvConfig cfg;
     TView x, y, r1, r2;
     const void* w = nullptr;
     const float* bias = nullptr;
     int pre_act = 0, post_act = 0;
+    int relu_from = CONV_NO_CUT, res_to = CONV_NO_CUT;
     int out_f32 = 0;
     double flop = 0;
     float descale = 1.0f;
@@ -62,10 +64,13 @@
 int conv_tiles_per_frame(int precision, const ConvConfig& cfg, int ho, int wo);
 void conv_tile_shape(int precision, const ConvConfig& cfg, int* th, int* tw);
 bool conv_supported(int precision, const ConvConfig& cfg);
+bool conv_supports_split_epilogue(int precision, const ConvConfig& cfg);
+int conv_epilogue_block(int precision, const ConvConfig& cfg);
+bool conv_is_adirect(int precision, const ConvConfig& cfg);
 void conv_launch(int precision, const ConvLaunch& L, hipStream_t s);
 size_t conv_weight_elems(int precision, const ConvConfig& cfg);
 size_t conv_lds_bytes(int precision, const ConvConfig& cfg);
-void conv_tile_weights(int precision, const ConvConfig& cfg, const float* w_hwio, int cin_real, int cout_real, void* dst, float* descale = nullptr);
+void conv_tile_weights(int precision, const ConvConfig& cfg, const float* w_hwio, int cin_real, int cout_real, void* dst, float* descale = nullptr, float w_absmax = 0.f);
 inline int prec_tensor_fmt(int precision) { return precision == EAGLE_PREC_F32 ? 1 : precision == EAGLE_PREC_F32S ? 2 : 0; }
 inline bool prec_is_f16_kernels(int precision) { return precision == EAGLE_PREC_F16 || precision == EAGLE_PREC_F32S; }
 ConvConfig conv_choose(int precision, int ks, int stride, int cin_pad, int cout_pad, int wo, bool plain_epilogue = false, bool second_residual = false);
diff --git a/eagle_amd/csrc/conv.hip b/eagle_amd/csrc/conv.hip
--- a/eagle_amd/csrc/conv.hip
+++ b/eagle_amd/csrc/conv.hip
@@ -118,6 +118,13 @@
     if (f && f->kind == ADIRECT) return c.ks == 3 && c.stride == (f->sform == S1 || f->sform == S1L ? 1 : 2) && c.kc == f->kc && c.nt == f->nt;
     return f && generic_inst(precision, c);
 }
+bool conv_supports_split_epilogue(int precision, const ConvConfig& c)
+{
+    const Form* f = find_form(precision, c.variant);
+    return f && precision == EAGLE_PREC_F32S && f->kind == ADIRECT && f->sform == S2T;
+}
+int conv_epilogue_block(int, const ConvConfig&) { return 48; }
+bool conv_is_adirect(int precision, const ConvConfig& c) { return kind_of(precision, c) == ADIRECT; }
 
 struct Tuned { int ks, s, cin, cout, wo, kc, nt, wx, variant; };
 static const Tuned g_tuned[] = {
@@ -263,7 +270,7 @@
     }
 }
 
-void conv_tile_weights(int precision, const ConvConfig& c, const float* w, int cin_real, int cout_real, void* dst, float* descale)
+void conv_tile_weights(int precision, const ConvConfig& c, const float* w, int cin_real, int cout_real, void* dst, float* descale, float w_absmax)
 {
     const int bn = c.nt * 16, nblk = c.cout_pad / bn, nch = c.cin / c.kc, taps = c.ks * c.ks, wimage = form_of(precision, c).wimage;
     auto W = [&](int tap, int ci, int co) -> float {
@@ -273,6 +280,10 @@
     if (precision == EAGLE_PREC_F32S) {
         float amax = 0.f;
         for (size_t k = 0; k < (size_t)taps * cin_real * cout_real; ++k) amax = std::max(amax, std::fabs(w[k]));
+        if (w_absmax > 0.f) {
+            if (amax > w_absmax) fail(EAGLE_E_INVALID, "conv_tile_weights: w_absmax %g is below the weights' largest magnitude %g", w_absmax, amax);
+            amax = w_absmax;
+        }
         int e = 0;
         if (amax > 0.f) (void)std::frexp(amax, &e);
         const int sw = 15 - e;
@@ -424,6 +435,14 @@
     }
     if (!a.r1 && a.r2) { a.r1 = a.r2; a.r1cs = a.r2cs; a.r1off = a.r2off; a.r2 = nullptr; }
     a.pre_act = L.pre_act; a.post_act = L.post_act; a.out_f32 = L.out_f32 || precision == EAGLE_PREC_F32;
+    a.relu_from = L.relu_from; a.res_to = L.res_to;
+    if (L.relu_from != CONV_NO_CUT || L.res_to != CONV_NO_CUT) {
+        const int blk = conv_epilogue_block(precision, c);
+        if (!conv_supports_split_epilogue(precision, c) || L.am_slot)
+            fail(EAGLE_E_NOKERNEL, "conv: the kernel form %d of family %d has no per-Cout-range epilogue", c.variant, precision);
+        if (L.relu_from < 0 || L.res_to < 0 || (L.relu_from != CONV_NO_CUT && L.relu_from % blk) || (L.res_to != CONV_NO_CUT && L.res_to % blk))
+            fail(EAGLE_E_INVALID, "conv: relu_from = %d / res_to = %d are not multiples of the epilogue block of %d channels", L.relu_from, L.res_to, blk);
+    }
     a.wx = c.wx;
     a.nchunks = c.cin / c.kc;
     a.zeros = conv_zero_page(); a.trash = conv_trash_page(); a.xcd = 0; a.gy = 1; a.stack = 0;
diff --git a/eagle_amd/csrc/conv_ad_split.inc b/eagle_amd/csrc/conv_ad_split.inc
--- a/eagle_amd/csrc/conv_ad_split.inc
+++ b/eagle_amd/csrc/conv_ad_split.inc
@@ -227,6 +227,7 @@
             }
         }
         const int co0 = nb * BN + cq * 48;
+        const bool with_res = co0 < a.res_to, relu = a.post_act == 1 || co0 >= a.relu_from;
         __builtin_amdgcn_sched_barrier(0);
         constexpr int NHR = 8 / KQ;
         const int row0 = (KQ == 2 && kq == 1) ? 2 : 0;
@@ -283,13 +284,13 @@
 #pragma unroll
                 for (int h2 = 0; h2 < HRB; ++h2)
 #pragma unroll
-                    for (int i = 0; i < 3; ++i) rres[h2][i] = __builtin_amdgcn_raw_buffer_load_b128(rrs, piece_off(hb0 + h2, i, a.r1cs, a.r1off), 0, EAGLE_RES_NT * 2);
+                    for (int i = 0; i < 3; ++i) rres[h2][i] = __builtin_amdgcn_raw_buffer_load_b128(rrs, with_res ? piece_off(hb0 + h2, i, a.r1cs, a.r1off) : OOB, 0, EAGLE_RES_NT * 2);
             }
             if (RES >= 2) {
 #pragma unroll
                 for (int h2 = 0; h2 < HRB; ++h2)
 #pragma unroll
-                    for (int i = 0; i < 3; ++i) rres2[h2][i] = __builtin_amdgcn_raw_buffer_load_b128(rrs2, piece_off(hb0 + h2, i, a.r2cs, a.r2off), 0, EAGLE_RES_NT * 2);
+                    for (int i = 0; i < 3; ++i) rres2[h2][i] = __builtin_amdgcn_raw_buffer_load_b128(rrs2, with_res ? piece_off(hb0 + h2, i, a.r2cs, a.r2off) : OOB, 0, EAGLE_RES_NT * 2);
             }
 #pragma unroll
             for (int h2 = 0; h2 < HRB; ++h2) {
@@ -323,7 +324,7 @@
                 }
 #pragma unroll
                 for (int tt = 0; tt < NT; ++tt) {
-                    if (a.post_act == 1) {
+                    if (relu) {
 #pragma unroll
                         for (int r = 0; r < 4; ++r) v[tt][r] = v[tt][r] > 0.f ? v[tt][r] : 0.f;
                     }
diff --git a/eagle_amd/csrc/conv_internal.h b/eagle_amd/csrc/conv_internal.h
--- a/eagle_amd/csrc/conv_internal.h
+++ b/eagle_amd/csrc/conv_internal.h
@@ -16,6 +16,7 @@
     const void* r1; int r1cs, r1off;
     const void* r2; int r2cs, r2off;
     int pre_act, post_act, out_f32;
+    int relu_from, res_to;
     int wx, tiles_x, tiles_y, nchunks;
     int gy;
     int stack;
diff --git a/eagle_amd/csrc/nets.hip b/eagle_amd/csrc/nets.hip
--- a/eagle_amd/csrc/nets.hip
+++ b/eagle_amd/csrc/nets.hip
@@ -1,6 +1,29 @@
 #include "runtime.h"
 
 namespace eagle {
+
+bool merge_heads(const std::vector<ConvHead>& heads, int taps, int cin, MergedHeads& m)
+{
+    const int n = (int)heads.size();
+    int n_res = 0; bool res_relu = false, plain = false;
+    for (const ConvHead& h : heads) { n_res += h.res ? 1 : 0; res_relu = res_relu || (h.res && h.relu); plain = plain || (!h.res && !h.relu); }
+    if (n == 0 || n_res > 1 || (res_relu && plain)) return false;
+    m = MergedHeads();
+    m.offset.assign(n, 0);
+    for (int rank = 0; rank < 3; ++rank)
+        for (int h = 0; h < n; ++h)
+            if ((heads[h].res ? 0 : heads[h].relu ? 2 : 1) == rank) { m.order.push_back(h); m.offset[h] = m.cout; m.cout += heads[h].cout; }
+    if (n_res) m.res_to = heads[m.order[0]].cout;
+    for (int k = n - 1; k >= 0 && heads[m.order[k]].relu; --k) m.relu_from = m.offset[m.order[k]];
+    m.w.assign((size_t)taps * cin * m.cout, 0.f); m.b.assign(m.cout, 0.f);
+    for (int h = 0; h < n; ++h) {
+        const int co = heads[h].cout, o0 = m.offset[h];
+        for (size_t r = 0; r < (size_t)taps * cin; ++r)
+            for (int o = 0; o < co; ++o) m.w[r * m.cout + o0 + o] = heads[h].w[r * co + o];
+        for (int o = 0; o < co; ++o) m.b[o0 + o] = heads[h].b[o];
+    }
+    return true;
+}
 
 struct Builder {
     EagleHandle* H;
@@ -36,6 +59,12 @@
     {
         std::vector<float> hwio, bias; int cin, cout, ks;
         fold(cname, bn, hwio, bias, cin, cout, ks);
+        return conv_folded(x, cname, hwio, bias, cin, cout, ks, stride, pre, r1, r2, post, out, out_f32, am_slot);
+    }
+    TView conv_folded(const TView& x, const std::string& cname, const std::vector<float>& hwio, std::vector<float>& bias, int cin, int cout, int ks, int stride, int pre,
+                      const TView* r1, const TView* r2, int post, const TView* out = nullptr, bool out_f32 = false, ArgmaxPart* const* am_slot = nullptr,
+                      const ConvConfig* cfg = nullptr, int relu_from = CONV_NO_CUT, int res_to = CONV_NO_CUT)
+    {
         if (cin > x.c) fail(EAGLE_E_INVALID, "%s: input has %d channels, weight expects %d", cname.c_str(), x.c, cin);
         const int cout_pad = (cout + 15) / 16 * 16;
         bias.resize(cout_pad, 0.f);
@@ -44,7 +73,8 @@
             if (FILE* f = fopen(dump, "a")) { fprintf(f, "%d,%d,%d,%d,%d,%d,%d\n", ks, stride, x.c, cout_pad, x.h, x.w, N); fclose(f); }
         }
         ConvLaunch L;
-        L.cfg = conv_choose(prec, ks, stride, x.c, cout_pad, wo, pre == ACT_NONE && post <= ACT_RELU && !out_f32, r1 && r2);
+        L.cfg = cfg ? *cfg : conv_choose(prec, ks, stride, x.c, cout_pad, wo, pre == ACT_NONE && post <= ACT_RELU && !out_f32, r1 && r2);
+        L.relu_from = relu_from; L.res_to = res_to;
         if (!conv_supported(prec, L.cfg))
             fail(EAGLE_E_NOKERNEL, "%s: no kernel instance (ks=%d s=%d kc=%d nt=%d)", cname.c_str(), ks, stride, L.cfg.kc, L.cfg.nt);
         const size_t ne = conv_weight_elems(prec, L.cfg);
@@ -72,7 +102,7 @@
         snprintf(label, sizeof(label), "conv %dx%d/%d %d->%d @%dx%d v%d%s", ks, ks, stride, cin, cout, ho, wo, L.cfg.variant, label_suffix);
         const double es = prec == EAGLE_PREC_F16 ? 2 : 4;
         emit_conv(label, L.flop, (double)N * x.h * x.w * cin * es + (double)N * ho * wo * cout * ((out_f32 || prec != EAGLE_PREC_F16) ? 4 : 2) * (am_slot ? 0 : 1) +
-                                 (r1 ? (double)N * ho * wo * cout * es : 0) + (r2 ? (double)N * ho * wo * cout * es : 0) + (double)ks * ks * cin * cout * es,
+                                 (r1 ? (double)N * ho * wo * std::min(cout, res_to) * es : 0) + (r2 ? (double)N * ho * wo * std::min(cout, res_to) * es : 0) + (double)ks * ks * cin * cout * es,
                   [L, pr](hipStream_t s) { conv_launch(pr, L, s); });
         return L.y;
     }
@@ -99,6 +129,33 @@
                     const float wv = w.data[((size_t)o * cin + i) * ks * ks + t];
                     hwio[((size_t)t * cin + i) * cout + o] = bn.empty() ? wv : (float)((double)wv * scale[o]);
                 }
+    }
+    struct HeadSpec { std::string conv, bn; bool res, relu; };
+    bool conv_heads(const TView& x, const std::vector<HeadSpec>& specs, int stride, const TView* res, TView& merged, std::vector<TView>& slices)
+    {
+        if (prec == EAGLE_PREC_F32 || specs.size() < 2) return false;
+        std::vector<std::vector<float>> hw(specs.size()), bs(specs.size());
+        std::vector<ConvHead> heads;
+        int cin0 = 0, ks0 = 0;
+        for (size_t h = 0; h < specs.size(); ++h) {
+            int cin, cout, ks;
+            fold(specs[h].conv, specs[h].bn, hw[h], bs[h], cin, cout, ks);
+            if (h == 0) { cin0 = cin; ks0 = ks; }
+            if (cin != cin0 || ks != ks0 || cout % 16) return false;
+            heads.push_back({hw[h].data(), bs[h].data(), cout, specs[h].res, specs[h].relu});
+        }
+        MergedHeads m;
+        if (!merge_heads(heads, ks0 * ks0, cin0, m)) return false;
+        const int wo = (x.w + 2 * (ks0 / 2) - ks0) / stride + 1;
+        const ConvConfig cfg = conv_choose(prec, ks0, stride, x.c, m.cout, wo, true, false);
+        if (!conv_supported(prec, cfg) || !conv_supports_split_epilogue(prec, cfg) || !conv_is_adirect(prec, cfg)) return false;
+        const int blk = conv_epilogue_block(prec, cfg);
+        if ((m.res_to != CONV_NO_CUT && m.res_to % blk) || (m.relu_from != CONV_NO_CUT && m.relu_from % blk)) return false;
+        merged = conv_folded(x, specs[0].conv, m.w, m.b, cin0, m.cout, ks0, stride, 0, nullptr, m.res_to != CONV_NO_CUT ? res : nullptr, 0, nullptr, false, nullptr,
+                             &cfg, m.relu_from, m.res_to);
+        slices.resize(specs.size());
+        for (size_t h = 0; h < specs.size(); ++h) slices[h] = merged.slice(m.offset[h], heads[h].cout);
+        return true;
     }
     void refuse_2gib(const std::string& name, const char* what, std::initializer_list<const TView*> ts)
     {
@@ -205,6 +262,28 @@
         B.fork_join(Op::JOIN, nb - 1);
         const int n_out = (last_single && m == n_modules - 1) ? 1 : nb;
         std::vector<TView> out;
+        const char* me = getenv("EAGLE_HR_MERGE_HEADS");
+        TView down0[4];
+        bool has_down0[4] = {};
+        std::vector<TView> merged;
+        if (B.prec != EAGLE_PREC_F32 && n_out > 2 && !(me && atoi(me) == 0)) {
+            std::vector<Builder::HeadSpec> specs; std::vector<int> who;
+            for (int i = 1; i < n_out; ++i) {
+                const std::string r = q + "fuse_layers." + std::to_string(i) + ".0.0.";
+                const bool last = i == 1;
+                specs.push_back({r + "0", r + "1", last, !last || i == nb - 1});
+                who.push_back(i);
+            }
+            TView mt; std::vector<TView> sl;
+            if (B.conv_heads(xs[0], specs, 2, &xs[1], mt, sl)) {
+                merged.push_back(mt);
+                for (size_t k = 0; k < who.size(); ++k) { down0[who[k]] = sl[k]; has_down0[who[k]] = true; }
+            }
+        }
+        auto release_own = [&](const TView& v) {
+            for (const TView& mt : merged) if (mt.p == v.p) return;
+            B.release(v);
+        };
         if (n_out > 1) B.fork_join(Op::FORK, n_out - 1);
         for (int i = 0; i < n_out; ++i) {
             B.set_stream(n_out > 1 ? i : 0);
@@ -215,17 +294,19 @@
                     const std::string r = q + "fuse_layers." + std::to_string(i) + "." + std::to_string(j) + "." + std::to_string(k) + ".";
                     const bool last = k == i - j - 1;
                     TView nt;
-                    if (!last) {
+                    if (j == 0 && k == 0 && has_down0[i]) {
+                        nt = down0[i];
+                    } else if (!last) {
                         nt = B.conv(t, r + "0", r + "1", 2, 0, nullptr, nullptr, R);
                     } else {
                         const TView* ident = (j == i - 1) ? &xs[i] : nullptr;
                         const bool relu_now = ident && i == nb - 1;
                         nt = B.conv(t, r + "0", r + "1", 2, 0, have_y ? &y : nullptr, ident, relu_now ? R : 0);
                     }
-                    if (k > 0) B.release(t);
+                    if (k > 0) release_own(t);
                     t = nt;
                 }
-                if (have_y) B.release(y);
+                if (have_y) release_own(y);
                 y = t; have_y = true;
             }
             if (i == 0) y = xs[0];
@@ -241,13 +322,14 @@
                 B.other([base, u0, u1, u2, n_up, o, Hh](hipStream_t s) { FuseUp u[3] = {u0, u1, u2}; fuse_sum_launch(base, u, n_up, 1, o, s, Hh->cur_sat); }, "fuse_sum",
                         Builder::vbytes(base) + Builder::vbytes(o) + (nu > 0 ? Builder::vbytes(ups[0].z) : 0) + (nu > 1 ? Builder::vbytes(ups[1].z) : 0) + (nu > 2 ? Builder::vbytes(ups[2].z) : 0));
                 for (int k = 0; k < nu; ++k) B.release(ups[k].z);
-                if (i != 0) B.release(y);
+                if (i != 0) release_own(y);
                 y = o;
             }
             out.push_back(y);
         }
         B.set_stream(0);
         if (n_out > 1) B.fork_join(Op::JOIN, n_out - 1);
+        for (const TView& mt : merged) B.release(mt);
         for (int b = 0; b < nb; ++b) B.release(xs[b]);
         xs = out;
     }
diff --git a/eagle_amd/csrc/ops_api.hip b/eagle_amd/csrc/ops_api.hip
--- a/eagle_amd/csrc/ops_api.hip
+++ b/eagle_amd/csrc/ops_api.hip
@@ -52,8 +52,18 @@
                     const float* bias, int cout, int ks, int stride, int pre_act, const float* r1, const float* r2,
                     int post_act, float* y)
 {
-    EagleHandle* hh = nullptr;
-    API_BEGIN
+    return eagle_op_conv2d_ex(device, precision, x, n, h, w, cin, w_hwio, bias, cout, ks, stride, pre_act, r1, r2, post_act, -1, -1, 0.f, y);
+}
+
+int eagle_op_conv2d_ex(int device, int precision, const float* x, int n, int h, int w, int cin, const float* w_hwio,
+                       const float* bias, int cout, int ks, int stride, int pre_act, const float* r1, const float* r2,
+                       int post_act, int relu_from, int res_to, float w_absmax, float* y)
+{
+    EagleHandle* hh = nullptr;
+    API_BEGIN
+    if (relu_from < -1 || res_to < -1 || (res_to >= 0 && res_to < cout && res_to % 16)) fail(EAGLE_E_INVALID, "eagle_op_conv2d_ex: relu_from / res_to are -1 (off) or channel counts, res_to a multiple of 16");
+    const int res_c = (res_to >= 0 && res_to < cout) ? res_to : cout;
+    if ((r1 || r2) && res_c == 0) fail(EAGLE_E_INVALID, "eagle_op_conv2d_ex: res_to = 0 takes no residual tensor");
     HIP_CHECK(hipSetDevice(device));
     Net net;
     const int g = precision == EAGLE_PREC_F32 ? 4 : 8;
@@ -64,19 +74,42 @@
     L.cfg = conv_choose(precision, ks, stride, cin_pad, cout_pad, wo, pre_act == ACT_NONE && post_act <= ACT_RELU, r1 && r2);
     if (!conv_supported(precision, L.cfg)) fail(EAGLE_E_NOKERNEL, "no kernel instance ks=%d s=%d kc=%d nt=%d", ks, stride, L.cfg.kc, L.cfg.nt);
     std::vector<char> tiled(conv_weight_elems(precision, L.cfg) * (precision == EAGLE_PREC_F32 ? 4 : 2));
-    conv_tile_weights(precision, L.cfg, w_hwio, cin, cout, tiled.data(), &L.descale);
+    conv_tile_weights(precision, L.cfg, w_hwio, cin, cout, tiled.data(), &L.descale, w_absmax);
     L.w = net.upload(tiled.data(), tiled.size());
     std::vector<float> b(cout_pad, 0.f);
     for (int i = 0; i < cout; ++i) b[i] = bias[i];
     L.bias = (const float*)net.upload(b.data(), b.size() * 4);
     L.y.n = n; L.y.h = ho; L.y.w = wo; L.y.c = cout_pad; L.y.cs = cout_pad; L.y.f32 = prec_tensor_fmt(precision);
     L.y.p = net.get((size_t)n * ho * wo * cout_pad * L.y.esize());
-    if (r1) to_dev(net, precision, r1, n, ho, wo, cout, cout_pad, L.r1);
-    if (r2) to_dev(net, precision, r2, n, ho, wo, cout, cout_pad, L.r2);
+    const int res_pad = res_c == cout ? cout_pad : res_c;
+    if (r1) to_dev(net, precision, r1, n, ho, wo, res_c, res_pad, L.r1);
+    if (r2) to_dev(net, precision, r2, n, ho, wo, res_c, res_pad, L.r2);
     L.pre_act = pre_act; L.post_act = post_act;
+    if (relu_from >= 0) L.relu_from = relu_from;
+    if (res_to >= 0) L.res_to = res_to;
     conv_launch(precision, L, nullptr);
     HIP_CHECK(hipDeviceSynchronize());
     from_dev(L.y, cout, y);
+    API_END(hh)
+}
+
+int eagle_op_merge_heads(int n_heads, int taps, int cin, const int* couts, const int* res, const int* relu, const float* const* w, const float* const* b,
+                         float* w_out, float* b_out, int* order, int* offset, int* res_to, int* relu_from)
+{
+    EagleHandle* hh = nullptr;
+    API_BEGIN
+    if (n_heads < 1 || taps < 1 || cin < 1 || !couts || !res || !relu || !w || !b || !w_out || !b_out || !order || !offset || !res_to || !relu_from)
+        fail(EAGLE_E_INVALID, "eagle_op_merge_heads: bad argument");
+    std::vector<ConvHead> heads;
+    for (int h = 0; h < n_heads; ++h) {
+        if (couts[h] < 1 || !w[h] || !b[h]) fail(EAGLE_E_INVALID, "eagle_op_merge_heads: head %d is empty", h);
+        heads.push_back({w[h], b[h], couts[h], res[h] != 0, relu[h] != 0});
+    }
+    MergedHeads m;
+    if (!merge_heads(heads, taps, cin, m)) fail(EAGLE_E_INVALID, "eagle_op_merge_heads: these heads have no order with single cut points");
+    std::copy(m.w.begin(), m.w.end(), w_out); std::copy(m.b.begin(), m.b.end(), b_out);
+    std::copy(m.order.begin(), m.order.end(), order); std::copy(m.offset.begin(), m.offset.end(), offset);
+    *res_to = m.res_to == CONV_NO_CUT ? -1 : m.res_to; *relu_from = m.relu_from == CONV_NO_CUT ? -1 : m.relu_from;
     API_END(hh)
 }
 
diff --git a/eagle_amd/csrc/runtime.h b/eagle_amd/csrc/runtime.h
--- a/eagle_amd/csrc/runtime.h
+++ b/eagle_amd/csrc/runtime.h
@@ -282,6 +282,13 @@
 namespace eagle {
 constexpr int REID_NB = 64;
 void finalize(EagleHandle* h);
+struct ConvHead { const float* w; const float* b; int cout; bool res, relu; };
+struct MergedHeads {
+    std::vector<float> w, b;
+    int cout = 0, res_to = CONV_NO_CUT, relu_from = CONV_NO_CUT;
+    std::vector<int> order, offset;
+};
+bool merge_heads(const std::vector<ConvHead>& heads, int taps, int cin, MergedHeads& m);
 size_t sat_pad_bytes(int B);
 void run_net(EagleHandle* h, Net* net, hipStream_t s, size_t& ev_i);
 void check_saturation(EagleHandle* h, const char* what);
diff --git a/eagle_amd/lib.py b/eagle_amd/lib.py
--- a/eagle_amd/lib.py
+++ b/eagle_amd/lib.py
@@ -261,6 +261,9 @@
     L.eagle_get_timings.argtypes = [vp, C.POINTER(EagleTimings)]
     L.eagle_get_kernel_times.argtypes = [vp, C.POINTER(EagleKernelTime), i32, C.POINTER(i32)]
     L.eagle_op_conv2d.argtypes = [i32, i32, fp, i32, i32, i32, i32, fp, fp, i32, i32, i32, i32, fp, fp, i32, fp]
+    L.eagle_op_conv2d_ex.argtypes = [i32, i32, fp, i32, i32, i32, i32, fp, fp, i32, i32, i32, i32, fp, fp, i32, i32, i32, C.c_float, fp]
+    L.eagle_op_merge_heads.argtypes = [i32, i32, i32, C.POINTER(i32), C.POINTER(i32), C.POINTER(i32), C.POINTER(fp), C.POINTER(fp), fp, fp, C.POINTER(i32), C.POINTER(i32),
+                                       C.POINTER(i32), C.POINTER(i32)]
     L.eagle_op_bottleneck.argtypes = [i32, fp, i32, i32, i32, i32, fp, fp, fp, fp, fp, fp, fp, fp, i32, fp, fp, fp]
     L.eagle_op_stem.argtypes = [i32, u8p, i32, i32, i32, i32, i32, fp, fp, fp, C.POINTER(C.c_uint32)]
     L.eagle_op_fuse_sum.argtypes = [i32, i32, fp, i32, i32, i32, i32, i32, C.POINTER(fp), C.POINTER(i32), C.POINTER(i32), i32, fp]
@@ -423,7 +426,7 @@
            "eagle_topview_mosaic_device", "eagle_topview_mosaic_finish", "eagle_topview_residual_device", "eagle_topview_mosaic_frames", "eagle_topview_residual_frames",
            "eagle_op_topview", "eagle_op_reid_crop", "eagle_op_reid_conv7", "eagle_op_reid_maxpool3s2", "eagle_op_reid_avgpool2", "eagle_op_reid_dw3",
            "eagle_op_reid_gate", "eagle_op_reid_head", "eagle_op_conv2d_sliced", "eagle_op_maxpool5", "eagle_op_upsample2", "eagle_op_split_to_f32", "eagle_op_gray_pyramid",
-           "eagle_op_flow"]
+           "eagle_op_flow", "eagle_op_conv2d_ex", "eagle_op_merge_heads"]
 
 FLOWKP_DTYPE = np.dtype([("label", "<i4"), ("x", "<i4"), ("y", "<i4"), ("score", "<f4")], align=True)
 E_REFERENCE_RAISES = -7
@@ -1208,7 +1211,7 @@
     return buf.raw
 
 
-def op_conv2d(x, w_hwio, bias, stride=1, pre=0, r1=None, r2=None, post=0, precision=PREC_F32, device=0):
+def op_conv2d(x, w_hwio, bias, stride=1, pre=0, r1=None, r2=None, post=0, precision=PREC_F32, device=0, relu_from=None, res_to=None, w_absmax=0.0):
     L = load()
     x = np.ascontiguousarray(x, np.float32); w = np.ascontiguousarray(w_hwio, np.float32); b = np.ascontiguousarray(bias, np.float32)
     n, h, wd, cin = x.shape
@@ -1218,10 +1221,33 @@
     y = np.empty((n, ho, wo, cout), np.float32)
     r1 = None if r1 is None else np.ascontiguousarray(r1, np.float32)
     r2 = None if r2 is None else np.ascontiguousarray(r2, np.float32)
-    rc = L.eagle_op_conv2d(device, precision, _fp(x), n, h, wd, cin, _fp(w), _fp(b), cout, ks, stride, pre, _fp(r1), _fp(r2), post, _fp(y))
+    if relu_from is None and res_to is None and not w_absmax:
+        rc = L.eagle_op_conv2d(device, precision, _fp(x), n, h, wd, cin, _fp(w), _fp(b), cout, ks, stride, pre, _fp(r1), _fp(r2), post, _fp(y))
+    else:
+        rc = L.eagle_op_conv2d_ex(device, precision, _fp(x), n, h, wd, cin, _fp(w), _fp(b), cout, ks, stride, pre, _fp(r1), _fp(r2), post,
+                                  -1 if relu_from is None else int(relu_from), -1 if res_to is None else int(res_to), float(w_absmax), _fp(y))
     if rc:
         raise EagleError(f"eagle_op_conv2d failed ({rc}): {L.eagle_last_error(None).decode()}")
     return y
+
+
+def merge_heads(heads):
+    L = load()
+    ws = [np.ascontiguousarray(h[0], np.float32) for h in heads]
+    bs = [np.ascontiguousarray(h[1], np.float32) for h in heads]
+    n = len(heads)
+    ks, _, cin, _ = ws[0].shape
+    couts = (C.c_int32 * n)(*[w.shape[3] for w in ws])
+    res = (C.c_int32 * n)(*[int(bool(h[2])) for h in heads]); relu = (C.c_int32 * n)(*[int(bool(h[3])) for h in heads])
+    fpt = C.POINTER(C.c_float)
+    wp = (fpt * n)(*[_fp(w) for w in ws]); bp = (fpt * n)(*[_fp(b) for b in bs])
+    total = sum(w.shape[3] for w in ws)
+    w_out = np.empty((ks, ks, cin, total), np.float32); b_out = np.empty(total, np.float32)
+    order = (C.c_int32 * n)(); offset = (C.c_int32 * n)(); res_to = C.c_int32(); relu_from = C.c_int32()
+    rc = L.eagle_op_merge_heads(n, ks * ks, cin, couts, res, relu, wp, bp, _fp(w_out), _fp(b_out), order, offset, C.byref(res_to), C.byref(relu_from))
+    if rc:
+        raise EagleError(f"eagle_op_merge_heads failed ({rc}): {L.eagle_last_error(None).decode()}")
+    return w_out, b_out, list(order), list(offset), None if res_to.value < 0 else res_to.value, None if relu_from.value < 0 else relu_from.value
 
 
 def op_bottleneck(x, w1, b1, w2, b2, w3, b3, res=None, reps=0, device=0, wd=None, bd=None):
diff --git a/include/eagle.h b/include/eagle.h
--- a/include/eagle.h
+++ b/include/eagle.h
@@ -612,6 +612,11 @@
 int eagle_op_conv2d(int device, int precision, const float* x, int n, int h, int w, int cin, const float* w_hwio,
                     const float* bias, int cout, int ks, int stride, int pre_act, const float* r1, const float* r2,
                     int post_act, float* y);
+int eagle_op_conv2d_ex(int device, int precision, const float* x, int n, int h, int w, int cin, const float* w_hwio,
+                       const float* bias, int cout, int ks, int stride, int pre_act, const float* r1, const float* r2,
+                       int post_act, int relu_from, int res_to, float w_absmax, float* y);
+int eagle_op_merge_heads(int n_heads, int taps, int cin, const int* couts, const int* res, const int* relu, const float* const* w, const float* const* b,
+                         float* w_out, float* b_out, int* order, int* offset, int* res_to, int* relu_from);
 int eagle_op_bottleneck(int device, const float* x, int n, int h, int w, int cin, const float* w1, const float* b1, const float* w2, const float* b2,
                         const float* w3, const float* b3, const float* res, float* y, int reps, float* ms,
                         const float* wd , const float* bd);
```

New measurement: 849.8, median of 6. No clear change (+0.3%).
